# whigg/surikatoko

Hardware: AMD Instinct MI355X
Metric: BA iterations/sec (higher is better)
Workload: dtype f64

## Files before the change

### include/srk_ba.h

```cpp
#ifndef SRK_BA_H
#define SRK_BA_H
#include <stdint.h>
#ifdef __cplusplus
extern "C" {
#endif

typedef struct srk_ba srk_ba;

enum srk_status {
    SRK_STATUS_NONE = 0,
    SRK_STATUS_ABS_ERR_THRESHOLD = 1,
    SRK_STATUS_SMALL_ERR_CHANGE = 2,
    SRK_STATUS_HESSIAN_OVERFLOW = 3,
    SRK_STATUS_ERR_CONVERGED = 4,
    SRK_STATUS_MAX_ITERATIONS = 5,
    SRK_STATUS_DEVICE_ERROR = 6
};

enum srk_error {
    SRK_OK = 0,
    SRK_E_ARGS = -1,
    SRK_E_DEVICE = -2,
    SRK_E_STATE = -3,
    SRK_E_NOMEM = -4
// ... 56 lines not shown
                               int32_t n_frames, float* cam_R, float* cam_T,
                               const float* K, int shared_k,
                               const int64_t* obs_row_ptr, const int32_t* obs_frame, const float* obs_uv,
                               const float* allowed_err_change, const float* max_hessian_factor,
                               int64_t max_iterations, srk_ba_report* out);

double srk_ba_reproj_error(srk_ba*, double f0,
                           int64_t n_points, const double* points_xyz,
                           int32_t n_frames, const double* cam_R, const double* cam_T,
                           const double* K, int shared_k,
                           const int64_t* obs_row_ptr, const int32_t* obs_frame, const double* obs_uv,
                           int64_t* seen );

int srk_ba_reproj_error_mvf(srk_ba*, double f0,
                            int64_t n_points, const double* points_xyz,
                            int32_t n_frames, const double* cam_R, const double* cam_T,
                            const double* K, int shared_k,
                            const int64_t* obs_row_ptr, const int32_t* obs_frame, const double* obs_uv,
                            double z_tol, double* reproj_err, int64_t* summands );

int srk_mvf_estimate_depths(srk_ba*, int64_t n_tracks, const int64_t* row_ptr, const int32_t* frame,
                            const double* x_meter , int32_t n_frames, const double* cam_R, const double* cam_T,
                            double* depth_out );
int srk_mvf_relative_motion(srk_ba*, int64_t n_points, const double* x_anchor , const double* x_target ,
                            const double* depth_anchor , double* R_out , double* T_out );
int srk_mvf_project_onto_so3(const double* R_noisy, const double* T_noisy, double* R_out, double* T_out);

int srk_ba_normalize_scene(int64_t n_points, double* points_xyz, int32_t n_frames, double* cam_R, double* cam_T,
                           double t1y, int32_t unity_comp_ind, srk_ba_normalizer* out);
void srk_ba_revert_normalization(int64_t n_points, double* points_xyz, int32_t n_frames, double* cam_R,
                                 double* cam_T, const srk_ba_normalizer* nrm);
int srk_ba_check_world_is_normalized(int32_t n_frames, const double* cam_R, const double* cam_T, double t1y,
                                     int32_t unity_comp_ind);

int srk_ba_upload_scene(srk_ba*, double f0,
                        int64_t n_points, const double* points_xyz,
                        int32_t n_frames, const double* cam_R, const double* cam_T,
                        const double* K, int shared_k,
                        const int64_t* obs_row_ptr, const int32_t* obs_frame, const double* obs_uv,
                        int already_normalized);
int srk_ba_optimize(srk_ba*, const double* allowed_err_change, const double* max_hessian_factor,
                    int64_t max_iterations, srk_ba_report* out);
int srk_ba_download_scene(srk_ba*, double* points_xyz, double* cam_R, double* cam_T, int revert_normalization);
int srk_ba_reset_scene(srk_ba*);

int srk_ba_phase_error(srk_ba*, double* err, int64_t* seen);
int srk_ba_phase_derivatives(srk_ba*);
int srk_ba_phase_schur(srk_ba*, double hessian_factor);
int srk_ba_phase_solve(srk_ba*);
int srk_ba_phase_backsub(srk_ba*, double hessian_factor);
int srk_ba_phase_accept(srk_ba*);

enum srk_buffer {
    SRK_BUF_GRAD = 0,
    SRK_BUF_POINT_BLOCKS,
    SRK_BUF_FRAME_BLOCKS,
    SRK_BUF_POINT_FRAME,
    SRK_BUF_RCS,
    SRK_BUF_RCS_RHS,
    SRK_BUF_CORRECTIONS,
    SRK_BUF_POINTS,
    SRK_BUF_CAM_R,
    SRK_BUF_CAM_T
};
int64_t srk_ba_buffer_size(srk_ba*, int which);
int srk_ba_download(srk_ba*, int which, double* dst, int64_t count);
int srk_ba_download_rcs_rows(srk_ba*, const int64_t* rows, int64_t n_rows, double* dst);

int srk_ba_set_covisibility(srk_ba*, const int32_t* min_cv );
int srk_ba_set_rcs_mode(srk_ba*, int mode );
int srk_ba_rcs_chunks(srk_ba*);
double srk_ba_rcs_fill(srk_ba*);
double srk_ba_solve_mfma_flops(srk_ba*);

int srk_ba_set_solver_fusion(srk_ba*, int on);
int64_t srk_ba_solver_sync_timeouts(srk_ba*);
int srk_ba_solver_fusion(srk_ba*);

int64_t srk_ba_iteration_log(srk_ba*, int64_t cap, int32_t* attempts, double* ms_since_start, double* err,
                             double* hessian_factor);

int srk_ba_set_speculation(srk_ba*, int on);

int srk_ba_set_deterministic(srk_ba*, int on);
int srk_ba_deterministic(srk_ba*);

int srk_ba_set_multi_schedule(srk_ba*, int mode);
int srk_ba_multi_schedule(srk_ba*);

int srk_ba_set_frame_reordering(srk_ba*, int mode);
int srk_ba_set_frame_order(srk_ba*, const int32_t* to_internal , int32_t n_frames);
int srk_ba_frame_order(srk_ba*, int32_t* to_internal );
int srk_frame_order(int mode, int64_t n_points, int32_t n_frames, const int64_t* obs_row_ptr, const int32_t* obs_frame,
                    int32_t* to_internal );

int srk_ba_set_jacobian_mode(srk_ba*, int mode);
int srk_ba_jacobian_kernel(srk_ba*);

int srk_ba_set_storage_precision(srk_ba*, int f32);

int srk_ba_set_schur_precision(srk_ba*, int fp32);

int srk_ba_set_fixed_intrinsics(srk_ba*, int on);
int srk_ba_frame_vars(srk_ba*);
int64_t srk_ba_schur_fallback_landmarks(srk_ba*);

int srk_ba_set_intrinsic_groups(srk_ba*, const int32_t* group , int32_t n_frames, int32_t n_groups);
int srk_ba_intrinsic_groups(srk_ba*);
int srk_ba_download_intrinsics(srk_ba*, double* K, int32_t n_groups);

int srk_ba_set_robust_loss(srk_ba*, int kind , double delta_pixels);
int srk_ba_robust_loss(srk_ba*, int* kind, double* delta_pixels);
int srk_ba_observation_weights(srk_ba*, double* w, int64_t count);

int srk_ba_set_observation_information(srk_ba*, const double* q , int64_t count);
int srk_ba_observation_information(srk_ba*, double* q, int64_t count);
int srk_ba_observation_residuals(srk_ba*, double* exy_pixels , int64_t count);

int srk_ba_set_constant_blocks(srk_ba*, const uint8_t* frame_const , int32_t n_frames,
                               const uint8_t* point_const , int64_t n_points, int keep_gauge);
int srk_ba_constant_blocks(srk_ba*, uint8_t* frame_const, uint8_t* point_const, int* keep_gauge);
int srk_ba_constant_counts(srk_ba*, int32_t* n_frames, int64_t* n_points);
int srk_ba_constant_pass_ms(srk_ba*, double* points_ms, double* frames_ms);

int srk_ba_set_position_priors(srk_ba*, int64_t n_point_priors, const int64_t* point_index ,
                               const double* point_pos , const double* point_info ,
                               int32_t n_frame_priors, const int32_t* frame_index ,
                               const double* frame_centre , const double* frame_info , int keep_gauge);
int srk_ba_position_prior_counts(srk_ba*, int64_t* n_point_priors, int32_t* n_frame_priors);
int srk_ba_position_priors(srk_ba*, int64_t* point_index, double* point_pos, double* point_info, int32_t* frame_index,
                           double* frame_centre, double* frame_info, int* keep_gauge);
int srk_ba_prior_error(srk_ba*, double* e_points, double* e_frames);
int srk_ba_prior_residuals(srk_ba*, double* d_points, double* d_frames);
int srk_ba_normalize_position_priors(const srk_ba_normalizer* nrm, int64_t n, const double* pos, const double* info,
                                     double* pos_out, double* info_out);
int srk_ba_prior_pass_ms(srk_ba*, double* derivative_ms, double* error_ms);

int srk_ba_set_relative_pose_factors(srk_ba*, int32_t n, const int32_t* frame_a, const int32_t* frame_b ,
                                     const double* rel_R , const double* rel_t ,
                                     const double* info );
int srk_ba_check_relative_pose_factors(int32_t n, const int32_t* frame_a, const int32_t* frame_b, const double* rel_R,
                                       const double* rel_t, const double* info, const char** why);
int srk_ba_relative_pose_factor_count(srk_ba*, int32_t* n);
int srk_ba_relative_pose_factors(srk_ba*, int32_t* frame_a, int32_t* frame_b, double* rel_R, double* rel_t, double* info);
int srk_ba_relative_pose_error(srk_ba*, double* e);
int srk_ba_relative_pose_residuals(srk_ba*, double* r);
int srk_ba_normalize_relative_pose_factors(const srk_ba_normalizer* nrm, int32_t n, const double* rel_t, const double* info,
                                           double* rel_t_out, double* info_out);
int srk_ba_relative_pose_pass_ms(srk_ba*, double* derivative_ms, double* couple_ms, double* error_ms);

int srk_ba_phase_covariance(srk_ba*, int32_t n_frames_sel, const int32_t* frames ,
                            double* frame_blocks , int64_t n_points_sel, const int64_t* points,
                            double* point_blocks );
int srk_ba_covariances(srk_ba*, double sigma_pixels, int32_t n_frames_sel, const int32_t* frames, double* frame_cov ,
                       int64_t n_points_sel, const int64_t* points, double* point_cov , int caller_coordinates);
int srk_ba_revert_covariances(const srk_ba_normalizer* nrm, int frame_vars, int32_t n_frames, double* frame_cov ,
                              int64_t n_points, double* point_cov );
int srk_ba_set_covariance_batch(srk_ba*, int64_t max_columns);

int srk_ba_phase_cross_covariance(srk_ba*, int64_t n_ff, const int32_t* ff_a, const int32_t* ff_b,
                                  double* ff_blocks , int64_t n_pf, const int64_t* pf_point,
                                  const int32_t* pf_frame, double* pf_blocks , int64_t n_pp, const int64_t* pp_a,
                                  const int64_t* pp_b, double* pp_blocks );
int srk_ba_cross_covariances(srk_ba*, double sigma_pixels, int64_t n_ff, const int32_t* ff_a, const int32_t* ff_b, double* ff_cov,
                             int64_t n_pf, const int64_t* pf_point, const int32_t* pf_frame, double* pf_cov, int64_t n_pp,
                             const int64_t* pp_a, const int64_t* pp_b, double* pp_cov, int caller_coordinates);
// ... 42 lines not shown
```

### surikatoko_amd/_lib.py

```python
import ctypes as C
import os
import subprocess

_HERE = os.path.dirname(os.path.abspath(__file__))
_PATH = os.environ.get("SRK_BA_LIBRARY") or os.path.join(_HERE, "libsrk_ba.so")
_lib = None


class LibraryNotBuilt(RuntimeError):
    pass


def library_path():
    return _PATH


def build_library(jobs=4):
    subprocess.check_call(["make", "-s", "-j", str(jobs), "-C", os.path.join(_HERE, "csrc")])
    return _PATH


class Report(C.Structure):
    _fields_ = [("status", C.c_int32), ("optimized", C.c_int32), ("iterations", C.c_int64),
                ("attempts", C.c_int64), ("seen", C.c_int64), ("err_initial", C.c_double),
                ("err_final", C.c_double), ("hessian_factor", C.c_double), ("world_scale", C.c_double),
                ("ms_jacobian", C.c_double), ("ms_schur", C.c_double), ("ms_solve", C.c_double),
                ("ms_backsub", C.c_double), ("ms_apply", C.c_double), ("ms_error", C.c_double),
                ("ms_total", C.c_double), ("schur_launches", C.c_int64), ("jacobian_launches", C.c_int64),
                ("ms_jacobian_kernel", C.c_double), ("ms_solve_syrk", C.c_double),
                ("solve_mfma_flops", C.c_double)]

    def as_dict(self):
        return {k: getattr(self, k) for k, _ in self._fields_}


class Normalizer(C.Structure):
    _fields_ = [("R0", C.c_double * 9), ("T0", C.c_double * 3), ("world_scale", C.c_double)]


class SceneSpecC(C.Structure):
    _fields_ = [("n_frames", C.c_int32), ("grid_nx", C.c_int32), ("grid_ny", C.c_int32), ("vis_window", C.c_int32),
                ("half_extent_x", C.c_double), ("half_extent_y", C.c_double), ("f0", C.c_double),
                ("noise_x3d_hi", C.c_double), ("noise_r_hi", C.c_double), ("noise_uv_pix", C.c_double),
                ("seed", C.c_uint32)]


ALLREDUCE_FN = C.CFUNCTYPE(C.c_int, C.c_void_p, C.c_void_p, C.c_int64)

EXPORTS = [
    "srk_ba_create", "srk_ba_destroy", "srk_ba_last_error", "srk_ba_status_string", "srk_ba_device_count",
    "srk_ba_set_stream", "srk_ba_set_allreduce", "srk_ba_rccl_get_unique_id", "srk_ba_rccl_init", "srk_ba_rccl_init_second", "srk_ba_rccl_set_comm", "srk_ba_compute_inplace", "srk_ba_compute_inplace_f32", "srk_ba_reproj_error", "srk_ba_reproj_error_mvf", "srk_mvf_estimate_depths", "srk_mvf_relative_motion",
    "srk_mvf_project_onto_so3", "srk_ba_set_schur_precision", "srk_ba_set_storage_precision", "srk_ba_set_speculation", "srk_ba_set_deterministic", "srk_ba_deterministic", "srk_ba_set_multi_schedule", "srk_ba_multi_schedule", "srk_ba_set_frame_reordering", "srk_ba_set_frame_order", "srk_ba_frame_order", "srk_frame_order", "srk_ba_set_solver_fusion", "srk_ba_solver_sync_timeouts", "srk_ba_iteration_log", "srk_ba_solver_fusion", "srk_ba_set_jacobian_mode", "srk_ba_jacobian_kernel", "srk_ba_set_fixed_intrinsics", "srk_ba_frame_vars", "srk_ba_schur_fallback_landmarks",
    "srk_ba_set_robust_loss", "srk_ba_robust_loss", "srk_ba_observation_weights",
    "srk_ba_set_observation_information", "srk_ba_observation_information", "srk_ba_observation_residuals",
    "srk_ba_set_intrinsic_groups", "srk_ba_intrinsic_groups", "srk_ba_download_intrinsics",
    "srk_ba_set_constant_blocks", "srk_ba_constant_blocks", "srk_ba_constant_counts", "srk_ba_constant_pass_ms",
    "srk_ba_set_position_priors", "srk_ba_position_prior_counts", "srk_ba_position_priors", "srk_ba_prior_error",
    "srk_ba_prior_residuals", "srk_ba_normalize_position_priors", "srk_ba_prior_pass_ms",
    "srk_ba_set_relative_pose_factors", "srk_ba_check_relative_pose_factors", "srk_ba_relative_pose_factor_count", "srk_ba_relative_pose_factors",
    "srk_ba_relative_pose_error", "srk_ba_relative_pose_residuals", "srk_ba_normalize_relative_pose_factors",
    "srk_ba_relative_pose_pass_ms",
    "srk_ba_phase_covariance", "srk_ba_covariances", "srk_ba_revert_covariances", "srk_ba_set_covariance_batch",
    "srk_ba_phase_cross_covariance", "srk_ba_cross_covariances", "srk_ba_revert_cross_covariances", "srk_ba_relative_pose_covariances",
    "srk_ba_normalize_scene", "srk_ba_revert_normalization", "srk_ba_check_world_is_normalized",
    "srk_ba_upload_scene", "srk_ba_optimize", "srk_ba_download_scene", "srk_ba_reset_scene", "srk_ba_phase_error",
    "srk_ba_phase_derivatives", "srk_ba_phase_schur", "srk_ba_phase_solve", "srk_ba_phase_backsub",
    "srk_ba_phase_accept", "srk_ba_buffer_size", "srk_ba_download", "srk_ba_download_rcs_rows", "srk_ba_set_profile", "srk_ba_dense_spd_solve",
    "srk_ba_set_covisibility", "srk_ba_set_rcs_mode", "srk_ba_rcs_fill", "srk_ba_solve_mfma_flops", "srk_ba_rcs_chunks",
    "srk_scene_num_observations", "srk_scene_generate", "srk_circle_camera_shots",
    "srk_read_matrix_file", "srk_decompose_proj_mat", "srk_triangulate_least_squares", "srk_dino_load",
]


def lib():
    global _lib
    if _lib is not None:
        return _lib
    try:
        import torch
    except ImportError:
        pass
    if not os.path.exists(_PATH):
        raise LibraryNotBuilt(
            f"{_PATH} is missing: run `python -c 'import __graft_entry__ as g; g.build()'` "
            "(or make -C surikatoko_amd/csrc).  There is no CPU fallback.")
    L = C.CDLL(_PATH)
    L.srk_ba_create.restype = C.c_void_p
    L.srk_ba_create.argtypes = [C.c_int]
    L.srk_ba_destroy.argtypes = [C.c_void_p]
    L.srk_ba_destroy.restype = None
    L.srk_ba_last_error.restype = C.c_char_p
    L.srk_ba_last_error.argtypes = [C.c_void_p]
    L.srk_ba_status_string.restype = C.c_char_p
    L.srk_ba_status_string.argtypes = [C.c_int]
    L.srk_ba_reproj_error.restype = C.c_double
    L.srk_ba_reproj_error_mvf.restype = C.c_int
    L.srk_ba_buffer_size.restype = C.c_int64
    L.srk_ba_buffer_size.argtypes = [C.c_void_p, C.c_int]
    L.srk_scene_num_observations.restype = C.c_int64
    L.srk_ba_rcs_fill.restype = C.c_double
    L.srk_ba_rcs_fill.argtypes = [C.c_void_p]
    L.srk_ba_solve_mfma_flops.restype = C.c_double
    L.srk_ba_solve_mfma_flops.argtypes = [C.c_void_p]
    L.srk_ba_set_stream.argtypes = [C.c_void_p, C.c_void_p]
    L.srk_ba_set_allreduce.argtypes = [C.c_void_p, ALLREDUCE_FN, C.c_void_p, C.c_int, C.c_int]
    L.srk_ba_set_robust_loss.argtypes = [C.c_void_p, C.c_int, C.c_double]
    L.srk_ba_robust_loss.argtypes = [C.c_void_p, C.POINTER(C.c_int), C.POINTER(C.c_double)]
    L.srk_ba_observation_weights.argtypes = [C.c_void_p, C.POINTER(C.c_double), C.c_int64]
    L.srk_ba_set_observation_information.argtypes = [C.c_void_p, C.POINTER(C.c_double), C.c_int64]
    L.srk_ba_observation_information.argtypes = [C.c_void_p, C.POINTER(C.c_double), C.c_int64]
    L.srk_ba_observation_residuals.argtypes = [C.c_void_p, C.POINTER(C.c_double), C.c_int64]
    L.srk_ba_set_intrinsic_groups.argtypes = [C.c_void_p, C.c_void_p, C.c_int32, C.c_int32]
    L.srk_ba_intrinsic_groups.argtypes = [C.c_void_p]
    L.srk_ba_download_intrinsics.argtypes = [C.c_void_p, C.POINTER(C.c_double), C.c_int32]
    L.srk_ba_set_constant_blocks.argtypes = [C.c_void_p, C.c_void_p, C.c_int32, C.c_void_p, C.c_int64, C.c_int]
    L.srk_ba_constant_blocks.argtypes = [C.c_void_p, C.c_void_p, C.c_void_p, C.POINTER(C.c_int)]
    L.srk_ba_constant_counts.argtypes = [C.c_void_p, C.POINTER(C.c_int32), C.POINTER(C.c_int64)]
    L.srk_ba_constant_pass_ms.argtypes = [C.c_void_p, C.POINTER(C.c_double), C.POINTER(C.c_double)]
    L.srk_ba_set_position_priors.argtypes = [C.c_void_p, C.c_int64, C.c_void_p, C.c_void_p, C.c_void_p, C.c_int32, C.c_void_p,
                                             C.c_void_p, C.c_void_p, C.c_int]
    L.srk_ba_position_prior_counts.argtypes = [C.c_void_p, C.POINTER(C.c_int64), C.POINTER(C.c_int32)]
    L.srk_ba_position_priors.argtypes = [C.c_void_p, C.c_void_p, C.c_void_p, C.c_void_p, C.c_void_p, C.c_void_p, C.c_void_p,
                                         C.POINTER(C.c_int)]
    L.srk_ba_prior_error.argtypes = [C.c_void_p, C.POINTER(C.c_double), C.POINTER(C.c_double)]
    L.srk_ba_prior_residuals.argtypes = [C.c_void_p, C.c_void_p, C.c_void_p]
    L.srk_ba_normalize_position_priors.argtypes = [C.c_void_p, C.c_int64, C.c_void_p, C.c_void_p, C.c_void_p, C.c_void_p]
    L.srk_ba_prior_pass_ms.argtypes = [C.c_void_p, C.POINTER(C.c_double), C.POINTER(C.c_double)]
    L.srk_ba_set_relative_pose_factors.argtypes = [C.c_void_p, C.c_int32, C.c_void_p, C.c_void_p, C.c_void_p, C.c_void_p, C.c_void_p]
    L.srk_ba_check_relative_pose_factors.argtypes = [C.c_int32, C.c_void_p, C.c_void_p, C.c_void_p, C.c_void_p, C.c_void_p, C.POINTER(C.c_char_p)]
    L.srk_ba_relative_pose_factor_count.argtypes = [C.c_void_p, C.POINTER(C.c_int32)]
    L.srk_ba_relative_pose_factors.argtypes = [C.c_void_p, C.c_void_p, C.c_void_p, C.c_void_p, C.c_void_p, C.c_void_p]
    L.srk_ba_relative_pose_error.argtypes = [C.c_void_p, C.POINTER(C.c_double)]
    L.srk_ba_relative_pose_residuals.argtypes = [C.c_void_p, C.c_void_p]
    L.srk_ba_normalize_relative_pose_factors.argtypes = [C.c_void_p, C.c_int32, C.c_void_p, C.c_void_p, C.c_void_p, C.c_void_p]
    L.srk_ba_relative_pose_pass_ms.argtypes = [C.c_void_p, C.POINTER(C.c_double), C.POINTER(C.c_double), C.POINTER(C.c_double)]
# ... 14 lines not shown
```

### surikatoko_amd/ba.py

```python
import ctypes as C
import math

import numpy as np

from ._lib import Normalizer, Report, lib

BUF_GRAD, BUF_POINT_BLOCKS, BUF_FRAME_BLOCKS, BUF_POINT_FRAME, BUF_RCS, BUF_RCS_RHS, BUF_CORRECTIONS, BUF_POINTS, \
    BUF_CAM_R, BUF_CAM_T = range(10)


def _p(a):
    return a.ctypes.data_as(C.c_void_p)


def status_string(status):
    return lib().srk_ba_status_string(int(status)).decode()


def device_count():
    return int(lib().srk_ba_device_count())


class Scene:

# ... 296 lines not shown
        a32 = C.c_float(term_crit.AllowedReprojErrRelativeChange()) if a64 is not None else None
        m32 = C.c_float(term_crit.MaxHessianFactor()) if m64 is not None else None
        self._f0 = float(f0)
        self.report = Report()
        rc = self._lib.srk_ba_compute_inplace_f32(
            C.c_void_p(self._h), C.c_float(f0), C.c_int64(points.shape[0]), _p(points), C.c_int32(cam_R.shape[0]), _p(cam_R),
            _p(cam_T), _p(K), C.c_int(int(bool(shared_k))), _p(rp), _p(fr), _p(obs_uv),
            C.byref(a32) if a32 is not None else None, C.byref(m32) if m32 is not None else None,
            C.c_int64(max_iterations), C.byref(self.report))
        self._raise(rc)
        self._status = status_string(self.report.status)
        return rc == 0

    def ReprojError(self, f0, scene):
        seen = C.c_int64(0)
        e = self._lib.srk_ba_reproj_error(C.c_void_p(self._h), C.c_double(f0), *scene.scene_args(), C.byref(seen))
        if math.isnan(e):
            msg = self.last_error()
            if "hip" in msg.lower():
                raise RuntimeError("srk_ba_reproj_error: " + msg)
            raise ValueError("srk_ba_reproj_error: " + msg)
        self._f0 = float(f0)
        return float(e), int(seen.value)

    def ReprojErrorMvf(self, f0, scene, z_tol=1e-5):
        e, n = C.c_double(0), C.c_int64(0)
        rc = self._lib.srk_ba_reproj_error_mvf(C.c_void_p(self._h), C.c_double(f0), *scene.scene_args(), C.c_double(z_tol),
                                               C.byref(e), C.byref(n))
        if rc < 0:
            msg = self.last_error()
            if "hip" in msg.lower():
                raise RuntimeError("srk_ba_reproj_error_mvf: " + msg)
            raise ValueError("srk_ba_reproj_error_mvf: " + msg)
        return rc == 1, float(e.value), int(n.value)

    def ReprojErrorPixPerPoint(self, reproj_err, seen_points_count):
        return self._f0 * math.sqrt(reproj_err / float(seen_points_count))

    def OptimizationStatusString(self):
        return self._status

    def PointsCount(self):
        return self._scene.N

    def FramesCount(self):
        return self._scene.M

    def VarsCount(self):
        return 3 * self._scene.N + self.frame_vars() * self._scene.M + 4 * self.intrinsic_groups()

    def NormalizedVarsCount(self):
        return self.VarsCount() - 7

    def upload(self, f0, scene, already_normalized=False):
        self._f0 = float(f0)
        self._scene = scene
        rc = self._lib.srk_ba_upload_scene(C.c_void_p(self._h), C.c_double(f0), *scene.scene_args(),
                                           C.c_int(int(already_normalized)))
        if rc == 1:
            return False
        self._raise(rc)
        return True

    def optimize(self, term_crit=None, max_iterations=0):
        a, m = self._criteria(term_crit)
        self.report = Report()
        rc = self._lib.srk_ba_optimize(C.c_void_p(self._h), a, m, C.c_int64(max_iterations), C.byref(self.report))
        self._raise(rc)
        self._status = status_string(self.report.status)
        return rc == 0

    def download(self, scene=None, revert_normalization=True):
        scene = scene or self._scene
        self._raise(self._lib.srk_ba_download_scene(C.c_void_p(self._h), _p(scene.points), _p(scene.cam_R),
                                                    _p(scene.cam_T), C.c_int(int(revert_normalization))))
        return scene

    def reset(self):
        self._raise(self._lib.srk_ba_reset_scene(C.c_void_p(self._h)))

    def set_speculation(self, on=True):
        self._raise(self._lib.srk_ba_set_speculation(C.c_void_p(self._h), C.c_int(int(bool(on)))))

    def set_deterministic(self, on=True):
        self._raise(self._lib.srk_ba_set_deterministic(C.c_void_p(self._h), C.c_int(int(bool(on)))))

    def deterministic(self):
        return int(self._lib.srk_ba_deterministic(C.c_void_p(self._h))) == 1

    MULTI_SCHEDULES = {"allreduce": 0, "dp": 1, "dp_force": 2}

    def set_multi_schedule(self, schedule="dp"):
        self._raise(self._lib.srk_ba_set_multi_schedule(C.c_void_p(self._h), C.c_int(self.MULTI_SCHEDULES[schedule])))

    def multi_schedule(self):
        return {0: "allreduce", 1: "dp", 2: "dp (self-check passed)", 3: "allreduce (dp self-check failed)"}[
            int(self._lib.srk_ba_multi_schedule(C.c_void_p(self._h)))]

    def set_frame_reordering(self, mode=-1):
        self._raise(self._lib.srk_ba_set_frame_reordering(C.c_void_p(self._h), C.c_int(mode)))

    def set_frame_order(self, to_internal=None):
        if to_internal is None:
            self._raise(self._lib.srk_ba_set_frame_order(C.c_void_p(self._h), None, C.c_int32(0)))
        else:
            a = np.ascontiguousarray(to_internal, dtype=np.int32)
            self._raise(self._lib.srk_ba_set_frame_order(C.c_void_p(self._h), _p(a), C.c_int32(a.size)))

    def frame_order(self):
        to_int = np.zeros(self._scene.M if self._scene is not None else 0, np.int32)
        rc = self._lib.srk_ba_frame_order(C.c_void_p(self._h), _p(to_int))
        if rc < 0:
            self._raise(rc)
        return to_int if rc == 1 else None

    def set_solver_fusion(self, on=True):
        self._raise(self._lib.srk_ba_set_solver_fusion(C.c_void_p(self._h), C.c_int(int(bool(on)))))

    def solver_fusion(self):
        return bool(self._lib.srk_ba_solver_fusion(C.c_void_p(self._h)))

    def solver_sync_timeouts(self):
        self._lib.srk_ba_solver_sync_timeouts.restype = C.c_int64
        return int(self._lib.srk_ba_solver_sync_timeouts(C.c_void_p(self._h)))

    def iteration_log(self):
        fn = self._lib.srk_ba_iteration_log
        fn.restype = C.c_int64
        n = int(fn(C.c_void_p(self._h), C.c_int64(0), None, None, None, None))
        att = np.zeros(max(n, 1), dtype=np.int32)
        ms = np.zeros(max(n, 1))
        err = np.zeros(max(n, 1))
        fac = np.zeros(max(n, 1))
        fn(C.c_void_p(self._h), C.c_int64(n), att.ctypes.data_as(C.c_void_p), ms.ctypes.data_as(C.c_void_p),
           err.ctypes.data_as(C.c_void_p), fac.ctypes.data_as(C.c_void_p))
        return {"attempts": att[:n], "ms": ms[:n], "err": err[:n], "hessian_factor": fac[:n]}

    def set_jacobian_mode(self, mode=-1):
        self._raise(self._lib.srk_ba_set_jacobian_mode(C.c_void_p(self._h), C.c_int(mode)))

    def jacobian_kernel(self):
        return int(self._lib.srk_ba_jacobian_kernel(C.c_void_p(self._h)))

    def set_storage_precision(self, f32=False):
        self._raise(self._lib.srk_ba_set_storage_precision(C.c_void_p(self._h), C.c_int(int(bool(f32)))))

    def set_fixed_intrinsics(self, on=True):
        self._raise(self._lib.srk_ba_set_fixed_intrinsics(C.c_void_p(self._h), C.c_int(int(bool(on)))))

    def frame_vars(self):
        n = int(self._lib.srk_ba_frame_vars(C.c_void_p(self._h)))
        self._raise(n)
        return n

    def set_intrinsic_groups(self, groups):
        if groups is None:
            self._raise(self._lib.srk_ba_set_intrinsic_groups(C.c_void_p(self._h), None, C.c_int32(0), C.c_int32(0)))
            return
        g = np.ascontiguousarray(groups, dtype=np.int32)
        n_groups = int(g.max()) + 1 if g.size else 0
        self._raise(self._lib.srk_ba_set_intrinsic_groups(C.c_void_p(self._h), g.ctypes.data_as(C.c_void_p),
                                                          C.c_int32(g.size), C.c_int32(n_groups)))

    def intrinsic_groups(self):
        n = int(self._lib.srk_ba_intrinsic_groups(C.c_void_p(self._h)))
        self._raise(n)
# ... 446 lines not shown
```

### surikatoko_amd/csrc/srk_ba_host.hip

```cpp
#include "../../include/srk_ba.h"
#include "srk_dev.hpp"
#include "srk_cov.hpp"
#include "srk_geom.hpp"
#include "srk_plan.hpp"

#include <dlfcn.h>
#include <rccl/rccl.h>

#include <algorithm>
#include <chrono>
#include <numeric>
#include <cmath>
#include <cstdio>
#include <cstdlib>
#include <cstring>
#include <string>
#include <iterator>
#include <map>
#include <memory>
#include <vector>
#include <unordered_set>
#include <thread>

namespace {

struct DevBuf {
    void* p = nullptr;
    size_t bytes = 0;
};

}

#define SRK_FUSION_RETRIES 3
#define SRK_SLOTS 3
struct srk_ba : SrkPlanKept {
    int device = 0;
    int cus = 256;
    bool own_stream = true;
    std::string last_error;

    bool have_scene = false;
    SrkDims d{};
    double f0 = 0;
    srk_ba_normalizer nrm{};
    bool normalized_on_upload = false;

    DevBuf pts[SRK_SLOTS + 1], camR[SRK_SLOTS + 1], camT[SRK_SLOTS + 1], K, cam[SRK_SLOTS + 1];
    DevBuf pts0, camR0, camT0;
    DevBuf row_ptr, obs_frame, obs_pt, obs_uv, col_ptr, fobs_pt, fobs_uv;
    DevBuf W, Vg, Ug, scratch;
    int frame_order_mode = -1;
    std::vector<int32_t> frame_order_given;
    DevBuf grp_first, grp_count, grp_nf, grp_frames, obs_slot, pt_mask, gen_list, wg_jmin;
    DevBuf cal_list;
    DevBuf lg_item, lg_np, lg_nf, lg_pts, lg_frames, lg_obs_off, lg_obs;
    DevBuf sc_pts, sc_R, sc_T, sc_K, sc_cam, sc_frame, sc_pt, sc_uv, sc_partial, sc_out;
    DevBuf jr_first, jr_count, jr_jmin, jr_group;
    DevBuf jd_nf, jd_frames, jd_mask;
    bool deterministic = false;
    DevBuf dj_ptr, dj_ent, dj_stage, ds_pair_ptr, ds_pair_fa, ds_pair_fb, ds_pair_ent, ds_f_ptr, ds_f_ent;
    int jac_mode = -1;
    std::vector<int64_t> env_col_h, env_off_h, row_end_h, col_begin_h;
    DevBuf env_col, env_off, band_col, band_off;
    int64_t env_packed = 0, band_packed = 0;
    bool use_envelope = true;
    bool use_chunks = true;
    struct Attempt {
        DevBuf S, rhs, wy, dc, acc, dx, err_partial, info, dinv, packed, sync_flags;
        DevBuf irr;
        DevBuf det_stage, det_rhs;
        DevBuf Ssh, rsh, ysh, dcsh, dinvsh, Tsh;
        SrkChunkPlan plan;
        SrkCholSync sync;
        std::vector<DevBuf> plan_bufs;
        std::vector<char> plan_zeroed;
        std::vector<std::unique_ptr<SrkChunkPlan>> plan_children;
        std::vector<int64_t> plan_sig;
        SrkSolveProf solve_prof;
        double* host_back = nullptr;
        hipStream_t stream = nullptr;
        hipEvent_t done = nullptr;
        hipEvent_t ev_a = nullptr, ev_b = nullptr;
        double* err_dst = nullptr;
        int trial = 1;
        int slot = 0;
        bool allocated = false;
    };
    Attempt att[SRK_SLOTS];
    hipStream_t main_stream = nullptr;
    hipEvent_t ev_jac = nullptr;
    bool speculate = true;
    int cur = 0;

    srk_allreduce_fn allreduce = nullptr;
    void* allreduce_ctx = nullptr;
    int rank = 0, world = 1;
    ncclComm_t comm = nullptr;
    bool comm_owned = false;
    ncclComm_t comm2 = nullptr;
    bool spec_multi = true;
    bool dp_schedule = true;
    bool dp_force = false;
    bool dp_verified = false;
    bool dp_selfcheck_failed = false;
    DevBuf dp_chk;
    hipStream_t comm_stream = nullptr;
    hipEvent_t ev_comm = nullptr;
    DevBuf status_all;
    double* dp_back = nullptr;
    int64_t seen_global = -1;

    hipEvent_t ev[16]{};
    std::vector<hipEvent_t> chol_ev;
    bool schur_fp32 = false;
    bool store_f32 = false;
    bool fixed_k = false;
    std::vector<int32_t> igroup_user;
    int32_t igroup_n = 0;
    int32_t shk_G = 0;
    int64_t shk_ncols = 0, shk_ldb = 0;
    DevBuf Ks[SRK_SLOTS + 1], shk_grp, shk_lo, shk_hi, shk_mptr, shk_mem, shk_env;
    std::vector<int32_t> shk_grp_h, shk_first;
    std::vector<double> shk_k22_user;
    std::vector<int64_t> shk_row_end, shk_col_begin;
    int loss_kind = SRK_LOSS_NONE;
    double loss_delta_pix = 0;
    std::vector<double> info_user;
    bool info_on = false;
    DevBuf info_q, info_qf;
    bool cst_set = false;
    int cst_keep_gauge = 1;
    std::vector<uint8_t> cst_frame_user, cst_point_user;
    DevBuf cst_pts, cst_frames;
// ... 74 lines not shown
        a.Reduce = reinterpret_cast<decltype(a.Reduce)>(dlsym(a.lib, "ncclReduce"));
        a.Broadcast = reinterpret_cast<decltype(a.Broadcast)>(dlsym(a.lib, "ncclBroadcast"));
        a.GroupStart = reinterpret_cast<decltype(a.GroupStart)>(dlsym(a.lib, "ncclGroupStart"));
        a.GroupEnd = reinterpret_cast<decltype(a.GroupEnd)>(dlsym(a.lib, "ncclGroupEnd"));
        a.rooted = a.Reduce && a.Broadcast && a.GroupStart && a.GroupEnd;
        a.ok = a.GetUniqueId && a.CommInitRank && a.CommDestroy && a.AllReduce && a.GetErrorString;
        return a;
    }();
    return api;
}
}

#define HIPCHK(h, expr)                                                                              \
    do {                                                                                             \
        hipError_t _e = (expr);                                                                      \
        if (_e != hipSuccess) {                                                                      \
            (h)->last_error = std::string(#expr) + ": " + hipGetErrorString(_e);                     \
            return SRK_E_DEVICE;                                                                     \
        }                                                                                            \
    } while (0)

static int dev_alloc(srk_ba* h, DevBuf& b, size_t bytes)
{
    if (bytes == 0) bytes = 8;
    if (b.p && b.bytes >= bytes) return SRK_OK;
    if (b.p) {
        hipFree(b.p);
        b.p = nullptr;
        b.bytes = 0;
    }
    hipError_t e = hipMalloc(&b.p, bytes);
    if (e != hipSuccess) {
        h->last_error = std::string("hipMalloc: ") + hipGetErrorString(e);
        b.p = nullptr;
        return e == hipErrorOutOfMemory ? SRK_E_NOMEM : SRK_E_DEVICE;
    }
    b.bytes = bytes;
    return SRK_OK;
}
static void dev_free(DevBuf& b)
{
    if (b.p) hipFree(b.p);
    b.p = nullptr;
    b.bytes = 0;
}
template <typename T> static T* P(const DevBuf& b) { return reinterpret_cast<T*>(b.p); }

extern "C" {

int srk_ba_device_count(void)
{
    int n = 0;
    if (hipGetDeviceCount(&n) != hipSuccess) return 0;
    return n;
}

srk_ba* srk_ba_create(int device_id)
{
    int n = srk_ba_device_count();
    if (n <= 0 || device_id < 0 || device_id >= n) {
        fprintf(stderr, "srk_ba_create: no usable HIP device (count=%d, requested=%d); there is no CPU fallback\n", n,
                device_id);
        return nullptr;
    }
    if (hipSetDevice(device_id) != hipSuccess) return nullptr;
    srk_ba* h = new srk_ba();
    h->device = device_id;
    hipDeviceProp_t prop;
    if (hipGetDeviceProperties(&prop, device_id) == hipSuccess && prop.multiProcessorCount > 0) h->cus = prop.multiProcessorCount;
    if (hipStreamCreate(&h->main_stream) != hipSuccess) {
        delete h;
        return nullptr;
    }
#ifdef SRK_DEV
    if (const char* e = getenv("SRK_CHOL_FUSED")) h->chol_fused = h->chol_fused_wanted = e[0] != '0';
    if (const char* e = getenv("SRK_MULTI_SPECULATION")) h->spec_multi = e[0] != '0';
    if (const char* e = getenv("SRK_MULTI_SCHEDULE")) {
        h->dp_schedule = std::strcmp(e, "allreduce") != 0;
        h->dp_force = std::strcmp(e, "dp_force") == 0;
    }
#endif
    h->att[0].stream = h->main_stream;
    bool ok = hipEventCreateWithFlags(&h->ev_jac, hipEventDisableTiming) == hipSuccess &&
              hipEventCreateWithFlags(&h->ev_comm, hipEventDisableTiming) == hipSuccess &&
              hipStreamCreateWithFlags(&h->comm_stream, hipStreamNonBlocking) == hipSuccess &&
              hipHostMalloc(reinterpret_cast<void**>(&h->dp_back), 64 * SRK_SLOTS, hipHostMallocDefault) == hipSuccess &&
              hipMalloc(&h->status_all.p, 64 * SRK_SLOTS) == hipSuccess;
    if (ok) h->status_all.bytes = 64 * SRK_SLOTS, ok = hipMemset(h->status_all.p, 0, 64 * SRK_SLOTS) == hipSuccess;
    for (int sl = 0; sl < SRK_SLOTS; ++sl) {
        auto& a = h->att[sl];
        a.slot = sl;
        a.trial = sl + 1;
        a.err_dst = ok ? P<double>(h->status_all) + 8 * sl : nullptr;
        if (sl > 0) ok = ok && hipStreamCreateWithFlags(&a.stream, hipStreamNonBlocking) == hipSuccess;
        ok = ok && hipEventCreateWithFlags(&a.done, hipEventDisableTiming) == hipSuccess &&
             hipEventCreateWithFlags(&a.ev_a, hipEventDisableTiming) == hipSuccess &&
             hipEventCreateWithFlags(&a.ev_b, hipEventDisableTiming) == hipSuccess &&
             hipHostMalloc(reinterpret_cast<void**>(&a.host_back), 64, hipHostMallocDefault) == hipSuccess;
    }
    for (auto& e : h->ev) ok = ok && hipEventCreate(&e) == hipSuccess;
    if (!ok) {
        delete h;
        return nullptr;
    }
    return h;
}

void srk_ba_destroy(srk_ba* h)
{
    if (!h) return;
    hipSetDevice(h->device);
    if (h->main_stream) hipStreamSynchronize(h->main_stream);
    for (int sl = 1; sl < SRK_SLOTS; ++sl)
        if (h->att[sl].stream) hipStreamSynchronize(h->att[sl].stream);
    if (h->comm_stream) hipStreamSynchronize(h->comm_stream);
    if (h->comm2) rccl().CommDestroy(h->comm2);
    if (h->comm && h->comm_owned) rccl().CommDestroy(h->comm);
    h->comm = h->comm2 = nullptr;
    for (int w = 0; w < SRK_SLOTS + 1; ++w)
        for (DevBuf* b : { &h->pts[w], &h->camR[w], &h->camT[w], &h->cam[w], &h->Ks[w] }) dev_free(*b);
    dev_free(h->status_all);
    if (h->dp_back) hipHostFree(h->dp_back);
    DevBuf* all[] = { &h->K, &h->pts0, &h->camR0, &h->camT0, &h->row_ptr,
                      &h->obs_frame, &h->obs_pt, &h->obs_uv, &h->col_ptr, &h->fobs_pt, &h->fobs_uv, &h->W, &h->Vg, &h->Ug,
                      &h->scratch, &h->grp_first, &h->grp_count, &h->grp_nf, &h->grp_frames, &h->obs_slot, &h->pt_mask,
                      &h->gen_list, &h->cal_list, &h->env_col, &h->env_off, &h->wg_jmin, &h->band_col, &h->band_off,
                      &h->dj_ptr, &h->dj_ent, &h->dj_stage, &h->ds_pair_ptr, &h->ds_pair_fa, &h->ds_pair_fb, &h->ds_pair_ent, &h->ds_f_ptr, &h->ds_f_ent,
                      &h->jd_nf, &h->jd_frames, &h->jd_mask,
                      &h->jr_first, &h->jr_count, &h->jr_jmin, &h->jr_group, &h->lg_item, &h->lg_np, &h->lg_nf, &h->lg_pts, &h->lg_frames,
                      &h->lg_obs_off, &h->lg_obs, &h->shk_grp, &h->shk_lo, &h->shk_hi, &h->shk_mptr, &h->shk_mem, &h->shk_env, &h->dp_chk,
                      &h->info_q, &h->info_qf, &h->cst_pts, &h->cst_frames, &h->pri_pt_list, &h->pri_pt_val, &h->pri_fr_list, &h->pri_fr_val,
                      &h->rp_fa, &h->rp_fb, &h->rp_val, &h->rp_fr_list, &h->rp_fr_ptr, &h->rp_fr_ent, &h->rp_tgt, &h->rp_cpl,
                      &h->cov_Y, &h->cov_grp, &h->cov_blk, &h->cov_out, &h->cov_free, &h->cov_colb, &h->cov_pairs };
    for (DevBuf* b : all) dev_free(*b);
    for (auto& a : h->att) {
        for (DevBuf* b : { &a.S, &a.rhs, &a.wy, &a.dc, &a.acc, &a.dx, &a.err_partial, &a.info, &a.dinv, &a.packed, &a.sync_flags, &a.irr, &a.det_stage, &a.det_rhs,
                          &a.Ssh, &a.rsh, &a.ysh, &a.dcsh, &a.dinvsh, &a.Tsh }) dev_free(*b);
        for (DevBuf& b : a.plan_bufs) dev_free(b);
        if (a.host_back) hipHostFree(a.host_back);
        if (a.done) hipEventDestroy(a.done);
        if (a.ev_a) hipEventDestroy(a.ev_a);
        if (a.ev_b) hipEventDestroy(a.ev_b);
    }
    for (DevBuf* b : { &h->sc_pts, &h->sc_R, &h->sc_T, &h->sc_K, &h->sc_cam, &h->sc_frame, &h->sc_pt, &h->sc_uv, &h->sc_partial, &h->sc_out })
        dev_free(*b);
    for (auto& e : h->ev)
        if (e) hipEventDestroy(e);
    for (auto& e : h->chol_ev) hipEventDestroy(e);
    if (h->ev_jac) hipEventDestroy(h->ev_jac);
    for (auto& e : h->ev_cst)
        if (e) hipEventDestroy(e);
    for (auto& e : h->ev_pri)
        if (e) hipEventDestroy(e);
    for (auto& e : h->ev_rp)
        if (e) hipEventDestroy(e);
    if (h->ev_comm) hipEventDestroy(h->ev_comm);
    if (h->comm_stream) hipStreamDestroy(h->comm_stream);
    for (int sl = 1; sl < SRK_SLOTS; ++sl)
        if (h->att[sl].stream) hipStreamDestroy(h->att[sl].stream);
    if (h->own_stream && h->main_stream) hipStreamDestroy(h->main_stream);
    delete h;
}

const char* srk_ba_last_error(const srk_ba* h) { return h ? h->last_error.c_str() : "null handle"; }

const char* srk_ba_status_string(int status)
{
    switch (status) {
    case SRK_STATUS_ABS_ERR_THRESHOLD: return "abs err threshold";
    case SRK_STATUS_SMALL_ERR_CHANGE: return "small relative err change";
    case SRK_STATUS_HESSIAN_OVERFLOW: return "hessian overflow";
    case SRK_STATUS_ERR_CONVERGED: return "err converged to limit value";
    case SRK_STATUS_MAX_ITERATIONS: return "max iterations";
    case SRK_STATUS_DEVICE_ERROR: return "device error";
    default: return "";
    }
}

int srk_ba_set_stream(srk_ba* h, void* hip_stream)
{
    if (!h) return SRK_E_ARGS;
    hipSetDevice(h->device);
    if (h->main_stream) hipStreamSynchronize(h->main_stream);
    if (h->own_stream && h->main_stream) hipStreamDestroy(h->main_stream);
    h->main_stream = h->att[0].stream = reinterpret_cast<hipStream_t>(hip_stream);
    h->own_stream = false;
    return SRK_OK;
}

static bool exchange_after_reordered_upload(srk_ba* h, int world_size)
{
    if (world_size < 2 || !h->have_scene || h->frame_int.empty() || h->frame_order_supplied) return false;
    h->last_error = "the uploaded scene's frames were renumbered for one rank; configure the exchange before the upload";
    return true;
}

static const char* fixed_k_conflict(bool fixed_k, bool deterministic, bool store_f32, bool schur_fp32, int world)
{
    if (!fixed_k) return nullptr;
    if (deterministic) return "fixed intrinsics: not available in deterministic mode";
    if (store_f32) return "fixed intrinsics: not available with f32 storage of the point-frame blocks";
    if (schur_fp32) return "fixed intrinsics: not available with fp32 Schur accumulation";
    if (world > 1) return "fixed intrinsics: not available with more than one rank";
    return nullptr;
}
static const char* groups_conflict(bool groups, bool fixed_k, bool store_f32, bool schur_fp32, int world)
{
    if (!groups) return nullptr;
    if (fixed_k) return "intrinsic groups: not available with fixed intrinsics";
    if (store_f32) return "intrinsic groups: not available with f32 storage of the point-frame blocks";
    if (schur_fp32) return "intrinsic groups: not available with fp32 Schur accumulation";
    if (world > 1) return "intrinsic groups: not available with more than one rank";
    return nullptr;
}
static const char* constant_conflict(bool constant, bool groups, int world)
{
    if (!constant) return nullptr;
    if (groups) return "constant blocks: not available with intrinsic groups";
    if (world > 1) return "constant blocks: not available with more than one rank";
    return nullptr;
}
static const char* prior_conflict(bool priors, bool groups, int world)
{
    if (!priors) return nullptr;
    if (groups) return "position priors: not available with intrinsic groups";
    if (world > 1) return "position priors: not available with more than one rank";
    return nullptr;
}
static const char* relpose_conflict(bool factors, bool groups, int world)
{
    if (!factors) return nullptr;
    if (groups) return "relative-pose factors: not available with intrinsic groups";
    if (world > 1) return "relative-pose factors: not available with more than one rank";
    return nullptr;
}
static bool refuse_modes(srk_ba* h, bool fixed_k, bool deterministic, bool store_f32, bool schur_fp32, int world, bool groups)
{
    const char* e = fixed_k_conflict(fixed_k, deterministic, store_f32, schur_fp32, world);
    if (!e) e = groups_conflict(groups, fixed_k, store_f32, schur_fp32, world);
    if (!e) e = constant_conflict(h->cst_set, groups, world);
    if (!e) e = prior_conflict(h->pri_set, groups, world);
    if (!e) e = relpose_conflict(h->rp_set, groups, world);
    if (e) h->last_error = e;
    return e != nullptr;
}

int srk_ba_set_allreduce(srk_ba* h, srk_allreduce_fn fn, void* ctx, int rank, int world_size)
{
    if (!h || world_size < 1 || rank < 0 || rank >= world_size) return SRK_E_ARGS;
    if (refuse_modes(h, h->fixed_k, h->deterministic, h->store_f32, h->schur_fp32, world_size, !h->igroup_user.empty())) return SRK_E_ARGS;
    if (exchange_after_reordered_upload(h, world_size)) return SRK_E_STATE;
    if (h->comm || h->comm2) {
        hipSetDevice(h->device);
        if (h->main_stream) hipStreamSynchronize(h->main_stream);
        for (int sl = 1; sl < SRK_SLOTS; ++sl)
            if (h->att[sl].stream) hipStreamSynchronize(h->att[sl].stream);
        if (h->comm_stream) hipStreamSynchronize(h->comm_stream);
        if (h->comm2) rccl().CommDestroy(h->comm2);
        if (h->comm && h->comm_owned) rccl().CommDestroy(h->comm);
        h->comm = h->comm2 = nullptr;
        h->comm_owned = false;
    }
    h->allreduce = fn;
    h->allreduce_ctx = ctx;
    h->rank = rank;
    h->world = world_size;
    h->seen_global = -1;
    return SRK_OK;
}

int srk_ba_rccl_get_unique_id(void* id128)
{
    if (!id128 || !rccl().ok) return SRK_E_DEVICE;
    static_assert(sizeof(ncclUniqueId) == 128, "ncclUniqueId");
    return rccl().GetUniqueId(reinterpret_cast<ncclUniqueId*>(id128)) == ncclSuccess ? SRK_OK : SRK_E_DEVICE;
}
static int rccl_attach(srk_ba* h, ncclComm_t comm, bool owned, int rank, int world_size)
{
    if (refuse_modes(h, h->fixed_k, h->deterministic, h->store_f32, h->schur_fp32, world_size, !h->igroup_user.empty())) {
        if (owned) rccl().CommDestroy(comm);
        return SRK_E_ARGS;
    }
    if (exchange_after_reordered_upload(h, world_size)) {
        if (owned) rccl().CommDestroy(comm);
        return SRK_E_STATE;
    }
    if (h->comm && h->comm_owned) rccl().CommDestroy(h->comm);
    if (h->comm2) rccl().CommDestroy(h->comm2);
    h->comm2 = nullptr;
    h->comm = comm;
    h->comm_owned = owned;
    h->allreduce = nullptr;
    h->allreduce_ctx = nullptr;
    h->rank = rank;
    h->world = world_size;
    h->seen_global = -1;
    return SRK_OK;
}
int srk_ba_rccl_init(srk_ba* h, const void* id128, int rank, int world_size)
{
    if (!h || !id128 || world_size < 1 || rank < 0 || rank >= world_size) return SRK_E_ARGS;
    if (!rccl().ok) { h->last_error = "librccl.so could not be loaded"; return SRK_E_DEVICE; }
    HIPCHK(h, hipSetDevice(h->device));
    ncclUniqueId id;
    std::memcpy(&id, id128, sizeof id);
    ncclComm_t comm = nullptr;
    ncclResult_t r = rccl().CommInitRank(&comm, world_size, id, rank);
    if (r != ncclSuccess) { h->last_error = std::string("ncclCommInitRank: ") + rccl().GetErrorString(r); return SRK_E_DEVICE; }
    return rccl_attach(h, comm, true, rank, world_size);
}
int srk_ba_rccl_init_second(srk_ba* h, const void* id128)
{
    if (!h || !id128) return SRK_E_ARGS;
    if (!h->comm || !rccl().ok) { h->last_error = "srk_ba_rccl_init_second: srk_ba_rccl_init comes first"; return SRK_E_STATE; }
    HIPCHK(h, hipSetDevice(h->device));
    ncclUniqueId id;
// ... 609 lines not shown
    h->cov_pt_frame0.clear();

    struct Up { DevBuf& buf; const void* src; size_t bytes; };
    std::vector<Up> up;
    auto add = [&](DevBuf& b, const void* src, int64_t bytes) { up.push_back({ b, src, (size_t)bytes }); };
    auto tab = [&](DevBuf& b, const auto& v, size_t at_least = 0) { add(b, v.empty() ? nullptr : v.data(), (int64_t)(sizeof(v[0]) * std::max(v.size(), at_least))); };
    const int n_slots = (opt.multi_rank && h->dp_schedule && h->speculate && (h->world >= 2 || h->dp_force))
                            ? (h->dp_force ? SRK_SLOTS : std::min(SRK_SLOTS, h->world))
                            : (h->speculate ? 2 : 1);
    for (int w = 0; w <= n_slots; ++w) {
        add(h->pts[w], w ? nullptr : plan.pts.data(), 24 * N);
        add(h->camR[w], w ? nullptr : plan.camR.data(), 72 * (int64_t)M);
        add(h->camT[w], w ? nullptr : plan.camT.data(), 24 * (int64_t)M);
        add(h->cam[w], nullptr, 8 * SRK_CAM_PACK * (int64_t)M);
        if (h->shk_G > 0) add(h->Ks[w], w ? nullptr : plan.K.data(), 72 * (int64_t)M);
    }
    tab(h->pts0, plan.pts); tab(h->camR0, plan.camR); tab(h->camT0, plan.camT); tab(h->K, plan.K);
    tab(h->row_ptr, plan.row_ptr_int); tab(h->obs_frame, plan.obs_frame); tab(h->obs_pt, plan.obs_pt); tab(h->obs_uv, plan.obs_uv);
    tab(h->col_ptr, plan.col_ptr); tab(h->fobs_pt, plan.fobs_pt); tab(h->fobs_uv, plan.fobs_uv);
    add(h->W, nullptr, (d.w_f32 ? 4 : 8) * SRK_WF_PLANES * d.Os);
    add(h->Vg, nullptr, 8 * 9 * d.Ns);
    add(h->Ug, nullptr, 8 * SRK_UGS(d.fv) * (int64_t)M);
    bool new_flags[SRK_SLOTS] = {};
    for (int sl = 0; sl < SRK_SLOTS; ++sl) {
        srk_ba::Attempt& a = h->att[sl];
        a.allocated = sl < n_slots;
        if (!a.allocated) continue;
        if (plan.det_active) {
            add(a.det_stage, nullptr, 8 * (int64_t)SRK_DET_STRIDE * plan.n_groups);
            add(a.det_rhs, nullptr, 8 * (int64_t)SRK_DET_LD * plan.n_groups);
        }
        add(a.S, nullptr, 8 * d.ld * d.ld);
        add(a.rhs, nullptr, 8 * d.ld);
        add(a.wy, nullptr, 8 * 2 * d.ld);
        add(a.dc, nullptr, 8 * d.ld);
        add(a.acc, nullptr, 8 * 3 * d.Ns + 64);
        add(a.dx, nullptr, 24 * N);
        add(a.err_partial, nullptr, 8 * (std::max<int64_t>(1024, srk_error_partials_staged(d)) +
                                         (h->pri_set ? srk_prior_partials((int64_t)h->pri_pt_idx.size(), (int64_t)h->pri_fr_idx.size()) : 0) +
                                         srk_relpose_partials((int64_t)h->rp_act.size())));
        add(a.info, nullptr, 64);
        add(a.dinv, nullptr, 8 * 64 * d.ld);
        add(a.irr, nullptr, 4 * (N + 2));
        new_flags[sl] = !a.sync_flags.p;
        if (new_flags[sl]) add(a.sync_flags, nullptr, 4 * SRK_SYNC_WORDS);
    }
    tab(h->cal_list, plan.cal_list);
    tab(h->grp_first, plan.grp_first); tab(h->grp_count, plan.grp_count); tab(h->grp_nf, plan.grp_nf); tab(h->grp_frames, plan.grp_frames);
    tab(h->obs_slot, plan.obs_slot); tab(h->pt_mask, plan.pt_mask); tab(h->gen_list, plan.gen_list);
    tab(h->lg_item, plan.lg_item); tab(h->lg_np, plan.lg_np); tab(h->lg_nf, plan.lg_nf); tab(h->lg_pts, plan.lg_pts);
    tab(h->lg_frames, plan.lg_frames); tab(h->lg_obs_off, plan.lg_obs_off); tab(h->lg_obs, plan.lg_obs);
    tab(h->wg_jmin, plan.wg_jmin);
    if (plan.jac_runs) {
        tab(h->jr_first, plan.jr_first); tab(h->jr_count, plan.jr_count); tab(h->jr_jmin, plan.jr_jmin);
        if (plan.jac_runs_masked) tab(h->jr_group, plan.jr_group);
    }
    if (plan.det_active) {
        tab(h->dj_ptr, plan.dj_ptr); tab(h->dj_ent, plan.dj_ent, 1);
        add(h->dj_stage, nullptr, 8 * (int64_t)SRK_UG * 64 * (int64_t)plan.jr_first.size());
        tab(h->ds_pair_ptr, plan.ds_pair_ptr); tab(h->ds_pair_fa, plan.ds_pair_fa, 1); tab(h->ds_pair_fb, plan.ds_pair_fb, 1); tab(h->ds_pair_ent, plan.ds_pair_ent, 1);
        tab(h->ds_f_ptr, plan.ds_f_ptr); tab(h->ds_f_ent, plan.ds_f_ent, 1);
    }
    if (plan.jr_own_runs) {
        tab(h->jd_nf, plan.jd_nf); tab(h->jd_frames, plan.jd_frames); tab(h->jd_mask, plan.jd_mask);
    }
    for (const Up& u : up)
        if ((rc = dev_alloc(h, u.buf, u.bytes)) != SRK_OK) return rc;
    hipStream_t s = h->main_stream;
    stage("device allocations");
    for (const Up& u : up)
        if (u.src && u.bytes > 0) HIPCHK(h, hipMemcpyAsync(u.buf.p, u.src, u.bytes, hipMemcpyHostToDevice, s));
    for (int sl = 0; sl < SRK_SLOTS; ++sl) {
        srk_ba::Attempt& a = h->att[sl];
        if (!a.allocated) continue;
        HIPCHK(h, hipMemsetAsync(a.irr.p, 0, 4, s));
        if (new_flags[sl]) HIPCHK(h, hipMemset(a.sync_flags.p, 0, 4 * SRK_SYNC_WORDS));
        a.sync.flags = P<unsigned>(a.sync_flags);
        a.sync.fused = h->chol_fused;
        HIPCHK(h, hipMemsetAsync(a.dc.p, 0, 8 * d.ld, s));
        HIPCHK(h, hipMemsetAsync(a.dx.p, 0, 24 * N > 0 ? 24 * N : 8, s));
    }
    h->cur = 0;
    for (int sl = 0; sl < SRK_SLOTS; ++sl) h->att[sl].trial = sl + 1;
    rc = compute_cam_packs(h, 0);
    if (rc != SRK_OK) return rc;
    HIPCHK(h, hipStreamSynchronize(s));
    static_cast<SrkPlanKept&>(*h) = plan;
    stage("host-to-device copies");
    rc = build_envelope(h);
    if (rc != SRK_OK) return rc;
    if (h->shk_G > 0) {
        if ((rc = build_shared_k(h)) != SRK_OK) return rc;
    } else {
        for (auto& a : h->att)
            for (DevBuf* b : { &a.Ssh, &a.rsh, &a.ysh, &a.dcsh, &a.dinvsh, &a.Tsh }) dev_free(*b);
    }
    stage("skyline, solver plans");
    if ((rc = apply_information(h)) != SRK_OK) return rc;
    if ((rc = apply_constant_blocks(h)) != SRK_OK) return rc;
    if ((rc = apply_position_priors(h)) != SRK_OK) return rc;
    if ((rc = apply_relative_pose_factors(h)) != SRK_OK) return rc;
    h->have_scene = true;
    return SRK_OK;
}

static int apply_relative_pose_factors(srk_ba* h)
{
    const SrkDims& d = h->d;
    h->n_rp = 0;
    h->n_rp_frames = 0;
    h->rp_int_a.clear(); h->rp_int_b.clear();
    h->app_rp = h->rp_set;
    h->app_rp_a = h->rp_a; h->app_rp_b = h->rp_b; h->app_rp_R = h->rp_R; h->app_rp_t = h->rp_t;
    const size_t n = h->rp_act.size();
    if (n == 0) return SRK_OK;
    std::vector<double> tn(h->rp_t.size()), ln(h->rp_info.size());
    srk_ba_normalize_relative_pose_factors(&h->nrm, (int32_t)h->rp_a.size(), h->rp_t.data(), h->rp_info.data(), tn.data(), ln.data());
    std::vector<int32_t> fa(n), fb(n);
    std::vector<double> val((size_t)SRK_RP_PLANES * n);
    std::vector<int64_t> tgt(n);
    const int64_t t0 = 4 - (10 - d.fv);
    for (size_t i = 0; i < n; ++i) {
        const size_t k = (size_t)h->rp_act[i];
        fa[i] = h->frame_int.empty() ? h->rp_a[k] : h->frame_int[(size_t)h->rp_a[k]];
        fb[i] = h->frame_int.empty() ? h->rp_b[k] : h->frame_int[(size_t)h->rp_b[k]];
        for (int e = 0; e < 9; ++e) val[(size_t)e * n + i] = h->rp_R[9 * k + (size_t)e];
        for (int e = 0; e < 3; ++e) val[(size_t)(9 + e) * n + i] = tn[3 * k + (size_t)e];
        for (int e = 0; e < 21; ++e) val[(size_t)(12 + e) * n + i] = ln[21 * k + (size_t)e];
        const int64_t hi = std::max(fa[i], fb[i]), lo = std::min(fa[i], fb[i]);
        tgt[i] = (d.fv * hi + t0) * d.ld + d.fv * lo + t0;
    }
    std::vector<int32_t> cnt((size_t)d.M, 0), list, ptr(1, 0), ent;
    for (size_t i = 0; i < n; ++i) { ++cnt[(size_t)fa[i]]; ++cnt[(size_t)fb[i]]; }
    std::vector<int32_t> at((size_t)d.M, -1);
    for (int32_t j = 0; j < d.M; ++j)
        if (cnt[(size_t)j]) {
            at[(size_t)j] = (int32_t)list.size();
            list.push_back(j);
            ptr.push_back(ptr.back() + cnt[(size_t)j]);
        }
    ent.resize((size_t)ptr.back());
    std::vector<int32_t> fill(ptr.begin(), ptr.end() - 1);
    for (size_t i = 0; i < n; ++i) {
        ent[(size_t)fill[(size_t)at[(size_t)fa[i]]]++] = (int32_t)(2 * i);
        ent[(size_t)fill[(size_t)at[(size_t)fb[i]]]++] = (int32_t)(2 * i + 1);
    }
    HIPCHK(h, hipSetDevice(h->device));
    hipStream_t s = h->main_stream;
    int rc;
    struct { DevBuf* b; const void* src; size_t bytes; } up[] = {
        { &h->rp_fa, fa.data(), 4 * n }, { &h->rp_fb, fb.data(), 4 * n }, { &h->rp_val, val.data(), 8 * val.size() },
        { &h->rp_fr_list, list.data(), 4 * list.size() }, { &h->rp_fr_ptr, ptr.data(), 4 * ptr.size() },
        { &h->rp_fr_ent, ent.data(), 4 * ent.size() }, { &h->rp_tgt, tgt.data(), 8 * n },
    };
    for (auto& u : up) {
        if ((rc = dev_alloc(h, *u.b, u.bytes)) != SRK_OK) return rc;
        HIPCHK(h, hipMemcpyAsync(u.b->p, u.src, u.bytes, hipMemcpyHostToDevice, s));
    }
    if ((rc = dev_alloc(h, h->rp_cpl, 8 * 36 * n)) != SRK_OK) return rc;
    HIPCHK(h, hipMemsetAsync(h->rp_cpl.p, 0, 8 * 36 * n, s));
    HIPCHK(h, hipStreamSynchronize(s));
    h->rp_int_a = fa;
    h->rp_int_b = fb;
    h->n_rp = (int32_t)n;
    h->n_rp_frames = (int32_t)list.size();
    return SRK_OK;
// ... 197 lines not shown
            HIPCHK(h, hipMemsetAsync(a.ysh.p, 0, 16 * ldb, h->main_stream));
            HIPCHK(h, hipMemsetAsync(a.dcsh.p, 0, 8 * ldb, h->main_stream));
        }
        for (size_t i = 0; i < a.plan_bufs.size(); ++i)
            if (a.plan_zeroed[i]) HIPCHK(h, hipMemsetAsync(a.plan_bufs[i].p, 0, a.plan_bufs[i].bytes, h->main_stream));
    }
    HIPCHK(h, hipStreamSynchronize(h->main_stream));
    h->poisoned = false;
    return SRK_OK;
}

static void frames_to_user(const srk_ba* h, double* a, int w)
{
    if (h->frame_int.empty()) return;
    const int32_t M = h->d.M;
    std::vector<double> tmp(a, a + (size_t)w * (size_t)M);
    for (int32_t j = 0; j < M; ++j) std::memcpy(a + (size_t)w * (size_t)j, &tmp[(size_t)w * (size_t)h->frame_int[(size_t)j]], (size_t)(8 * w));
}

extern "C" int srk_ba_reset_scene(srk_ba* h)
{
    if (!h || !h->have_scene) return SRK_E_STATE;
    HIPCHK(h, hipSetDevice(h->device));
    hipStream_t s = h->main_stream;
    for (int sl = 1; sl < SRK_SLOTS; ++sl) HIPCHK(h, hipStreamSynchronize(h->att[sl].stream));
    {
        int rcp = clear_poison(h);
        if (rcp != SRK_OK) return rcp;
    }
    h->cur = 0;
    for (int sl = 0; sl < SRK_SLOTS; ++sl) h->att[sl].trial = sl + 1;
    if (h->d.N > 0) HIPCHK(h, hipMemcpyAsync(h->pts[0].p, h->pts0.p, 24 * h->d.N, hipMemcpyDeviceToDevice, s));
    HIPCHK(h, hipMemcpyAsync(h->camR[0].p, h->camR0.p, 72 * (int64_t)h->d.M, hipMemcpyDeviceToDevice, s));
    HIPCHK(h, hipMemcpyAsync(h->camT[0].p, h->camT0.p, 24 * (int64_t)h->d.M, hipMemcpyDeviceToDevice, s));
    if (h->shk_G > 0) HIPCHK(h, hipMemcpyAsync(h->Ks[0].p, h->K.p, 72 * (int64_t)h->d.M, hipMemcpyDeviceToDevice, s));
    return compute_cam_packs(h, 0);
}

extern "C" int srk_ba_download_scene(srk_ba* h, double* pts, double* cam_R, double* cam_T, int revert)
{
    if (!h || !h->have_scene) return SRK_E_STATE;
    HIPCHK(h, hipSetDevice(h->device));
    hipStream_t s = h->main_stream;
    int c = h->cur;
    std::vector<double> tmp((size_t)(3 * h->d.N));
    if (h->d.N > 0) HIPCHK(h, hipMemcpyAsync(tmp.data(), h->pts[c].p, 24 * h->d.N, hipMemcpyDeviceToHost, s));
    HIPCHK(h, hipMemcpyAsync(cam_R, h->camR[c].p, 72 * (int64_t)h->d.M, hipMemcpyDeviceToHost, s));
    HIPCHK(h, hipMemcpyAsync(cam_T, h->camT[c].p, 24 * (int64_t)h->d.M, hipMemcpyDeviceToHost, s));
    HIPCHK(h, hipStreamSynchronize(s));
    frames_to_user(h, cam_R, 9);
    frames_to_user(h, cam_T, 3);
    for (int64_t i = 0; i < h->d.N; ++i) std::memcpy(pts + 3 * h->perm[(size_t)i], &tmp[(size_t)(3 * i)], 24);
    if (revert && h->normalized_on_upload) srk_ba_revert_normalization(h->d.N, pts, h->d.M, cam_R, cam_T, &h->nrm);
    return SRK_OK;
}


static int exchange(srk_ba* h, srk_ba::Attempt& a, double* dev_ptr, int64_t count)
{
    if (h->comm) {
        ncclComm_t comm = (a.slot == 1 && h->comm2) ? h->comm2 : h->comm;
        ncclResult_t r = rccl().AllReduce(dev_ptr, dev_ptr, (size_t)count, ncclDouble, ncclSum, comm, a.stream);
        if (r != ncclSuccess) {
            h->last_error = std::string("ncclAllReduce: ") + rccl().GetErrorString(r);
            return SRK_E_DEVICE;
        }
        return SRK_OK;
    }
    if (!h->allreduce) return SRK_OK;
    HIPCHK(h, hipStreamSynchronize(a.stream));
    int rc = h->allreduce(h->allreduce_ctx, dev_ptr, count);
    if (rc != 0) {
        h->last_error = "allreduce hook failed";
        return SRK_E_DEVICE;
    }
    return SRK_OK;
}

enum { SRK_COLL_ALLREDUCE = 0, SRK_COLL_REDUCE = 1, SRK_COLL_BCAST = 2 };
#define SRK_RETRY_ALLREDUCE 1000
#ifdef SRK_DEV
static int g_dp_corrupt = 0;
extern "C" void srk_dbg_dp_corrupt(int stage) { g_dp_corrupt = stage; }
#endif
static int dp_checksum(srk_ba* h, hipStream_t st, const double* p, int64_t n, double out[2])
{
    int rc = dev_alloc(h, h->dp_chk, 8 * (512 + 2 + 16));
    if (rc != SRK_OK) return rc;
    srk_launch_checksum(st, p, n, P<double>(h->dp_chk), P<double>(h->dp_chk) + 512);
    HIPCHK(h, hipGetLastError());
    HIPCHK(h, hipMemcpyAsync(out, P<double>(h->dp_chk) + 512, 16, hipMemcpyDeviceToHost, st));
    HIPCHK(h, hipStreamSynchronize(st));
    return SRK_OK;
}
static int dp_allreduce_host(srk_ba* h, double* v, int n)
{
    int rc = dev_alloc(h, h->dp_chk, 8 * (512 + 2 + 16));
    if (rc != SRK_OK) return rc;
    double* stage = P<double>(h->dp_chk) + 514;
    HIPCHK(h, hipMemcpyAsync(stage, v, (size_t)(8 * n), hipMemcpyHostToDevice, h->comm_stream));
    ncclResult_t r = rccl().AllReduce(stage, stage, (size_t)n, ncclDouble, ncclSum, h->comm, h->comm_stream);
    if (r != ncclSuccess) { h->last_error = std::string("ncclAllReduce (self-check): ") + rccl().GetErrorString(r); return SRK_E_DEVICE; }
    HIPCHK(h, hipMemcpyAsync(v, stage, (size_t)(8 * n), hipMemcpyDeviceToHost, h->comm_stream));
    HIPCHK(h, hipStreamSynchronize(h->comm_stream));
    return SRK_OK;
}
static int coll_group(srk_ba* h, int op, int G, double* const* ptrs, const int64_t* counts)
{
    if (h->comm) {
        for (int k = 0; k < G; ++k) {
            HIPCHK(h, hipEventRecord(h->att[k].ev_a, h->att[k].stream));
            HIPCHK(h, hipStreamWaitEvent(h->comm_stream, h->att[k].ev_a, 0));
        }
        const bool rooted = rccl().rooted && op != SRK_COLL_ALLREDUCE;
        if (!rooted && op == SRK_COLL_BCAST)
            for (int k = 0; k < G; ++k)
                if (h->rank != k % h->world) HIPCHK(h, hipMemsetAsync(ptrs[k], 0, (size_t)(8 * counts[k]), h->comm_stream));
        ncclResult_t r = ncclSuccess;
        if (rooted) r = rccl().GroupStart();
        for (int k = 0; k < G && r == ncclSuccess; ++k) {
            const int root = k % h->world;
            if (rooted && op == SRK_COLL_REDUCE)
                r = rccl().Reduce(ptrs[k], ptrs[k], (size_t)counts[k], ncclDouble, ncclSum, root, h->comm, h->comm_stream);
            else if (rooted && op == SRK_COLL_BCAST)
                r = rccl().Broadcast(ptrs[k], ptrs[k], (size_t)counts[k], ncclDouble, root, h->comm, h->comm_stream);
            else
                r = rccl().AllReduce(ptrs[k], ptrs[k], (size_t)counts[k], ncclDouble, ncclSum, h->comm, h->comm_stream);
        }
        if (rooted) {
            ncclResult_t r2 = rccl().GroupEnd();
            if (r == ncclSuccess) r = r2;
        }
        if (r != ncclSuccess) {
            h->last_error = std::string("RCCL collective: ") + rccl().GetErrorString(r);
            return SRK_E_DEVICE;
        }
        HIPCHK(h, hipEventRecord(h->ev_comm, h->comm_stream));
        for (int k = 0; k < G; ++k) HIPCHK(h, hipStreamWaitEvent(h->att[k].stream, h->ev_comm, 0));
        return SRK_OK;
    }
    if (!h->allreduce) return SRK_OK;
    for (int k = 0; k < G; ++k) {
        hipStream_t st = h->att[k].stream;
        if (op == SRK_COLL_BCAST && h->rank != k % h->world) HIPCHK(h, hipMemsetAsync(ptrs[k], 0, (size_t)(8 * counts[k]), st));
        HIPCHK(h, hipStreamSynchronize(st));
        if (h->allreduce(h->allreduce_ctx, ptrs[k], counts[k]) != 0) {
            h->last_error = "allreduce hook failed";
            return SRK_E_DEVICE;
        }
    }
    return SRK_OK;
}

static const SrkLoss* robust_loss(const srk_ba* h, SrkLoss& L)
{
    if (h->loss_kind == SRK_LOSS_NONE && !h->info_on) return nullptr;
    L.kind = h->loss_kind;
    L.d = h->loss_delta_pix / h->f0;
    L.d2 = L.d * L.d;
    L.q = h->info_on ? P<double>(h->info_q) : nullptr;
    L.qf = h->info_on && !h->fobs_of.empty() ? P<double>(h->info_qf) : nullptr;
    return &L;
}

static int phase_error(srk_ba* h, srk_ba::Attempt& a, int which, double* err_host, bool with_status = false, bool no_exchange = false)
{
    const SrkDims& d = h->d;
    hipStream_t s = a.stream;
    int32_t np = srk_error_partials(d);
    SrkLoss L;
    SrkPrior pr;
    const SrkPrior* prior = position_priors(h, pr);
    const bool timed = prior && h->profile_level >= 1 && pri_events(h);
    if (prior) h->pri_timed[1] = timed;
    SrkRelPose rpl;
    const SrkRelPose* relpose = relpose_factors(h, rpl);
    const bool rp_timed = relpose && h->profile_level >= 1 && rp_events(h);
    if (relpose) h->rp_timed[2] = rp_timed;
    srk_launch_error(s, d, P<double>(h->pts[which]), P<double>(h->cam[which]), P<int32_t>(h->obs_frame),
                     P<int32_t>(h->obs_pt), P<double>(h->obs_uv), P<double>(a.err_partial), np, a.err_dst,
                     h->jac_fused ? P<int32_t>(h->wg_jmin) : nullptr, with_status ? P<int>(a.info) : nullptr,
                     with_status ? reinterpret_cast<int*>(reinterpret_cast<char*>(a.acc.p) + 8 * 3 * d.Ns) : nullptr,
                     robust_loss(h, L), prior, timed ? &h->ev_pri[2] : nullptr, relpose, rp_timed ? &h->ev_rp[4] : nullptr);
    HIPCHK(h, hipGetLastError());
    int rc = no_exchange ? SRK_OK : exchange(h, a, a.err_dst, with_status ? 3 : 1);
    if (rc != SRK_OK) return rc;
    if (err_host) {
        HIPCHK(h, hipMemcpyAsync(err_host, a.err_dst, 8, hipMemcpyDeviceToHost, s));
        HIPCHK(h, hipStreamSynchronize(s));
    }
    return SRK_OK;
}

static bool cst_events(srk_ba* h)
{
    for (auto& e : h->ev_cst)
        if (!e && hipEventCreate(&e) != hipSuccess) return false;
    return true;
}

static int phase_derivatives(srk_ba* h)
{
    const SrkDims& d = h->d;
    hipStream_t s = h->main_stream;
    int c = h->cur;
    HIPCHK(h, hipMemsetAsync(h->Vg.p, 0, 8 * 9 * d.Ns, s));
    HIPCHK(h, hipMemsetAsync(h->Ug.p, 0, 8 * SRK_UGS(d.fv) * (int64_t)d.M, s));
    if (h->profile_level >= 1) HIPCHK(h, hipEventRecord(h->ev[12], s));
    const SrkDetJac detj{ P<double>(h->dj_stage), P<int32_t>(h->dj_ptr), P<int32_t>(h->dj_ent) };
    SrkLoss Ls;
    const SrkLoss* L = robust_loss(h, Ls);
    if (h->jac_runs) {
        srk_launch_jac_runs(s, d, P<double>(h->pts[c]), P<double>(h->cam[c]), P<int64_t>(h->row_ptr), P<int32_t>(h->obs_frame),
                            P<double>(h->obs_uv), P<double>(h->W), P<double>(h->Vg), P<double>(h->Ug), P<int32_t>(h->jr_first),
                            P<int32_t>(h->jr_count), h->jr_tasks, P<int32_t>(h->jr_jmin),
                            h->jac_runs_masked ? P<int32_t>(h->jr_group) : nullptr,
                            h->jr_own_runs ? P<int32_t>(h->jd_nf) : P<int32_t>(h->grp_nf),
                            h->jr_own_runs ? P<int32_t>(h->jd_frames) : P<int32_t>(h->grp_frames),
                            h->jr_own_runs ? P<uint32_t>(h->jd_mask) : P<uint32_t>(h->pt_mask), h->det_active ? &detj : nullptr,
                            h->jr_own_runs ? SRK_JD_MAXNF_HOST : SRK_GRP_MAXNF_HOST, L);
        if (h->profile_level >= 1) HIPCHK(h, hipEventRecord(h->ev[13], s));
    } else if (h->jac_fused) {
        srk_launch_jac_fused(s, d, P<double>(h->pts[c]), P<double>(h->cam[c]), P<int32_t>(h->obs_frame),
                             P<int32_t>(h->obs_pt), P<double>(h->obs_uv), P<double>(h->W), P<double>(h->Vg),
                             P<double>(h->Ug), P<int32_t>(h->wg_jmin), L);
        if (h->profile_level >= 1) HIPCHK(h, hipEventRecord(h->ev[13], s));
    } else {
        srk_launch_jac_points(s, d, P<double>(h->pts[c]), P<double>(h->cam[c]), P<int32_t>(h->obs_frame),
                              P<int32_t>(h->obs_pt), P<double>(h->obs_uv), P<double>(h->W), P<double>(h->Vg), L);
        if (h->profile_level >= 1) HIPCHK(h, hipEventRecord(h->ev[13], s));
        srk_launch_jac_frames(s, d, h->max_frame_obs, P<double>(h->pts[c]), P<double>(h->cam[c]),
                              P<int64_t>(h->col_ptr), P<int32_t>(h->fobs_pt), P<double>(h->fobs_uv), P<double>(h->Ug), L);
    }
    HIPCHK(h, hipGetLastError());
    SrkPrior pr;
    if (const SrkPrior* prior = position_priors(h, pr)) {
        const bool timed = h->profile_level >= 1 && pri_events(h);
        if (timed) HIPCHK(h, hipEventRecord(h->ev_pri[0], s));
        srk_launch_prior_add(s, d, P<double>(h->pts[c]), P<double>(h->cam[c]), *prior, P<double>(h->Vg), P<double>(h->Ug));
        if (timed) HIPCHK(h, hipEventRecord(h->ev_pri[1], s));
        h->pri_timed[0] = timed;
        HIPCHK(h, hipGetLastError());
    }
    SrkRelPose rpl;
    if (const SrkRelPose* relpose = relpose_factors(h, rpl)) {
        const bool timed = h->profile_level >= 1 && rp_events(h);
        if (timed) HIPCHK(h, hipEventRecord(h->ev_rp[0], s));
        srk_launch_relpose_add(s, d, P<double>(h->cam[c]), *relpose, P<double>(h->Ug));
        if (timed) HIPCHK(h, hipEventRecord(h->ev_rp[1], s));
        h->rp_timed[0] = timed;
        HIPCHK(h, hipGetLastError());
    }
    if (h->n_cst_pts > 0) {
        const bool timed = h->profile_level >= 1 && cst_events(h);
        if (timed) HIPCHK(h, hipEventRecord(h->ev_cst[0], s));
        srk_launch_const_points(s, d, P<int32_t>(h->cst_pts), h->n_cst_pts, P<int64_t>(h->row_ptr), P<double>(h->W), P<double>(h->Vg));
        if (timed) HIPCHK(h, hipEventRecord(h->ev_cst[1], s));
        h->cst_timed[0] = timed;
        HIPCHK(h, hipGetLastError());
    }
    return SRK_OK;
}

static int phase_schur(srk_ba* h, srk_ba::Attempt& a, double c, bool local_only = false);
static int schur_pack(srk_ba* h, srk_ba::Attempt& a)
{
    const SrkDims& d = h->d;
    hipStream_t s = a.stream;
    int rc;
    if ((rc = dev_alloc(h, a.packed, (size_t)(8 * (h->band_packed + d.ld)))) != SRK_OK) return rc;
    double* tail = P<double>(a.packed) + h->band_packed;
    srk_launch_band_pack(s, d.ld, P<int64_t>(h->band_col), P<int64_t>(h->band_off), P<double>(a.S), P<double>(a.packed), 0);
    HIPCHK(h, hipMemcpyAsync(tail, a.rhs.p, (size_t)(8 * d.ld), hipMemcpyDeviceToDevice, s));
    HIPCHK(h, hipGetLastError());
    return SRK_OK;
}
static int schur_unpack(srk_ba* h, srk_ba::Attempt& a)
{
    const SrkDims& d = h->d;
    hipStream_t s = a.stream;
    double* tail = P<double>(a.packed) + h->band_packed;
    srk_launch_band_pack(s, d.ld, P<int64_t>(h->band_col), P<int64_t>(h->band_off), P<double>(a.S), P<double>(a.packed), 1);
    HIPCHK(h, hipMemcpyAsync(a.rhs.p, tail, (size_t)(8 * d.ld), hipMemcpyDeviceToDevice, s));
    HIPCHK(h, hipGetLastError());
    return SRK_OK;
}
static int phase_schur(srk_ba* h, srk_ba::Attempt& a, double c, bool local_only)
{
    const SrkDims& d = h->d;
    hipStream_t s = a.stream;
    srk_launch_env_zero(s, d.ld, P<int64_t>(h->env_col), P<double>(a.S), P<double>(a.rhs), P<int32_t>(a.irr));
    const SrkDetSchur dets{ P<double>(a.det_stage), P<double>(a.det_rhs), P<int32_t>(h->ds_pair_ptr), P<int32_t>(h->ds_pair_fa),
                            P<int32_t>(h->ds_pair_fb), P<int32_t>(h->ds_pair_ent), h->ds_n_pairs, P<int32_t>(h->ds_f_ptr), P<int32_t>(h->ds_f_ent) };
    const bool cal = d.fv == 6;
    srk_launch_schur_grouped(s, d, c, P<int64_t>(h->row_ptr), P<int32_t>(h->obs_pt), P<uint8_t>(h->obs_slot),
                             P<uint32_t>(h->pt_mask), P<double>(h->W), P<double>(h->Vg), P<double>(a.S),
                             P<double>(a.rhs), P<int32_t>(h->grp_first), P<int32_t>(h->grp_count), P<int32_t>(h->grp_nf),
                             P<int32_t>(h->grp_frames), h->n_groups, h->n_groups_wide, h->n_groups_mid,
                             !cal && h->schur_fp32 ? 1 : 0, P<int32_t>(a.irr), h->n_mm_uniform, h->n_mm_ragged,
                             !cal && h->det_active ? &dets : nullptr);
    if (cal) {
        srk_launch_schur(s, d, c, P<int64_t>(h->row_ptr), P<int32_t>(h->obs_frame), P<double>(h->W), P<double>(h->Vg),
                         P<double>(a.S), P<double>(a.rhs), P<int32_t>(h->cal_list), h->n_cal_list);
    } else {
        srk_launch_schur_long(s, d, c, P<double>(h->W), P<double>(h->Vg), P<double>(a.S), P<double>(a.rhs),
                              P<int32_t>(h->lg_item), h->n_long_items, P<int32_t>(h->lg_np), P<int32_t>(h->lg_nf), P<int32_t>(h->lg_pts),
                              P<int32_t>(h->lg_frames), P<int64_t>(h->lg_obs_off), P<int32_t>(h->lg_obs), h->long_fb);
        srk_launch_schur(s, d, c, P<int64_t>(h->row_ptr), P<int32_t>(h->obs_frame), P<double>(h->W), P<double>(h->Vg),
                         P<double>(a.S), P<double>(a.rhs), P<int32_t>(h->gen_list), h->n_generic);
    }
    HIPCHK(h, hipGetLastError());
    srk_launch_assemble(s, d, c, P<double>(h->Ug), P<double>(a.S), P<double>(a.rhs), h->rank == 0 ? 1.0 : 0.0,
                        P<int64_t>(h->row_ptr), P<int32_t>(h->obs_frame), P<double>(h->W), P<double>(h->Vg), P<int32_t>(a.irr));
    HIPCHK(h, hipGetLastError());
    SrkRelPose rpl;
    if (const SrkRelPose* relpose = relpose_factors(h, rpl)) {
        const bool timed = h->profile_level >= 1 && rp_events(h);
        if (timed) HIPCHK(h, hipEventRecord(h->ev_rp[2], s));
        srk_launch_relpose_couple(s, d, *relpose, P<double>(a.S));
        if (timed) HIPCHK(h, hipEventRecord(h->ev_rp[3], s));
        h->rp_timed[1] = timed;
        HIPCHK(h, hipGetLastError());
    }
    if (h->n_cst_frames > 0) {
        const bool timed = h->profile_level >= 1 && cst_events(h);
        if (timed) HIPCHK(h, hipEventRecord(h->ev_cst[2], s));
        srk_launch_const_frames(s, d, P<int32_t>(h->cst_frames), h->n_cst_frames, P<int64_t>(h->env_col), P<double>(a.S), P<double>(a.rhs));
        if (timed) HIPCHK(h, hipEventRecord(h->ev_cst[3], s));
        h->cst_timed[1] = timed;
        HIPCHK(h, hipGetLastError());
    }
    if (h->shk_G > 0) {
        srk_launch_rcs_fold(s, shk_args(h, a), P<double>(a.S), P<double>(a.rhs), P<double>(a.Ssh), P<double>(a.rsh));
        HIPCHK(h, hipGetLastError());
    }
    h->last_hessian_factor = c;
    if ((h->allreduce || h->comm) && !local_only) {
        int rc = schur_pack(h, a);
        if (rc == SRK_OK) rc = exchange(h, a, P<double>(a.packed), h->band_packed + d.ld);
        if (rc == SRK_OK) rc = schur_unpack(h, a);
        if (rc != SRK_OK) return rc;
    }
    return SRK_OK;
}

static int launch_solve(srk_ba* h, srk_ba::Attempt& a, SrkSolveProf* prof)
{
    const SrkDims& d = h->d;
    if (h->shk_G > 0) {
        const bool sky = h->use_envelope;
        double* w = P<double>(a.ysh);
        if (!(prof && prof->dry)) HIPCHK(h, hipMemcpyAsync(w, a.rsh.p, (size_t)(8 * h->shk_ldb), hipMemcpyDeviceToDevice, a.stream));
        srk_chol_solve_bordered(a.stream, h->shk_ncols, h->shk_ldb, P<double>(a.Ssh), w, w + h->shk_ldb,
                                P<double>(a.dcsh), P<double>(a.dinvsh), P<int>(a.info), sky ? h->shk_row_end.data() : nullptr,
                                sky ? h->shk_col_begin.data() : nullptr, 6 * (int64_t)d.M, 4 * (int64_t)h->shk_G, prof, &a.sync);
    } else if (a.plan.P >= 2)
        srk_chol_solve_chunked(a.stream, a.plan, d.ld, P<double>(a.S), P<double>(a.rhs), P<double>(a.dc),
                               P<int64_t>(h->env_col), P<int>(a.info), prof, &a.sync);
    else
        srk_chol_solve(a.stream, d.ld, P<double>(a.S), P<double>(a.rhs), P<double>(a.wy), P<double>(a.dc),
                       P<int>(a.info), h->row_end_h.data(), h->col_begin_h.data(), P<double>(a.dinv), prof, &a.sync, d.fv * (int64_t)d.M);
    return SRK_OK;
}

static int phase_solve(srk_ba* h, srk_ba::Attempt& a, bool profile)
{
    const SrkDims& d = h->d;
    if (!h->lean_resets) HIPCHK(h, hipMemsetAsync(a.info.p, 0, 4, a.stream));
    a.solve_prof = SrkSolveProf{};
    if (profile) {
        size_t need = (size_t)(2 * (2 * (d.ld / SRK_CHOL_NB) + 64));
        while (h->chol_ev.size() < need) {
            hipEvent_t e;
            HIPCHK(h, hipEventCreate(&e));
            h->chol_ev.push_back(e);
        }
        a.solve_prof.ev = h->chol_ev.data();
        a.solve_prof.cap = h->chol_ev.size();
    }
    const int rc = launch_solve(h, a, profile ? &a.solve_prof : nullptr);
    if (rc != SRK_OK) return rc;
    HIPCHK(h, hipGetLastError());
    return SRK_OK;
}

static int read_info(srk_ba* h, srk_ba::Attempt& a, int* info_host)
{
    HIPCHK(h, hipMemcpyAsync(info_host, a.info.p, 4, hipMemcpyDeviceToHost, a.stream));
    HIPCHK(h, hipStreamSynchronize(a.stream));
    return SRK_OK;
}

static int phase_backsub_apply(srk_ba* h, srk_ba::Attempt& a, double c)
{
    const SrkDims& d = h->d;
    hipStream_t s = a.stream;
    int cur = h->cur, tr = a.trial;
    if (!h->lean_resets) HIPCHK(h, hipMemsetAsync(a.acc.p, 0, 8 * 3 * d.Ns + 64, s));
    if (h->shk_G > 0)
        srk_launch_rcs_expand(s, shk_args(h, a), P<double>(a.dcsh), P<double>(a.dc), kbuf(h, cur), kbuf(h, tr));
    srk_launch_backsub(s, d, c, P<int32_t>(h->obs_frame), P<int32_t>(h->obs_pt), P<double>(h->W), P<double>(h->Vg),
                       P<double>(a.dc), P<double>(a.acc), P<double>(h->pts[cur]), P<double>(h->pts[tr]),
                       P<double>(a.dx));
    HIPCHK(h, hipGetLastError());
    return SRK_OK;
}

static int phase_cam_apply(srk_ba* h, srk_ba::Attempt& a)
{
    int cur = h->cur, tr = a.trial;
    srk_launch_cam_apply(a.stream, h->d.M, P<double>(h->camR[cur]), P<double>(h->camT[cur]), P<double>(a.dc),
                         P<double>(h->camR[tr]), P<double>(h->camT[tr]), kbuf(h, tr), h->f0, P<double>(h->cam[tr]), h->d.fv);
    srk_launch_const_cam_keep(a.stream, P<int32_t>(h->cst_frames), h->n_cst_frames, P<double>(h->camR[cur]), P<double>(h->camT[cur]),
                              P<double>(h->cam[cur]), P<double>(h->camR[tr]), P<double>(h->camT[tr]), P<double>(h->cam[tr]));
    HIPCHK(h, hipGetLastError());
    return SRK_OK;
}

extern "C" {

int srk_ba_phase_error(srk_ba* h, double* err, int64_t* seen)
{
    if (!h || !h->have_scene) return SRK_E_STATE;
    HIPCHK(h, hipSetDevice(h->device));
    if (seen) *seen = h->d.O;
    return phase_error(h, h->att[0], h->cur, err);
}
int srk_ba_phase_derivatives(srk_ba* h)
{
    if (!h || !h->have_scene) return SRK_E_STATE;
    HIPCHK(h, hipSetDevice(h->device));
    int rc = phase_derivatives(h);
    if (rc != SRK_OK) return rc;
    HIPCHK(h, hipStreamSynchronize(h->main_stream));
    return SRK_OK;
}
int srk_ba_phase_schur(srk_ba* h, double c)
{
    if (!h || !h->have_scene) return SRK_E_STATE;
    HIPCHK(h, hipSetDevice(h->device));
    srk_ba::Attempt& a = h->att[0];
    h->last_slot = 0;
    int rc = clear_poison(h);
    if (rc != SRK_OK) return rc;
    rc = phase_schur(h, a, c);
    if (rc != SRK_OK) return rc;
    HIPCHK(h, hipStreamSynchronize(a.stream));
    return SRK_OK;
}
int srk_ba_phase_solve(srk_ba* h)
{
    if (!h || !h->have_scene) return SRK_E_STATE;
    HIPCHK(h, hipSetDevice(h->device));
    srk_ba::Attempt& a = h->att[0];
    int rc = phase_solve(h, a, false);
    if (rc != SRK_OK) return rc;
    int info = 0;
    rc = read_info(h, a, &info);
    if (rc != SRK_OK) return rc;
    if (info && srk_debug()) fprintf(stderr, "srk_ba_phase_solve: info=%d (1 = pivot, 4 = non-finite solution, 8 = hand-off timeout of the fused solve)\n", info);
    if ((info & 8) && a.plan.P >= 2) {
        fusion_off(h);
        HIPCHK(h, hipStreamSynchronize(a.stream));
        for (size_t i = 0; i < a.plan_bufs.size(); ++i)
            if (a.plan_zeroed[i]) HIPCHK(h, hipMemsetAsync(a.plan_bufs[i].p, 0, a.plan_bufs[i].bytes, a.stream));
        HIPCHK(h, hipMemsetAsync(a.info.p, 0, 4, a.stream));
        rc = phase_solve(h, a, false);
        if (rc != SRK_OK) return rc;
        rc = read_info(h, a, &info);
        if (rc != SRK_OK) return rc;
    } else if (info & 8) {
        fusion_off(h);
        h->last_error = "a hand-off of the fused solve timed out; the system was factorised in place: call srk_ba_phase_schur again "
                        "(the unfused launch sequence is selected from now on)";
    }
    if (info) h->poisoned = true;
    return info ? 1 : 0;
}
int srk_ba_phase_backsub(srk_ba* h, double c)
{
    if (!h || !h->have_scene) return SRK_E_STATE;
    HIPCHK(h, hipSetDevice(h->device));
    srk_ba::Attempt& a = h->att[0];
    int rc = phase_backsub_apply(h, a, c);
    if (rc != SRK_OK) return rc;
    rc = phase_cam_apply(h, a);
    if (rc != SRK_OK) return rc;
    HIPCHK(h, hipStreamSynchronize(a.stream));
    return SRK_OK;
}
int srk_ba_phase_accept(srk_ba* h)
{
    if (!h || !h->have_scene) return SRK_E_STATE;
    std::swap(h->cur, h->att[0].trial);
    return SRK_OK;
}

}


static void cov_revert_frame(const srk_ba_normalizer& nrm, int fv, double* B)
{
    const int off = fv - 6;
    const double is = 1.0 / nrm.world_scale;
    double D[100] = {};
    for (int i = 0; i < off; ++i) D[i * fv + i] = 1.0;
    for (int a = 0; a < 3; ++a)
        for (int b = 0; b < 3; ++b) {
            D[(off + a) * fv + off + b] = nrm.R0[3 * b + a] * is;
            D[(off + 3 + a) * fv + off + 3 + b] = nrm.R0[3 * b + a];
        }
    double T[100];
    for (int i = 0; i < fv; ++i)
        for (int j = 0; j < fv; ++j) {
            double v = 0;
            for (int k = 0; k < fv; ++k) v += D[i * fv + k] * B[k * fv + j];
            T[i * fv + j] = v;
        }
    for (int i = 0; i < fv; ++i)
        for (int j = i; j < fv; ++j) {
            double v = 0;
            for (int k = 0; k < fv; ++k) v += T[i * fv + k] * D[j * fv + k];
            B[i * fv + j] = B[j * fv + i] = v;
        }
}
static void cov_revert_point(const srk_ba_normalizer& nrm, double* B)
{
    const double is2 = 1.0 / (nrm.world_scale * nrm.world_scale);
    const double* R = nrm.R0;
    double T[9];
    for (int i = 0; i < 3; ++i)
        for (int j = 0; j < 3; ++j) T[3 * i + j] = R[i] * B[j] + R[3 + i] * B[3 + j] + R[6 + i] * B[6 + j];
    for (int i = 0; i < 3; ++i)
        for (int j = i; j < 3; ++j) B[3 * i + j] = B[3 * j + i] = (T[3 * i] * R[j] + T[3 * i + 1] * R[3 + j] + T[3 * i + 2] * R[6 + j]) * is2;
}

static int cov_check_args(srk_ba* h, int32_t nf, const int32_t* frames, const double* fb, int64_t np, const int64_t* points, const double* pb)
{
    if (nf < 0 || np < 0 || (nf > 0 && (!frames || !fb)) || (np > 0 && (!points || !pb))) {
        h->last_error = "covariance: a negative count, or a NULL array with a positive count";
        return SRK_E_ARGS;
    }
    if (h->world > 1 || h->allreduce || h->comm) { h->last_error = "covariance: more than one rank is not supported"; return SRK_E_ARGS; }
    if (h->shk_G > 0) { h->last_error = "covariance: intrinsic groups are not supported"; return SRK_E_ARGS; }
    for (int32_t k = 0; k < nf; ++k)
        if (frames[k] < 0 || frames[k] >= h->d.M) { h->last_error = "covariance: a frame index is out of range"; return SRK_E_ARGS; }
    for (int64_t k = 0; k < np; ++k)
        if (points[k] < 0 || points[k] >= h->d.N) { h->last_error = "covariance: a landmark index is out of range"; return SRK_E_ARGS; }
    return SRK_OK;
}

static int cov_prepare(srk_ba* h, bool want_selection, bool want_points, std::vector<int64_t>& pt_int)
{
    const SrkDims& d = h->d;
    srk_ba::Attempt& a = h->att[0];
    hipStream_t s = a.stream;
    const int fv = d.fv;
    const int64_t n_rows = fv * (int64_t)d.M;
    int rc;
    HIPCHK(h, hipMemsetAsync(a.info.p, 0, 4, s));
    HIPCHK(h, hipMemsetAsync(a.rhs.p, 0, (size_t)(8 * d.ld), s));
    srk_chol_solve(s, d.ld, P<double>(a.S), P<double>(a.rhs), P<double>(a.wy), P<double>(a.dc), P<int>(a.info), h->row_end_h.data(),
                   h->col_begin_h.data(), P<double>(a.dinv), nullptr, nullptr, n_rows);
    HIPCHK(h, hipGetLastError());
    int info = 0;
    if ((rc = read_info(h, a, &info)) != SRK_OK) return rc;
    if (info) { h->poisoned = true; return 1; }
    if (!want_selection) return 0;

// ... 78 lines not shown
            grp.push_back(g);
            ++b1;
        }
        const int64_t ncp = (cols + SRK_COV_CB - 1) / SRK_COV_CB * SRK_COV_CB;
        blk.assign((size_t)(ncp / SRK_COV_CB), n_tiles);
        for (const SrkCovGroup& g : grp)
            for (int64_t q = g.col0 / SRK_COV_CB; q <= (g.col0 + g.ncols - 1) / SRK_COV_CB; ++q)
                blk[(size_t)q] = std::min<int32_t>(blk[(size_t)q], g.first_row / 64);
        const int32_t ng = (int32_t)grp.size();
        if ((rc = dev_alloc(h, h->cov_Y, (size_t)(8 * d.ld * ncp))) != SRK_OK) return rc;
        if ((rc = dev_alloc(h, h->cov_grp, sizeof(SrkCovGroup) * grp.size())) != SRK_OK) return rc;
        if ((rc = dev_alloc(h, h->cov_blk, 4 * blk.size())) != SRK_OK) return rc;
        if ((rc = dev_alloc(h, h->cov_out, (size_t)(800 * ng))) != SRK_OK) return rc;
        HIPCHK(h, hipMemcpyAsync(h->cov_grp.p, grp.data(), sizeof(SrkCovGroup) * grp.size(), hipMemcpyHostToDevice, s));
        HIPCHK(h, hipMemcpyAsync(h->cov_blk.p, blk.data(), 4 * blk.size(), hipMemcpyHostToDevice, s));
        HIPCHK(h, hipMemsetAsync(h->cov_Y.p, 0, (size_t)(8 * 64 * (int64_t)n_tiles * ncp), s));
        HIPCHK(h, hipMemsetAsync(h->cov_out.p, 0, (size_t)(800 * ng), s));
        srk_launch_cov_rhs(s, d, c, P<SrkCovGroup>(h->cov_grp), ng, P<int64_t>(h->row_ptr), P<int32_t>(h->obs_frame), P<double>(h->W),
                           P<double>(h->Vg), P<uint8_t>(h->cov_free), P<double>(h->cov_Y), ncp, P<int>(a.info));
        srk_launch_cov_fwd(s, d.ld, P<double>(a.S), P<double>(a.dinv), P<int64_t>(h->cov_colb), n_tiles, P<int32_t>(h->cov_blk),
                           P<double>(h->cov_Y), ncp);
        srk_launch_cov_gram(s, d, c, P<SrkCovGroup>(h->cov_grp), ng, P<double>(h->Vg), P<double>(h->cov_Y), ncp, n_rows, P<double>(h->cov_out));
        HIPCHK(h, hipGetLastError());
        HIPCHK(h, hipMemcpyAsync(res.data() + 100 * b0, h->cov_out.p, (size_t)(800 * ng), hipMemcpyDeviceToHost, s));
        HIPCHK(h, hipStreamSynchronize(s));
        b0 = b1;
    }
    if ((rc = read_info(h, a, &info)) != SRK_OK) return rc;
    if (info) return 1;
    for (size_t k = 0; k < sel.size(); ++k) {
        const int n = sel[k].g.ncols;
        for (int e = 0; e < n * n; ++e)
            if (!std::isfinite(res[100 * k + e])) return 1;
    }
    for (size_t k = 0; k < sel.size(); ++k) {
        const int n = sel[k].g.ncols;
        double* dst = sel[k].g.is_point ? point_blocks + 9 * (sel[k].dst - nf) : frame_blocks + (int64_t)fv * fv * sel[k].dst;
        std::memcpy(dst, res.data() + 100 * k, sizeof(double) * (size_t)(n * n));
    }
    for (int64_t k = 0; k < np; ++k)
        if (pt_zero[(size_t)k]) std::fill(point_blocks + 9 * k, point_blocks + 9 * k + 9, 0.0);
    return 0;
}

extern "C" {

int srk_ba_set_covariance_batch(srk_ba* h, int64_t max_columns)
{
    if (!h || max_columns < 0) return SRK_E_ARGS;
    h->cov_batch_cols = max_columns;
    return SRK_OK;
}

int srk_ba_phase_covariance(srk_ba* h, int32_t n_frames_sel, const int32_t* frames, double* frame_blocks, int64_t n_points_sel,
                            const int64_t* points, double* point_blocks)
{
    if (!h || !h->have_scene) return SRK_E_STATE;
    int rc = cov_check_args(h, n_frames_sel, frames, frame_blocks, n_points_sel, points, point_blocks);
    if (rc != SRK_OK) return rc;
    HIPCHK(h, hipSetDevice(h->device));
    return phase_covariance(h, n_frames_sel, frames, frame_blocks, n_points_sel, points, point_blocks);
}

int srk_ba_revert_covariances(const srk_ba_normalizer* nrm, int frame_vars, int32_t n_frames, double* frame_cov, int64_t n_points,
                              double* point_cov)
{
    if (!nrm || (frame_vars != 6 && frame_vars != 10) || n_frames < 0 || n_points < 0 || (n_frames > 0 && !frame_cov) ||
        (n_points > 0 && !point_cov) || !(nrm->world_scale > 0) || !std::isfinite(nrm->world_scale))
        return SRK_E_ARGS;
    for (int32_t k = 0; k < n_frames; ++k) cov_revert_frame(*nrm, frame_vars, frame_cov + (int64_t)frame_vars * frame_vars * k);
    for (int64_t k = 0; k < n_points; ++k) cov_revert_point(*nrm, point_cov + 9 * k);
    return SRK_OK;
}

int srk_ba_covariances(srk_ba* h, double sigma_pixels, int32_t n_frames_sel, const int32_t* frames, double* frame_cov,
                       int64_t n_points_sel, const int64_t* points, double* point_cov, int caller_coordinates)
{
    if (!h || !h->have_scene) return SRK_E_STATE;
    if (!(sigma_pixels > 0) || !std::isfinite(sigma_pixels)) { h->last_error = "covariances: sigma_pixels must be finite and positive"; return SRK_E_ARGS; }
    int rc = cov_check_args(h, n_frames_sel, frames, frame_cov, n_points_sel, points, point_cov);
    if (rc != SRK_OK) return rc;
    HIPCHK(h, hipSetDevice(h->device));
    if ((rc = clear_poison(h)) != SRK_OK) return rc;
    if ((rc = phase_derivatives(h)) != SRK_OK) return rc;
    h->last_slot = 0;
    if ((rc = phase_schur(h, h->att[0], 0.0)) != SRK_OK) return rc;
    rc = phase_covariance(h, n_frames_sel, frames, frame_cov, n_points_sel, points, point_cov);
    if (rc != 0) return rc;
    const int fv = h->d.fv;
    const double k = 2.0 * (sigma_pixels / h->f0) * (sigma_pixels / h->f0);
    for (int64_t e = 0; e < (int64_t)fv * fv * n_frames_sel; ++e) frame_cov[e] *= k;
    for (int64_t e = 0; e < 9 * n_points_sel; ++e) point_cov[e] *= k;
    if (caller_coordinates && h->normalized_on_upload) srk_ba_revert_covariances(&h->nrm, fv, n_frames_sel, frame_cov, n_points_sel, point_cov);
    return 0;
}

}


struct CovPairArgs {
    int64_t n_ff; const int32_t* ff_a; const int32_t* ff_b; double* ff_blocks;
    int64_t n_pf; const int64_t* pf_point; const int32_t* pf_frame; double* pf_blocks;
    int64_t n_pp; const int64_t* pp_a; const int64_t* pp_b; double* pp_blocks;
};

static void cov_cross_map(const srk_ba_normalizer& nrm, int fv, double* D)
{
    const double is = 1.0 / nrm.world_scale;
    const int n = fv ? fv : 3, off = fv ? fv - 6 : 0;
    std::fill(D, D + n * n, 0.0);
    for (int i = 0; i < off; ++i) D[i * n + i] = 1.0;
    for (int a = 0; a < 3; ++a)
        for (int b = 0; b < 3; ++b) {
            D[(off + a) * n + off + b] = nrm.R0[3 * b + a] * is;
            if (fv) D[(off + 3 + a) * n + off + 3 + b] = nrm.R0[3 * b + a];
        }
}
static void cov_revert_cross(const double* Dp, int np, const double* Dq, int nq, double* B)
{
    double T[100];
    for (int i = 0; i < np; ++i)
        for (int j = 0; j < nq; ++j) {
            double v = 0;
            for (int k = 0; k < np; ++k) v += Dp[i * np + k] * B[k * nq + j];
            T[i * nq + j] = v;
        }
    for (int i = 0; i < np; ++i)
        for (int j = 0; j < nq; ++j) {
            double v = 0;
            for (int k = 0; k < nq; ++k) v += T[i * nq + k] * Dq[j * nq + k];
            B[i * nq + j] = v;
        }
}

static int cov_cross_check_args(srk_ba* h, const CovPairArgs& q)
{
    if (q.n_ff < 0 || q.n_pf < 0 || q.n_pp < 0 || (q.n_ff > 0 && (!q.ff_a || !q.ff_b || !q.ff_blocks)) ||
        (q.n_pf > 0 && (!q.pf_point || !q.pf_frame || !q.pf_blocks)) || (q.n_pp > 0 && (!q.pp_a || !q.pp_b || !q.pp_blocks))) {
        h->last_error = "cross-covariance: a negative count, or a NULL array with a positive count";
        return SRK_E_ARGS;
    }
    if (q.n_ff + q.n_pf + q.n_pp > INT32_MAX / 2) { h->last_error = "cross-covariance: too many pairs in one call"; return SRK_E_ARGS; }
    if (h->world > 1 || h->allreduce || h->comm) { h->last_error = "cross-covariance: more than one rank is not supported"; return SRK_E_ARGS; }
    if (h->shk_G > 0) { h->last_error = "cross-covariance: intrinsic groups are not supported"; return SRK_E_ARGS; }
    const auto bad_f = [&](int32_t f) { return f < 0 || f >= h->d.M; };
    const auto bad_p = [&](int64_t i) { return i < 0 || i >= h->d.N; };
    for (int64_t k = 0; k < q.n_ff; ++k)
        if (bad_f(q.ff_a[k]) || bad_f(q.ff_b[k])) { h->last_error = "cross-covariance: a frame index is out of range"; return SRK_E_ARGS; }
    for (int64_t k = 0; k < q.n_pf; ++k) {
        if (bad_p(q.pf_point[k])) { h->last_error = "cross-covariance: a landmark index is out of range"; return SRK_E_ARGS; }
        if (bad_f(q.pf_frame[k])) { h->last_error = "cross-covariance: a frame index is out of range"; return SRK_E_ARGS; }
    }
    for (int64_t k = 0; k < q.n_pp; ++k)
        if (bad_p(q.pp_a[k]) || bad_p(q.pp_b[k])) { h->last_error = "cross-covariance: a landmark index is out of range"; return SRK_E_ARGS; }
    return SRK_OK;
}

static int phase_cross_covariance(srk_ba* h, const CovPairArgs& q)
{
    const SrkDims& d = h->d;
    srk_ba::Attempt& a = h->att[0];
    hipStream_t s = a.stream;
    const int fv = d.fv;
    const double c = h->last_hessian_factor;
    const int64_t n_rows = fv * (int64_t)d.M;
    const int32_t n_tiles = (int32_t)((n_rows + 63) / 64);
    const int64_t n_all = q.n_ff + q.n_pf + q.n_pp;
    std::vector<int64_t> pt_int;
    int rc = cov_prepare(h, n_all > 0, q.n_pf + q.n_pp > 0, pt_int);
// ... 42 lines not shown
    std::vector<int32_t> blk;
    for (size_t b0 = 0; b0 < pairs.size();) {
        size_t b1 = b0;
        int64_t cols = 0;
        members.clear();
        for (; b1 < pairs.size(); ++b1) {
            const Pair& x = pairs[b1];
            const int64_t need = (slot[(size_t)x.p] < 0 ? blocks[(size_t)x.p].ncols : 0) +
                                 (x.q != x.p && slot[(size_t)x.q] < 0 ? blocks[(size_t)x.q].ncols : 0);
            if (cols + need > max_cols) break;
            for (int32_t m : { x.p, x.q })
                if (slot[(size_t)m] < 0) { slot[(size_t)m] = 0; members.push_back(m); }
            cols += need;
        }
        std::stable_sort(members.begin(), members.end(), [&](int32_t x, int32_t y) { return blocks[(size_t)x].first_row < blocks[(size_t)y].first_row; });
        grp.clear();
        cols = 0;
        for (int32_t m : members) {
            SrkCovGroup g = blocks[(size_t)m];
            g.col0 = (int32_t)cols;
            cols += g.ncols;
            slot[(size_t)m] = (int32_t)grp.size();
            grp.push_back(g);
        }
        const int64_t ncp = (cols + SRK_COV_CB - 1) / SRK_COV_CB * SRK_COV_CB;
        blk.assign((size_t)(ncp / SRK_COV_CB), n_tiles);
        for (const SrkCovGroup& g : grp)
            for (int64_t cb = g.col0 / SRK_COV_CB; cb <= (g.col0 + g.ncols - 1) / SRK_COV_CB; ++cb)
                blk[(size_t)cb] = std::min<int32_t>(blk[(size_t)cb], g.first_row / 64);
        tab.clear();
        int32_t n_kind[3] = { 0, 0, 0 };
        for (int kind = 0; kind < 3; ++kind)
            for (size_t k = b0; k < b1; ++k)
                if (pairs[k].kind == kind) {
                    pairs[k].res = (int64_t)(b0 + tab.size());
                    tab.push_back(SrkCovPair{ slot[(size_t)pairs[k].p], slot[(size_t)pairs[k].q] });
                    ++n_kind[kind];
                }
        const int32_t ng = (int32_t)grp.size(), npr = (int32_t)tab.size();
        if ((rc = dev_alloc(h, h->cov_Y, (size_t)(8 * d.ld * ncp))) != SRK_OK) return rc;
        if ((rc = dev_alloc(h, h->cov_grp, sizeof(SrkCovGroup) * grp.size())) != SRK_OK) return rc;
        if ((rc = dev_alloc(h, h->cov_blk, 4 * blk.size())) != SRK_OK) return rc;
        if ((rc = dev_alloc(h, h->cov_pairs, sizeof(SrkCovPair) * tab.size())) != SRK_OK) return rc;
        if ((rc = dev_alloc(h, h->cov_out, (size_t)(800 * (int64_t)npr))) != SRK_OK) return rc;
        HIPCHK(h, hipMemcpyAsync(h->cov_grp.p, grp.data(), sizeof(SrkCovGroup) * grp.size(), hipMemcpyHostToDevice, s));
        HIPCHK(h, hipMemcpyAsync(h->cov_blk.p, blk.data(), 4 * blk.size(), hipMemcpyHostToDevice, s));
        HIPCHK(h, hipMemcpyAsync(h->cov_pairs.p, tab.data(), sizeof(SrkCovPair) * tab.size(), hipMemcpyHostToDevice, s));
        HIPCHK(h, hipMemsetAsync(h->cov_Y.p, 0, (size_t)(8 * 64 * (int64_t)n_tiles * ncp), s));
        HIPCHK(h, hipMemsetAsync(h->cov_out.p, 0, (size_t)(800 * (int64_t)npr), s));
        srk_launch_cov_rhs(s, d, c, P<SrkCovGroup>(h->cov_grp), ng, P<int64_t>(h->row_ptr), P<int32_t>(h->obs_frame), P<double>(h->W),
                           P<double>(h->Vg), P<uint8_t>(h->cov_free), P<double>(h->cov_Y), ncp, P<int>(a.info));
        srk_launch_cov_fwd(s, d.ld, P<double>(a.S), P<double>(a.dinv), P<int64_t>(h->cov_colb), n_tiles, P<int32_t>(h->cov_blk),
                           P<double>(h->cov_Y), ncp);
        srk_launch_cov_cross(s, d, c, P<SrkCovGroup>(h->cov_grp), P<SrkCovPair>(h->cov_pairs), n_kind[0], n_kind[1], n_kind[2], P<double>(h->Vg),
                             P<double>(h->cov_Y), ncp, n_rows, P<double>(h->cov_out));
        HIPCHK(h, hipGetLastError());
        HIPCHK(h, hipMemcpyAsync(res.data() + 100 * b0, h->cov_out.p, (size_t)(800 * (int64_t)npr), hipMemcpyDeviceToHost, s));
        HIPCHK(h, hipStreamSynchronize(s));
        for (int32_t m : members) slot[(size_t)m] = -1;
        b0 = b1;
    }
    int info = 0;
    if ((rc = read_info(h, a, &info)) != SRK_OK) return rc;
    if (info) return 1;
    const int shape[3][2] = { { fv, fv }, { 3, fv }, { 3, 3 } };
    for (const Pair& x : pairs)
        for (int e = 0; e < shape[x.kind][0] * shape[x.kind][1]; ++e)
            if (!std::isfinite(res[(size_t)(100 * x.res + e)])) return 1;
    double* const outs[3] = { q.ff_blocks, q.pf_blocks, q.pp_blocks };
    const int64_t counts[3] = { q.n_ff, q.n_pf, q.n_pp };
    for (int kind = 0; kind < 3; ++kind)
        if (counts[kind] > 0) std::fill(outs[kind], outs[kind] + counts[kind] * shape[kind][0] * shape[kind][1], 0.0);
    for (const Pair& x : pairs) {
        const int n = shape[x.kind][0] * shape[x.kind][1];
        std::memcpy(outs[x.kind] + x.dst * n, res.data() + 100 * x.res, sizeof(double) * (size_t)n);
    }
    return 0;
}

static int cov_build_undamped(srk_ba* h)
{
    int rc;
    if ((rc = clear_poison(h)) != SRK_OK) return rc;
    if ((rc = phase_derivatives(h)) != SRK_OK) return rc;
    h->last_slot = 0;
    return phase_schur(h, h->att[0], 0.0);
}

extern "C" {

int srk_ba_phase_cross_covariance(srk_ba* h, int64_t n_ff, const int32_t* ff_a, const int32_t* ff_b, double* ff_blocks, int64_t n_pf,
                                  const int64_t* pf_point, const int32_t* pf_frame, double* pf_blocks, int64_t n_pp, const int64_t* pp_a,
                                  const int64_t* pp_b, double* pp_blocks)
{
    if (!h || !h->have_scene) return SRK_E_STATE;
    const CovPairArgs q{ n_ff, ff_a, ff_b, ff_blocks, n_pf, pf_point, pf_frame, pf_blocks, n_pp, pp_a, pp_b, pp_blocks };
    int rc = cov_cross_check_args(h, q);
    if (rc != SRK_OK) return rc;
    HIPCHK(h, hipSetDevice(h->device));
    return phase_cross_covariance(h, q);
}

int srk_ba_revert_cross_covariances(const srk_ba_normalizer* nrm, int frame_vars, int64_t n_ff, double* ff_blocks, int64_t n_pf,
                                    double* pf_blocks, int64_t n_pp, double* pp_blocks)
{
    if (!nrm || (frame_vars != 6 && frame_vars != 10) || n_ff < 0 || n_pf < 0 || n_pp < 0 || (n_ff > 0 && !ff_blocks) ||
        (n_pf > 0 && !pf_blocks) || (n_pp > 0 && !pp_blocks) || !(nrm->world_scale > 0) || !std::isfinite(nrm->world_scale))
        return SRK_E_ARGS;
    const int fv = frame_vars;
    double Df[100], Dp[9];
    cov_cross_map(*nrm, fv, Df);
    cov_cross_map(*nrm, 0, Dp);
    for (int64_t k = 0; k < n_ff; ++k) cov_revert_cross(Df, fv, Df, fv, ff_blocks + (int64_t)fv * fv * k);
    for (int64_t k = 0; k < n_pf; ++k) cov_revert_cross(Dp, 3, Df, fv, pf_blocks + (int64_t)3 * fv * k);
    for (int64_t k = 0; k < n_pp; ++k) cov_revert_cross(Dp, 3, Dp, 3, pp_blocks + 9 * k);
    return SRK_OK;
}

int srk_ba_cross_covariances(srk_ba* h, double sigma_pixels, int64_t n_ff, const int32_t* ff_a, const int32_t* ff_b, double* ff_cov,
                             int64_t n_pf, const int64_t* pf_point, const int32_t* pf_frame, double* pf_cov, int64_t n_pp,
                             const int64_t* pp_a, const int64_t* pp_b, double* pp_cov, int caller_coordinates)
{
    if (!h || !h->have_scene) return SRK_E_STATE;
    if (!(sigma_pixels > 0) || !std::isfinite(sigma_pixels)) { h->last_error = "cross-covariances: sigma_pixels must be finite and positive"; return SRK_E_ARGS; }
    const CovPairArgs q{ n_ff, ff_a, ff_b, ff_cov, n_pf, pf_point, pf_frame, pf_cov, n_pp, pp_a, pp_b, pp_cov };
    int rc = cov_cross_check_args(h, q);
    if (rc != SRK_OK) return rc;
    HIPCHK(h, hipSetDevice(h->device));
    if ((rc = cov_build_undamped(h)) != SRK_OK) return rc;
    if ((rc = phase_cross_covariance(h, q)) != 0) return rc;
    const int fv = h->d.fv;
    const double k = 2.0 * (sigma_pixels / h->f0) * (sigma_pixels / h->f0);
    for (int64_t e = 0; e < (int64_t)fv * fv * n_ff; ++e) ff_cov[e] *= k;
    for (int64_t e = 0; e < (int64_t)3 * fv * n_pf; ++e) pf_cov[e] *= k;
    for (int64_t e = 0; e < 9 * n_pp; ++e) pp_cov[e] *= k;
    if (caller_coordinates && h->normalized_on_upload) {
        double Df[100], Dp[9];
        cov_cross_map(h->nrm, fv, Df);
        cov_cross_map(h->nrm, 0, Dp);
        const auto square = [](const double* D, int n, bool swapped, double* B) {
            const auto transpose = [&] {
                for (int i = 0; i < n; ++i)
                    for (int j = i + 1; j < n; ++j) std::swap(B[i * n + j], B[j * n + i]);
            };
            if (swapped) transpose();
            cov_revert_cross(D, n, D, n, B);
            if (swapped) transpose();
        };
        for (int64_t e = 0; e < n_ff; ++e) {
            double* B = ff_cov + (int64_t)fv * fv * e;
            if (ff_a[e] == ff_b[e]) cov_revert_frame(h->nrm, fv, B);
            else square(Df, fv, ff_a[e] > ff_b[e], B);
        }
        for (int64_t e = 0; e < n_pf; ++e) cov_revert_cross(Dp, 3, Df, fv, pf_cov + (int64_t)3 * fv * e);
        for (int64_t e = 0; e < n_pp; ++e) {
            if (pp_a[e] == pp_b[e]) cov_revert_point(h->nrm, pp_cov + 9 * e);
            else square(Dp, 3, pp_a[e] > pp_b[e], pp_cov + 9 * e);
        }
    }
    return 0;
}

int srk_ba_relative_pose_covariances(srk_ba* h, double sigma_pixels, int32_t n, const int32_t* frame_a, const int32_t* frame_b, double* cov)
{
    if (!h || !h->have_scene) return SRK_E_STATE;
    if (!(sigma_pixels > 0) || !std::isfinite(sigma_pixels)) { h->last_error = "relative-pose covariances: sigma_pixels must be finite and positive"; return SRK_E_ARGS; }
    if (n < 0 || (n > 0 && (!frame_a || !frame_b || !cov))) {
        h->last_error = "relative-pose covariances: a negative count, or a NULL array with a positive count";
        return SRK_E_ARGS;
// ... 67 lines not shown
            for (int cc = r; cc < 6; ++cc) {
                double v = 0;
                for (int e = 0; e < 12; ++e) v += JS[r][e] * J[cc][e];
                v *= kf * (r < 3 ? is : 1.0) * (cc < 3 ? is : 1.0);
                out[6 * r + cc] = out[6 * cc + r] = v;
            }
    }
    return 0;
}

}


namespace {

struct LmRun {
    enum { Done = 0, Again = 1 };
    enum class Decrease { Undecided, Accepted, Overflow, Converged };

    srk_ba* const h;
    srk_ba_report* const rep;
    const double* const allowed_err_change;
    const double* const max_hessian_factor;
    const int64_t max_iterations;
    const std::chrono::steady_clock::time_point t_begin = std::chrono::steady_clock::now();
    double hessian_factor = (double)0.0001f;
    double err_value = 0;
    bool result_true = false, spec_wanted = false, spec_drain = false;
    int64_t prev_attempts = 0;
    Decrease decrease = Decrease::Undecided;
    bool have_prev = false, jac_timed = false, dp_mode = false;
    double err_new_prev = 0, err_new = 0;
    int accepted_slot = 0, round = 0;
    unsigned spec_in_flight = 0;
    std::chrono::steady_clock::time_point t_iter;

    bool undecided() const { return decrease == Decrease::Undecided; }
    int fail_device(int rc)
    {
        rep->status = SRK_STATUS_DEVICE_ERROR;
        rep->optimized = 0;
        return rc;
    }
    double ev_ms(int a, int b) const
    {
        float ms = 0;
        if (h->profile_level < 1 || hipEventElapsedTime(&ms, h->ev[a], h->ev[b]) != hipSuccess) return 0.0;
        return (double)ms;
    }
    int mark(int i)
    {
        if (h->profile_level >= 1) HIPCHK(h, hipEventRecord(h->ev[i], h->main_stream));
        return SRK_OK;
    }

    int begin()
    {
        hipStream_t s = h->main_stream;
        const SrkDims& d = h->d;
        srk_ba::Attempt& a0 = h->att[0];
        h->iter_log.clear();
        rep->world_scale = h->nrm.world_scale;
        rearm_fusion(h);
        int rc = clear_poison(h);
        if (rc != SRK_OK) return rc;
        for (auto& a : h->att)
            if (a.allocated) {
                HIPCHK(h, hipMemsetAsync(a.info.p, 0, 4, s));
                HIPCHK(h, hipMemsetAsync(a.acc.p, 0, 8 * 3 * d.Ns + 64, s));
            }
        HIPCHK(h, hipStreamSynchronize(s));
        if (h->seen_global < 0) {
            double seen_d = (double)d.O;
            if (h->allreduce || h->comm) {
                HIPCHK(h, hipMemcpyAsync(a0.err_dst, &seen_d, 8, hipMemcpyHostToDevice, s));
                rc = exchange(h, a0, a0.err_dst, 1);
                if (rc != SRK_OK) return fail_device(rc);
                HIPCHK(h, hipMemcpyAsync(&seen_d, a0.err_dst, 8, hipMemcpyDeviceToHost, s));
                HIPCHK(h, hipStreamSynchronize(s));
            }
            h->seen_global = (int64_t)seen_d;
        }
        rep->seen = h->seen_global;

        double err_initial = 0;
        if ((rc = mark(0)) != SRK_OK) return rc;
        rc = phase_error(h, a0, h->cur, nullptr);
        if (rc != SRK_OK) return fail_device(rc);
        if ((rc = mark(1)) != SRK_OK) return rc;
        HIPCHK(h, hipMemcpyAsync(&err_initial, a0.err_dst, 8, hipMemcpyDeviceToHost, s));
        HIPCHK(h, hipStreamSynchronize(s));
        rep->ms_error += ev_ms(0, 1);
        rep->err_initial = rep->err_final = err_value = err_initial;
        if (allowed_err_change && err_initial < *allowed_err_change) {
            rep->status = SRK_STATUS_ABS_ERR_THRESHOLD;
            result_true = true;
            return Done;
        }
        return Again;
    }

    int enqueue_schur(int sl, double c)
    {
        srk_ba::Attempt& a = h->att[sl];
        int r2 = SRK_OK, e;
        if (sl >= 1 && hipStreamWaitEvent(a.stream, h->ev_jac, 0) != hipSuccess) r2 = SRK_E_DEVICE;
        if (sl == 0 && (e = mark(2)) != SRK_OK) return e;
        if (r2 == SRK_OK) r2 = phase_schur(h, a, c);
        if (sl == 0 && (e = mark(3)) != SRK_OK) return e;
        return r2;
    }
    int enqueue_rest(int sl, double c)
    {
        srk_ba::Attempt& a = h->att[sl];
        int e, r2 = phase_solve(h, a, h->profile_level >= 2);
        if (sl == 0 && (e = mark(4)) != SRK_OK) return e;
        if (r2 == SRK_OK) r2 = phase_backsub_apply(h, a, c);
        if (sl == 0 && (e = mark(5)) != SRK_OK) return e;
        if (r2 == SRK_OK) r2 = phase_cam_apply(h, a);
        if (sl == 0 && (e = mark(6)) != SRK_OK) return e;
        if (r2 == SRK_OK) r2 = phase_error(h, a, a.trial, nullptr, true);
        if (sl == 0 && (e = mark(7)) != SRK_OK) return e;
        if (r2 == SRK_OK && hipMemcpyAsync(a.host_back, a.err_dst, 24, hipMemcpyDeviceToHost, a.stream) != hipSuccess)
            r2 = SRK_E_DEVICE;
        if (r2 == SRK_OK && hipEventRecord(a.done, a.stream) != hipSuccess) r2 = SRK_E_DEVICE;
        return r2;
    }
    int redo_unfused(int sl, double c)
    {
        fusion_off(h);
        if (srk_debug()) fprintf(stderr, "srk_ba[rank %d]: hand-off timeout in the fused solve (slot %d); repeating unfused\n", h->rank, sl);
        h->poisoned = true;
        int r2 = clear_poison(h);
        if (r2 == SRK_OK) r2 = enqueue_schur(sl, c);
        if (r2 == SRK_OK) r2 = enqueue_rest(sl, c);
        return r2;
    }

    int judge(int sl)
    {
        if (hipStreamSynchronize(h->att[sl].stream) != hipSuccess) return SRK_E_DEVICE;
        const double* hb = h->att[sl].host_back;
        const bool multi_rank = (h->allreduce || h->comm) && !dp_mode;
        if (multi_rank ? ((int)hb[1] != 0 && h->att[sl].sync.fused) : (((int)hb[1] & 8) != 0 && !dp_mode)) {
            int r2 = redo_unfused(sl, hessian_factor);
            if (r2 != SRK_OK) return r2;
            if (hipStreamSynchronize(h->att[sl].stream) != hipSuccess) return SRK_E_DEVICE;
        }
        struct { double err; int info; } back{ hb[0], (int)hb[1] };
        const int info2 = (int)hb[2];
        rep->attempts += 1;
        rep->schur_launches += 2;
        h->last_slot = sl;
        if (srk_debug())
            fprintf(stderr, "srk_ba[rank %d] iteration %lld attempt %lld (slot %d, +%.3f ms): hessian_factor %.3g err %.17g -> "
                            "%.17g, solver info %d, point-update info %d\n", h->rank, (long long)rep->iterations + 1,
                    (long long)rep->attempts, sl,
                    std::chrono::duration<double, std::milli>(std::chrono::steady_clock::now() - t_iter).count(),
                    hessian_factor, err_value, back.err, back.info, info2);
        if (back.info != 0 || info2 != 0) { h->poisoned = true; decrease = Decrease::Overflow; return SRK_OK; }
        err_new = back.err;
        if (err_new - err_value < 0) { decrease = Decrease::Accepted; accepted_slot = sl; return SRK_OK; }
        if (have_prev && allowed_err_change) {
            double change = err_new - err_new_prev;
            if (std::fabs(change) < *allowed_err_change) { decrease = Decrease::Converged; return SRK_OK; }
        }
        hessian_factor *= 10;
        if (max_hessian_factor && hessian_factor > *max_hessian_factor) { decrease = Decrease::Overflow; return SRK_OK; }
        err_new_prev = err_new;
        have_prev = true;
        return SRK_OK;
    }

    int pair_round()
    {
        const bool multi = h->allreduce || h->comm;
        const bool can_speculate = h->speculate && h->att[1].allocated && h->profile_level == 0 &&
                                   (!multi || (h->spec_multi && (h->allreduce || h->comm2)));
        const bool pair_pays = round == 0 ? (spec_wanted || rep->iterations >= 1) : (round >= 2 || prev_attempts >= 4);
        const int want = (can_speculate && pair_pays) ? 2 : 1;
        int n_now = 1;
        for (double cc = hessian_factor * 10; n_now < want && !(max_hessian_factor && cc > *max_hessian_factor); cc *= 10) ++n_now;
        const bool speculate_now = n_now >= 2;
        ++round;
        double cfk[SRK_SLOTS];
        for (int k = 0; k < SRK_SLOTS; ++k) cfk[k] = k == 0 ? hessian_factor : cfk[k - 1] * 10;
        int rc = enqueue_schur(0, cfk[0]);
        if (multi) {
            if (rc == SRK_OK) rc = enqueue_rest(0, cfk[0]);
            if (rc == SRK_OK && speculate_now) rc = enqueue_schur(1, cfk[1]);
        } else {
            for (int k = 1; k < n_now && rc == SRK_OK; ++k) rc = enqueue_schur(k, cfk[k]);
            if (rc == SRK_OK) rc = enqueue_rest(0, cfk[0]);
        }
        for (int k = 1; k < n_now && rc == SRK_OK; ++k) rc = enqueue_rest(k, cfk[k]);
        if (rc != SRK_OK) return fail_device(rc);
        for (int k = 1; k < n_now; ++k) spec_in_flight |= 1u << k;
        rc = judge(0);
        if (rc != SRK_OK) return fail_device(rc);
        if (!jac_timed) {
            rep->ms_jacobian += ev_ms(0, 1);
            rep->ms_jacobian_kernel += ev_ms(12, 13);
            jac_timed = true;
        }
        rep->ms_schur += ev_ms(2, 3);
        rep->ms_solve += ev_ms(3, 4);
        rep->ms_backsub += ev_ms(4, 5);
        rep->ms_apply += ev_ms(5, 6);
        rep->ms_error += ev_ms(6, 7);
        if (h->profile_level >= 2) {
            for (size_t kb = 0; kb < h->att[0].solve_prof.n; ++kb) {
                float ms = 0;
                if (hipEventElapsedTime(&ms, h->chol_ev[2 * kb], h->chol_ev[2 * kb + 1]) == hipSuccess)
                    rep->ms_solve_syrk += ms;
            }
            rep->solve_mfma_flops += h->att[0].solve_prof.flops;
        }
        if (undecided()) spec_wanted = true;
        for (int k = 1; k < n_now && undecided(); ++k) {
            rc = judge(k);
            if (rc != SRK_OK) return fail_device(rc);
            spec_in_flight &= ~(1u << k);
        }
        return SRK_OK;
    }

    int dp_round(int G, const double* cf)
    {
        double* ptrs[SRK_SLOTS];
        int64_t counts[SRK_SLOTS];
        const bool verify = h->comm != nullptr && !h->dp_verified;
        double expect[2 * SRK_SLOTS] = {}, rootv[2 * SRK_SLOTS] = {};
        int r2 = dp_build_and_reduce(G, cf, ptrs, counts, verify ? expect : nullptr);
        if (verify && (r2 = dp_verify_reduce(G, r2, ptrs, counts, expect)) == SRK_RETRY_ALLREDUCE) return r2;
        if (r2 == SRK_OK) r2 = dp_solve_and_broadcast(G, ptrs, counts, verify ? rootv : nullptr);
        if (verify && (r2 = dp_verify_broadcast(G, r2, ptrs, counts, rootv)) == SRK_RETRY_ALLREDUCE) return r2;
        if (r2 == SRK_OK) r2 = dp_score(G, cf);
        if (r2 == SRK_OK) r2 = dp_collect_status(G);
        return r2;
    }
    int dp_build_and_reduce(int G, const double* cf, double** ptrs, int64_t* counts, double* expect)
    {
        int r2 = SRK_OK;
        for (int k = 0; k < G && r2 == SRK_OK; ++k) {
            srk_ba::Attempt& a = h->att[k];
            if (k > 0 && hipStreamWaitEvent(a.stream, h->ev_jac, 0) != hipSuccess) r2 = SRK_E_DEVICE;
            if (r2 == SRK_OK) r2 = phase_schur(h, a, cf[k], true);
            if (r2 == SRK_OK) r2 = schur_pack(h, a);
            ptrs[k] = P<double>(a.packed);
            counts[k] = h->band_packed + h->d.ld;
        }
        if (expect && r2 == SRK_OK) {
            for (int k = 0; k < G && r2 == SRK_OK; ++k) r2 = dp_checksum(h, h->att[k].stream, ptrs[k], counts[k], expect + 2 * k);
            if (r2 == SRK_OK) r2 = dp_allreduce_host(h, expect, 2 * G);
        }
        if (r2 == SRK_OK) r2 = coll_group(h, SRK_COLL_REDUCE, G, ptrs, counts);
        return r2;
    }
    int dp_solve_and_broadcast(int G, double** ptrs, int64_t* counts, double* rootv)
    {
        int r2 = SRK_OK;
        for (int k = 0; k < G && r2 == SRK_OK; ++k) {
            srk_ba::Attempt& a = h->att[k];
            if (h->rank == k % h->world) {
                r2 = schur_unpack(h, a);
                if (r2 == SRK_OK) r2 = phase_solve(h, a, false);
            }
            ptrs[k] = P<double>(a.dc);
            counts[k] = h->d.ld;
        }
        if (rootv && r2 == SRK_OK) {
            for (int k = 0; k < G && r2 == SRK_OK; ++k)
                if (h->rank == k % h->world) r2 = dp_checksum(h, h->att[k].stream, ptrs[k], counts[k], rootv + 2 * k);
            if (r2 == SRK_OK) r2 = dp_allreduce_host(h, rootv, 2 * G);
        }
        if (r2 == SRK_OK) r2 = coll_group(h, SRK_COLL_BCAST, G, ptrs, counts);
        return r2;
    }
    int dp_score(int G, const double* cf)
    {
        int r2 = SRK_OK;
        for (int k = 0; k < G && r2 == SRK_OK; ++k) {
            srk_ba::Attempt& a = h->att[k];
            r2 = phase_backsub_apply(h, a, cf[k]);
            if (r2 == SRK_OK) r2 = phase_cam_apply(h, a);
            if (r2 == SRK_OK) r2 = phase_error(h, a, a.trial, nullptr, true, true);
        }
        return r2;
    }
    int dp_collect_status(int G)
    {
        if (h->comm) {
            for (int k = 0; k < G; ++k) {
                if (hipEventRecord(h->att[k].ev_b, h->att[k].stream) != hipSuccess ||
                    hipStreamWaitEvent(h->comm_stream, h->att[k].ev_b, 0) != hipSuccess) return SRK_E_DEVICE;
            }
            ncclResult_t nr = rccl().AllReduce(h->status_all.p, h->status_all.p, (size_t)(8 * G), ncclDouble, ncclSum, h->comm, h->comm_stream);
            if (nr != ncclSuccess) { h->last_error = std::string("ncclAllReduce: ") + rccl().GetErrorString(nr); return SRK_E_DEVICE; }
            if (hipMemcpyAsync(h->dp_back, h->status_all.p, (size_t)(64 * G), hipMemcpyDeviceToHost, h->comm_stream) != hipSuccess ||
                hipStreamSynchronize(h->comm_stream) != hipSuccess) return SRK_E_DEVICE;
        } else {
            for (int k = 0; k < G; ++k)
                if (hipStreamSynchronize(h->att[k].stream) != hipSuccess) return SRK_E_DEVICE;
            if (h->allreduce(h->allreduce_ctx, P<double>(h->status_all), 8 * G) != 0) { h->last_error = "allreduce hook failed"; return SRK_E_DEVICE; }
            if (hipMemcpy(h->dp_back, h->status_all.p, (size_t)(64 * G), hipMemcpyDeviceToHost) != hipSuccess) return SRK_E_DEVICE;
        }
        for (int k = 0; k < G; ++k)
            for (int e = 0; e < 3; ++e) h->att[k].host_back[e] = h->dp_back[8 * k + e];
        return SRK_OK;
    }
    int dp_selfcheck_failed(const char* what)
    {
        h->dp_schedule = false;
        h->dp_selfcheck_failed = true;
        h->last_error = std::string("damping-parallel schedule: self-check of the first native round failed (") + what +
                        "); this handle runs the all-reduce schedule";
        if (srk_debug()) fprintf(stderr, "srk_ba[rank %d]: %s\n", h->rank, h->last_error.c_str());
        return SRK_RETRY_ALLREDUCE;
    }
    int dp_verify_reduce(int G, int r2, double* const* ptrs, const int64_t* counts, const double* expect)
    {
        if (r2 == SRK_E_DEVICE) return dp_selfcheck_failed("an RCCL call of the reduce group returned an error");
        double bad = 0;
        for (int k = 0; k < G && r2 == SRK_OK; ++k) {
            if (h->rank != k % h->world) continue;
            double got[2];
            r2 = dp_checksum(h, h->att[k].stream, ptrs[k], counts[k], got);
            if (!(std::fabs(got[0] - expect[2 * k]) <= 1e-9 * expect[2 * k + 1] + 1e-300)) bad += 1;
        }
#ifdef SRK_DEV
        if (g_dp_corrupt == 1) bad += 1, g_dp_corrupt = 0;
#endif
        if (r2 == SRK_OK) r2 = dp_allreduce_host(h, &bad, 1);
        if (r2 == SRK_OK && bad > 0) return dp_selfcheck_failed("a reduced band does not sum to the all-reduced checksum");
        return r2;
    }
    int dp_verify_broadcast(int G, int r2, double* const* ptrs, const int64_t* counts, const double* rootv)
    {
        if (r2 == SRK_E_DEVICE) return dp_selfcheck_failed("an RCCL call of the broadcast group returned an error");
        double bad = 0;
        for (int k = 0; k < G && r2 == SRK_OK; ++k) {
            double got[2];
            r2 = dp_checksum(h, h->att[k].stream, ptrs[k], counts[k], got);
            if (got[0] == got[0] && rootv[2 * k] == rootv[2 * k] && (got[0] != rootv[2 * k] || got[1] != rootv[2 * k + 1])) bad += 1;
        }
#ifdef SRK_DEV
        if (g_dp_corrupt == 2) bad += 1, g_dp_corrupt = 0;
#endif
        if (r2 == SRK_OK) r2 = dp_allreduce_host(h, &bad, 1);
        if (r2 == SRK_OK && bad > 0) return dp_selfcheck_failed("broadcast corrections differ from the solving rank's");
        if (r2 == SRK_OK) h->dp_verified = true;
        return r2;
    }
    int dp_rounds()
    {
        while (dp_mode && undecided()) {
            double cf[SRK_SLOTS];
            int G = 0;
            for (double cc = hessian_factor; G < SRK_SLOTS && h->att[G].allocated; cc *= 10) {
                if (G > 0 && max_hessian_factor && cc > *max_hessian_factor) break;
                cf[G++] = cc;
            }
            int rc = dp_round(G, cf);
            if (rc == SRK_RETRY_ALLREDUCE) {
                dp_mode = false;
                h->poisoned = true;
                rc = clear_poison(h);
                if (rc != SRK_OK) return fail_device(rc);
                break;
            }
            if (rc != SRK_OK) return fail_device(rc);
            bool timeout = false;
            for (int k = 0; k < G; ++k) timeout = timeout || (((int)h->att[k].host_back[1] & 8) != 0);
            if (timeout && h->chol_fused) {
                fusion_off(h);
                h->poisoned = true;
                rc = clear_poison(h);
                if (rc != SRK_OK) return fail_device(rc);
                continue;
            }
            for (int k = 0; k < G && undecided(); ++k) {
                rc = judge(k);
                if (rc != SRK_OK) return fail_device(rc);
            }
        }
        return SRK_OK;
    }

    int iterate()
    {
        hipStream_t s = h->main_stream;
        if (max_iterations > 0 && rep->iterations >= max_iterations) {
            rep->status = SRK_STATUS_MAX_ITERATIONS;
            result_true = false;
            return Done;
        }
        int rc;
        if ((rc = mark(0)) != SRK_OK) return rc;
        rc = phase_derivatives(h);
        if (rc != SRK_OK) return fail_device(rc);
        if ((rc = mark(1)) != SRK_OK) return rc;
        rep->jacobian_launches += 2;
        HIPCHK(h, hipEventRecord(h->ev_jac, s));
        t_iter = std::chrono::steady_clock::now();

        decrease = Decrease::Undecided;
        have_prev = jac_timed = false;
        err_new_prev = 0, err_new = std::nan("");
        accepted_slot = round = 0;
        spec_in_flight = 0;
        dp_mode = (h->allreduce || h->comm) && (h->world >= 2 || h->dp_force) && h->dp_schedule &&
                  h->profile_level == 0 && h->att[1].allocated;
        const int64_t attempts_before = rep->attempts;
        if ((rc = dp_rounds()) != SRK_OK) return rc;
        while (undecided())
            if ((rc = pair_round()) != SRK_OK) return rc;
        prev_attempts = rep->attempts - attempts_before;
        if (spec_in_flight) {
            for (int k = 1; k < SRK_SLOTS; ++k)
                if (spec_in_flight & (1u << k)) HIPCHK(h, hipStreamWaitEvent(s, h->att[k].done, 0));
            spec_in_flight = 0;
            spec_drain = true;
        }
        if (decrease != Decrease::Accepted) {
            rep->status = decrease == Decrease::Overflow ? SRK_STATUS_HESSIAN_OVERFLOW : SRK_STATUS_ERR_CONVERGED;
            result_true = false;
            return Done;
        }
        {
            const int newcur = h->att[accepted_slot].trial;
            h->att[accepted_slot].trial = h->cur;
            h->cur = newcur;
        }
        rep->iterations += 1;
        if (h->iter_log.size() < (size_t)1 << 20)
            h->iter_log.push_back({ (int32_t)prev_attempts, std::chrono::duration<double, std::milli>(std::chrono::steady_clock::now() - t_begin).count(),
                                    err_new, hessian_factor });
        double change = err_new - err_value;
        rep->err_final = err_new;
        if (allowed_err_change && std::fabs(change) < *allowed_err_change) {
            rep->status = SRK_STATUS_SMALL_ERR_CHANGE;
            result_true = true;
            return Done;
        }
        err_value = err_new;
        hessian_factor /= 10;
        return Again;
    }

    int finish()
    {
        if (spec_drain) {
            for (int k = 1; k < SRK_SLOTS; ++k) {
                if (!h->att[k].allocated) continue;
                HIPCHK(h, hipStreamSynchronize(h->att[k].stream));
                if (h->att[k].host_back[1] != 0.0 || h->att[k].host_back[2] != 0.0) h->poisoned = true;
            }
        }
        rep->hessian_factor = hessian_factor;
        rep->optimized = result_true ? 1 : 0;
        rep->ms_total = std::chrono::duration<double, std::milli>(std::chrono::steady_clock::now() - t_begin).count();
        return result_true ? 0 : 1;
    }
};

}

extern "C" {

int srk_ba_optimize(srk_ba* h, const double* allowed_err_change, const double* max_hessian_factor,
                    int64_t max_iterations, srk_ba_report* rep)
{
    srk_ba_report local;
    if (!rep) rep = &local;
    std::memset(rep, 0, sizeof *rep);
    if (!h || !h->have_scene) return SRK_E_STATE;
    HIPCHK(h, hipSetDevice(h->device));
    LmRun run{ h, rep, allowed_err_change, max_hessian_factor, max_iterations };
    struct LeanGuard {
        srk_ba* h;
        explicit LeanGuard(srk_ba* hh) : h(hh) { h->lean_resets = true; }
        ~LeanGuard() { h->lean_resets = false; }
    } lean_guard(h);
    int rc = run.begin();
    while (rc == LmRun::Again) rc = run.iterate();
    return rc < 0 ? rc : run.finish();
}

int srk_ba_compute_inplace(srk_ba* h, double f0, int64_t N, double* pts, int32_t M, double* cam_R, double* cam_T,
                           const double* K, int shared_k, const int64_t* row_ptr, const int32_t* obs_frame,
                           const double* obs_uv, const double* allowed_err_change, const double* max_hessian_factor,
                           int64_t max_iterations, srk_ba_report* rep)
{
    srk_ba_report local;
    if (!rep) rep = &local;
    std::memset(rep, 0, sizeof *rep);
    if (!h) return SRK_E_ARGS;
    int rc = srk_ba_upload_scene(h, f0, N, pts, M, cam_R, cam_T, K, shared_k, row_ptr, obs_frame, obs_uv, 0);
    if (rc == 1) {
        rep->status = SRK_STATUS_NONE;
        return 1;
    }
    if (rc != SRK_OK) return rc;
    int result = srk_ba_optimize(h, allowed_err_change, max_hessian_factor, max_iterations, rep);
    if (result < 0) return result;
    if (!h->cst_set) {
        rc = srk_ba_download_scene(h, pts, cam_R, cam_T, 1);
        if (rc != SRK_OK) return rc;
        return result;
    }
    std::vector<double> p2((size_t)(3 * N)), r2((size_t)(9 * (int64_t)M)), t2((size_t)(3 * (int64_t)M));
    rc = srk_ba_download_scene(h, p2.data(), r2.data(), t2.data(), 1);
    if (rc != SRK_OK) return rc;
    for (int64_t i = 0; i < N; ++i)
        if (h->cst_point_user.empty() || !h->cst_point_user[(size_t)i]) std::memcpy(pts + 3 * i, &p2[(size_t)(3 * i)], 24);
    for (int32_t j = 0; j < M; ++j)
        if (h->cst_frame_user.empty() || !h->cst_frame_user[(size_t)j]) {
            std::memcpy(cam_R + 9 * (int64_t)j, &r2[9 * (size_t)j], 72);
            std::memcpy(cam_T + 3 * (int64_t)j, &t2[3 * (size_t)j], 24);
        }
    return result;
}

static int score_scene(srk_ba* h, double f0, int64_t N, const double* pts, int32_t M, const double* cam_R,
                       const double* cam_T, const double* K, int shared_k, const int64_t* row_ptr,
                       const int32_t* obs_frame, const double* obs_uv, int32_t min_frames, double z_tol, double* err,
                       int64_t* count)
{
    int rc = validate_scene(h, f0, N, pts, M, cam_R, cam_T, K, row_ptr, obs_frame, obs_uv, min_frames);
    if (rc != SRK_OK) return rc;
    HIPCHK(h, hipSetDevice(h->device));
    hipStream_t s = h->main_stream;
    const int64_t O = row_ptr[N];
    std::vector<int32_t> obs_pt((size_t)O);
// ... 584 lines not shown
    }
    return build_envelope(h);
}

int srk_ba_set_rcs_mode(srk_ba* h, int use_envelope)
{
    if (!h) return SRK_E_ARGS;
    h->use_envelope = use_envelope != 0;
    h->use_chunks = use_envelope != 1;
    if (h->have_scene) return build_envelope(h);
    return SRK_OK;
}

int srk_ba_rcs_chunks(srk_ba* h) { return (h && h->have_scene) ? h->att[0].plan.P : 0; }

double srk_ba_rcs_fill(srk_ba* h)
{
    if (!h || !h->have_scene) return -1.0;
    double full = 0.5 * (double)h->d.ld * (double)h->d.ld;
    return (double)h->env_packed / full;
}

double srk_ba_solve_mfma_flops(srk_ba* h)
{
    if (!h || !h->have_scene) return -1.0;
    SrkSolveProf dry;
    dry.dry = true;
    return launch_solve(h, h->att[0], &dry) == SRK_OK ? dry.flops : -1.0;
}

int srk_ba_set_solver_fusion(srk_ba* h, int on)
{
    if (!h || (on != 0 && on != 1)) return SRK_E_ARGS;
    h->chol_fused = h->chol_fused_wanted = on != 0;
    h->fusion_rearms_left = SRK_FUSION_RETRIES;
    for (auto& a : h->att) a.sync.fused = h->chol_fused;
    return SRK_OK;
}
int64_t srk_ba_solver_sync_timeouts(srk_ba* h) { return h ? h->sync_timeouts : -1; }
int64_t srk_ba_iteration_log(srk_ba* h, int64_t cap, int32_t* attempts, double* ms_since_start, double* err, double* hessian_factor)
{
    if (!h) return -1;
    const int64_t n = (int64_t)h->iter_log.size();
    for (int64_t k = 0; k < n && k < cap; ++k) {
        if (attempts) attempts[k] = h->iter_log[k].attempts;
        if (ms_since_start) ms_since_start[k] = h->iter_log[k].ms;
        if (err) err[k] = h->iter_log[k].err;
        if (hessian_factor) hessian_factor[k] = h->iter_log[k].factor;
    }
    return n;
}
int srk_ba_solver_fusion(srk_ba* h) { return h ? (h->chol_fused ? 1 : 0) : -1; }

int srk_ba_set_deterministic(srk_ba* h, int on)
{
    if (!h) return SRK_E_ARGS;
    if (refuse_modes(h, h->fixed_k, on != 0, h->store_f32, h->schur_fp32, h->world, !h->igroup_user.empty())) return SRK_E_ARGS;
    h->deterministic = on != 0;
    return SRK_OK;
}
int srk_ba_deterministic(srk_ba* h) { return (h && h->have_scene && h->det_active) ? 1 : 0; }
int srk_ba_set_multi_schedule(srk_ba* h, int mode)
{
    if (!h || mode < 0 || mode > 2) return SRK_E_ARGS;
    h->dp_schedule = mode != 0;
    h->dp_force = mode == 2;
    h->dp_selfcheck_failed = false;
    return SRK_OK;
}
int srk_ba_multi_schedule(srk_ba* h)
{
    if (!h) return -1;
    if (h->dp_selfcheck_failed) return 3;
    if (!h->dp_schedule) return 0;
    return h->dp_verified ? 2 : 1;
}
int srk_ba_set_speculation(srk_ba* h, int on)
{
    if (!h || (on != 0 && on != 1)) return SRK_E_ARGS;
    h->speculate = on != 0;
    return SRK_OK;
}

int srk_ba_set_frame_reordering(srk_ba* h, int mode)
{
    if (!h || mode < -1 || mode > 1) return SRK_E_ARGS;
    h->frame_order_mode = mode;
    return SRK_OK;
}
int srk_ba_set_frame_order(srk_ba* h, const int32_t* to_internal, int32_t n_frames)
{
    if (!h || (to_internal && n_frames < 1)) return SRK_E_ARGS;
    if (!to_internal) { h->frame_order_given.clear(); return SRK_OK; }
    std::vector<char> hit((size_t)n_frames, 0);
    for (int32_t j = 0; j < n_frames; ++j) {
        if (to_internal[j] < 0 || to_internal[j] >= n_frames || hit[(size_t)to_internal[j]]) { h->last_error = "set_frame_order: not a permutation"; return SRK_E_ARGS; }
        hit[(size_t)to_internal[j]] = 1;
    }
    h->frame_order_given.assign(to_internal, to_internal + n_frames);
    return SRK_OK;
}
int srk_ba_frame_order(srk_ba* h, int32_t* to_internal)
{
    if (!h || !h->have_scene) return SRK_E_STATE;
    for (int32_t j = 0; to_internal && j < h->d.M; ++j) to_internal[j] = h->frame_int.empty() ? j : h->frame_int[(size_t)j];
    return h->frame_int.empty() ? 0 : 1;
}
int srk_frame_order(int mode, int64_t N, int32_t M, const int64_t* row_ptr, const int32_t* obs_frame, int32_t* to_internal)
{
    if (N < 0 || M < 1 || !row_ptr || (row_ptr[N] > 0 && !obs_frame) || !to_internal) return SRK_E_ARGS;
    std::vector<int32_t> to_int;
    const bool on = srk_frame_reorder(mode, N, M, row_ptr, obs_frame, to_int);
    for (int32_t j = 0; j < M; ++j) to_internal[j] = on ? to_int[(size_t)j] : j;
    return on ? 1 : 0;
}

int srk_ba_set_jacobian_mode(srk_ba* h, int mode)
{
    if (!h || mode < -1 || mode > 2) return SRK_E_ARGS;
    h->jac_mode = mode;
    return SRK_OK;
}
int srk_ba_jacobian_kernel(srk_ba* h) { return (h && h->have_scene) ? (h->jac_runs ? (h->jac_runs_masked ? 3 : 2) : (h->jac_fused ? 1 : 0)) : -1; }

int srk_ba_set_storage_precision(srk_ba* h, int f32)
{
    if (!h || (f32 != 0 && f32 != 1)) return SRK_E_ARGS;
    if (refuse_modes(h, h->fixed_k, h->deterministic, f32 != 0, h->schur_fp32, h->world, !h->igroup_user.empty())) return SRK_E_ARGS;
    h->store_f32 = f32 != 0;
    return SRK_OK;
}

int srk_ba_set_schur_precision(srk_ba* h, int fp32)
{
    if (!h || (fp32 != 0 && fp32 != 1)) return SRK_E_ARGS;
    if (refuse_modes(h, h->fixed_k, h->deterministic, h->store_f32, fp32 != 0, h->world, !h->igroup_user.empty())) return SRK_E_ARGS;
    h->schur_fp32 = fp32 != 0;
    return SRK_OK;
}

int srk_ba_set_fixed_intrinsics(srk_ba* h, int on)
{
    if (!h || (on != 0 && on != 1)) return SRK_E_ARGS;
    if (refuse_modes(h, on != 0, h->deterministic, h->store_f32, h->schur_fp32, h->world, !h->igroup_user.empty())) return SRK_E_ARGS;
    h->fixed_k = on != 0;
    return SRK_OK;
}
int srk_ba_frame_vars(srk_ba* h)
{
    if (!h) return SRK_E_ARGS;
    if (h->have_scene) return h->shk_G > 0 ? 6 : h->d.fv;
    return (h->fixed_k || !h->igroup_user.empty()) ? 6 : 10;
}

int srk_ba_set_intrinsic_groups(srk_ba* h, const int32_t* group, int32_t n_frames, int32_t n_groups)
{
    if (!h) return SRK_E_ARGS;
    if (!group) {
        h->igroup_user.clear();
        h->igroup_n = 0;
        return SRK_OK;
    }
    if (n_groups < 1 || n_groups > SRK_SHK_MAX_GROUPS) { h->last_error = "intrinsic groups: the number of groups must be 1..32"; return SRK_E_ARGS; }
    if (n_frames < 1) { h->last_error = "intrinsic groups: need at least one frame"; return SRK_E_ARGS; }
    std::vector<int32_t> used((size_t)n_groups, 0);
    for (int32_t j = 0; j < n_frames; ++j) {
// ... 567 lines not shown
```

Measured before the change: 371.3.

## Add look-ahead scheduling that starts next iteration's derivatives on speculative acceptance

Adds a look-ahead optimizer loop. While the current damping attempt is still being judged, a trial that lowers the error immediately starts computing the next iteration's Jacobian, Schur complement and solve into a second set of derivative buffers (la_W, la_Vg, la_Ug, la_dj_stage) on the attempt streams. If that trial is accepted, the buffers are swapped in and the next iteration resumes the pipelined work, hiding host round-trips and serial derivative latency. It is on by default for single-rank scenes without intrinsic groups below an observations-per-CU threshold. The cost is extra device memory, much more complex host bookkeeping, and wasted GPU work when the speculated trial is rejected.

```diff
diff --git a/include/srk_ba.h b/include/srk_ba.h
--- a/include/srk_ba.h
+++ b/include/srk_ba.h
@@ -162,6 +162,8 @@
 
 int srk_ba_set_speculation(srk_ba*, int on);
 
+int srk_ba_set_lookahead(srk_ba*, int on);
+
 int srk_ba_set_deterministic(srk_ba*, int on);
 int srk_ba_deterministic(srk_ba*);
 
diff --git a/surikatoko_amd/_lib.py b/surikatoko_amd/_lib.py
--- a/surikatoko_amd/_lib.py
+++ b/surikatoko_amd/_lib.py
@@ -50,7 +50,7 @@
 EXPORTS = [
     "srk_ba_create", "srk_ba_destroy", "srk_ba_last_error", "srk_ba_status_string", "srk_ba_device_count",
     "srk_ba_set_stream", "srk_ba_set_allreduce", "srk_ba_rccl_get_unique_id", "srk_ba_rccl_init", "srk_ba_rccl_init_second", "srk_ba_rccl_set_comm", "srk_ba_compute_inplace", "srk_ba_compute_inplace_f32", "srk_ba_reproj_error", "srk_ba_reproj_error_mvf", "srk_mvf_estimate_depths", "srk_mvf_relative_motion",
-    "srk_mvf_project_onto_so3", "srk_ba_set_schur_precision", "srk_ba_set_storage_precision", "srk_ba_set_speculation", "srk_ba_set_deterministic", "srk_ba_deterministic", "srk_ba_set_multi_schedule", "srk_ba_multi_schedule", "srk_ba_set_frame_reordering", "srk_ba_set_frame_order", "srk_ba_frame_order", "srk_frame_order", "srk_ba_set_solver_fusion", "srk_ba_solver_sync_timeouts", "srk_ba_iteration_log", "srk_ba_solver_fusion", "srk_ba_set_jacobian_mode", "srk_ba_jacobian_kernel", "srk_ba_set_fixed_intrinsics", "srk_ba_frame_vars", "srk_ba_schur_fallback_landmarks",
+    "srk_mvf_project_onto_so3", "srk_ba_set_schur_precision", "srk_ba_set_storage_precision", "srk_ba_set_speculation", "srk_ba_set_lookahead", "srk_ba_set_deterministic", "srk_ba_deterministic", "srk_ba_set_multi_schedule", "srk_ba_multi_schedule", "srk_ba_set_frame_reordering", "srk_ba_set_frame_order", "srk_ba_frame_order", "srk_frame_order", "srk_ba_set_solver_fusion", "srk_ba_solver_sync_timeouts", "srk_ba_iteration_log", "srk_ba_solver_fusion", "srk_ba_set_jacobian_mode", "srk_ba_jacobian_kernel", "srk_ba_set_fixed_intrinsics", "srk_ba_frame_vars", "srk_ba_schur_fallback_landmarks",
     "srk_ba_set_robust_loss", "srk_ba_robust_loss", "srk_ba_observation_weights",
     "srk_ba_set_observation_information", "srk_ba_observation_information", "srk_ba_observation_residuals",
     "srk_ba_set_intrinsic_groups", "srk_ba_intrinsic_groups", "srk_ba_download_intrinsics",
diff --git a/surikatoko_amd/ba.py b/surikatoko_amd/ba.py
--- a/surikatoko_amd/ba.py
+++ b/surikatoko_amd/ba.py
@@ -402,6 +402,9 @@
     def set_speculation(self, on=True):
         self._raise(self._lib.srk_ba_set_speculation(C.c_void_p(self._h), C.c_int(int(bool(on)))))
 
+    def set_lookahead(self, on=True):
+        self._raise(self._lib.srk_ba_set_lookahead(C.c_void_p(self._h), C.c_int(int(bool(on)))))
+
     def set_deterministic(self, on=True):
         self._raise(self._lib.srk_ba_set_deterministic(C.c_void_p(self._h), C.c_int(int(bool(on)))))
 
diff --git a/surikatoko_amd/csrc/srk_ba_host.hip b/surikatoko_amd/csrc/srk_ba_host.hip
--- a/surikatoko_amd/csrc/srk_ba_host.hip
+++ b/surikatoko_amd/csrc/srk_ba_host.hip
@@ -32,6 +32,7 @@
 }
 
 #define SRK_FUSION_RETRIES 3
+#define SRK_LA_RING 16
 #define SRK_SLOTS 3
 struct srk_ba : SrkPlanKept {
     int device = 0;
@@ -49,6 +50,11 @@
     DevBuf pts0, camR0, camT0;
     DevBuf row_ptr, obs_frame, obs_pt, obs_uv, col_ptr, fobs_pt, fobs_uv;
     DevBuf W, Vg, Ug, scratch;
+    DevBuf la_W, la_Vg, la_Ug, la_dj_stage;
+    bool lookahead = true;
+    bool la_no_memory = false;
+    hipEvent_t la_ev_jac = nullptr;
+    double* la_back = nullptr;
     int frame_order_mode = -1;
     std::vector<int32_t> frame_order_given;
     DevBuf grp_first, grp_count, grp_nf, grp_frames, obs_slot, pt_mask, gen_list, wg_jmin;
@@ -289,6 +295,8 @@
 #endif
     h->att[0].stream = h->main_stream;
     bool ok = hipEventCreateWithFlags(&h->ev_jac, hipEventDisableTiming) == hipSuccess &&
+              hipEventCreateWithFlags(&h->la_ev_jac, hipEventDisableTiming) == hipSuccess &&
+              hipHostMalloc(reinterpret_cast<void**>(&h->la_back), 8 * 3 * 2 * SRK_LA_RING, hipHostMallocDefault) == hipSuccess &&
               hipEventCreateWithFlags(&h->ev_comm, hipEventDisableTiming) == hipSuccess &&
               hipStreamCreateWithFlags(&h->comm_stream, hipStreamNonBlocking) == hipSuccess &&
               hipHostMalloc(reinterpret_cast<void**>(&h->dp_back), 64 * SRK_SLOTS, hipHostMallocDefault) == hipSuccess &&
@@ -329,7 +337,7 @@
     dev_free(h->status_all);
     if (h->dp_back) hipHostFree(h->dp_back);
     DevBuf* all[] = { &h->K, &h->pts0, &h->camR0, &h->camT0, &h->row_ptr,
-                      &h->obs_frame, &h->obs_pt, &h->obs_uv, &h->col_ptr, &h->fobs_pt, &h->fobs_uv, &h->W, &h->Vg, &h->Ug,
+                      &h->obs_frame, &h->obs_pt, &h->obs_uv, &h->col_ptr, &h->fobs_pt, &h->fobs_uv, &h->W, &h->Vg, &h->Ug, &h->la_W, &h->la_Vg, &h->la_Ug, &h->la_dj_stage,
                       &h->scratch, &h->grp_first, &h->grp_count, &h->grp_nf, &h->grp_frames, &h->obs_slot, &h->pt_mask,
                       &h->gen_list, &h->cal_list, &h->env_col, &h->env_off, &h->wg_jmin, &h->band_col, &h->band_off,
                       &h->dj_ptr, &h->dj_ent, &h->dj_stage, &h->ds_pair_ptr, &h->ds_pair_fa, &h->ds_pair_fb, &h->ds_pair_ent, &h->ds_f_ptr, &h->ds_f_ent,
@@ -355,6 +363,8 @@
         if (e) hipEventDestroy(e);
     for (auto& e : h->chol_ev) hipEventDestroy(e);
     if (h->ev_jac) hipEventDestroy(h->ev_jac);
+    if (h->la_ev_jac) hipEventDestroy(h->la_ev_jac);
+    if (h->la_back) hipHostFree(h->la_back);
     for (auto& e : h->ev_cst)
         if (e) hipEventDestroy(e);
     for (auto& e : h->ev_pri)
@@ -439,6 +449,14 @@
     if (!factors) return nullptr;
     if (groups) return "relative-pose factors: not available with intrinsic groups";
     if (world > 1) return "relative-pose factors: not available with more than one rank";
+    return nullptr;
+}
+#define SRK_LA_MAX_OBS_PER_CU 3500
+static bool lookahead_pays(int64_t observations, int cus) { return observations <= (int64_t)SRK_LA_MAX_OBS_PER_CU * std::max(cus, 1); }
+static const char* lookahead_conflict(bool groups, int world)
+{
+    if (groups) return "look-ahead: the intrinsics of a scene buffer set (intrinsic groups) are not in its pool";
+    if (world > 1) return "look-ahead: one rank only";
     return nullptr;
 }
 static bool refuse_modes(srk_ba* h, bool fixed_k, bool deterministic, bool store_f32, bool schur_fp32, int world, bool groups)
@@ -1214,6 +1232,7 @@
     }
     h->cur = 0;
     for (int sl = 0; sl < SRK_SLOTS; ++sl) h->att[sl].trial = sl + 1;
+    h->la_no_memory = false;
     rc = compute_cam_packs(h, 0);
     if (rc != SRK_OK) return rc;
     HIPCHK(h, hipStreamSynchronize(s));
@@ -1577,6 +1596,10 @@
 #ifdef SRK_DEV
 static int g_dp_corrupt = 0;
 extern "C" void srk_dbg_dp_corrupt(int stage) { g_dp_corrupt = stage; }
+static int g_la_favourite = 0;
+static int64_t g_la_ahead_drops = 0;
+extern "C" void srk_dbg_lookahead_favourite(int ordinal) { g_la_favourite = ordinal; }
+extern "C" int64_t srk_dbg_lookahead_drops(void) { return g_la_ahead_drops; }
 #endif
 static int dp_checksum(srk_ba* h, hipStream_t st, const double* p, int64_t n, double out[2])
 {
@@ -1694,20 +1717,27 @@
     return true;
 }
 
-static int phase_derivatives(srk_ba* h)
+struct SrkDerivSet {
+    void *W, *Vg, *Ug, *dj_stage;
+};
+static SrkDerivSet deriv_set(const srk_ba* h, bool lookahead = false)
+{
+    if (lookahead) return { h->la_W.p, h->la_Vg.p, h->la_Ug.p, h->la_dj_stage.p };
+    return { h->W.p, h->Vg.p, h->Ug.p, h->dj_stage.p };
+}
+
+static int phase_derivatives(srk_ba* h, int c, const SrkDerivSet& ds, hipStream_t s)
 {
     const SrkDims& d = h->d;
-    hipStream_t s = h->main_stream;
-    int c = h->cur;
-    HIPCHK(h, hipMemsetAsync(h->Vg.p, 0, 8 * 9 * d.Ns, s));
-    HIPCHK(h, hipMemsetAsync(h->Ug.p, 0, 8 * SRK_UGS(d.fv) * (int64_t)d.M, s));
+    HIPCHK(h, hipMemsetAsync(ds.Vg, 0, 8 * 9 * d.Ns, s));
+    HIPCHK(h, hipMemsetAsync(ds.Ug, 0, 8 * SRK_UGS(d.fv) * (int64_t)d.M, s));
     if (h->profile_level >= 1) HIPCHK(h, hipEventRecord(h->ev[12], s));
-    const SrkDetJac detj{ P<double>(h->dj_stage), P<int32_t>(h->dj_ptr), P<int32_t>(h->dj_ent) };
+    const SrkDetJac detj{ static_cast<double*>(ds.dj_stage), P<int32_t>(h->dj_ptr), P<int32_t>(h->dj_ent) };
     SrkLoss Ls;
     const SrkLoss* L = robust_loss(h, Ls);
     if (h->jac_runs) {
         srk_launch_jac_runs(s, d, P<double>(h->pts[c]), P<double>(h->cam[c]), P<int64_t>(h->row_ptr), P<int32_t>(h->obs_frame),
-                            P<double>(h->obs_uv), P<double>(h->W), P<double>(h->Vg), P<double>(h->Ug), P<int32_t>(h->jr_first),
+                            P<double>(h->obs_uv), static_cast<double*>(ds.W), static_cast<double*>(ds.Vg), static_cast<double*>(ds.Ug), P<int32_t>(h->jr_first),
                             P<int32_t>(h->jr_count), h->jr_tasks, P<int32_t>(h->jr_jmin),
                             h->jac_runs_masked ? P<int32_t>(h->jr_group) : nullptr,
                             h->jr_own_runs ? P<int32_t>(h->jd_nf) : P<int32_t>(h->grp_nf),
@@ -1717,22 +1747,22 @@
         if (h->profile_level >= 1) HIPCHK(h, hipEventRecord(h->ev[13], s));
     } else if (h->jac_fused) {
         srk_launch_jac_fused(s, d, P<double>(h->pts[c]), P<double>(h->cam[c]), P<int32_t>(h->obs_frame),
-                             P<int32_t>(h->obs_pt), P<double>(h->obs_uv), P<double>(h->W), P<double>(h->Vg),
-                             P<double>(h->Ug), P<int32_t>(h->wg_jmin), L);
+                             P<int32_t>(h->obs_pt), P<double>(h->obs_uv), static_cast<double*>(ds.W), static_cast<double*>(ds.Vg),
+                             static_cast<double*>(ds.Ug), P<int32_t>(h->wg_jmin), L);
         if (h->profile_level >= 1) HIPCHK(h, hipEventRecord(h->ev[13], s));
     } else {
         srk_launch_jac_points(s, d, P<double>(h->pts[c]), P<double>(h->cam[c]), P<int32_t>(h->obs_frame),
-                              P<int32_t>(h->obs_pt), P<double>(h->obs_uv), P<double>(h->W), P<double>(h->Vg), L);
+                              P<int32_t>(h->obs_pt), P<double>(h->obs_uv), static_cast<double*>(ds.W), static_cast<double*>(ds.Vg), L);
         if (h->profile_level >= 1) HIPCHK(h, hipEventRecord(h->ev[13], s));
         srk_launch_jac_frames(s, d, h->max_frame_obs, P<double>(h->pts[c]), P<double>(h->cam[c]),
-                              P<int64_t>(h->col_ptr), P<int32_t>(h->fobs_pt), P<double>(h->fobs_uv), P<double>(h->Ug), L);
+                              P<int64_t>(h->col_ptr), P<int32_t>(h->fobs_pt), P<double>(h->fobs_uv), static_cast<double*>(ds.Ug), L);
     }
     HIPCHK(h, hipGetLastError());
     SrkPrior pr;
     if (const SrkPrior* prior = position_priors(h, pr)) {
         const bool timed = h->profile_level >= 1 && pri_events(h);
         if (timed) HIPCHK(h, hipEventRecord(h->ev_pri[0], s));
-        srk_launch_prior_add(s, d, P<double>(h->pts[c]), P<double>(h->cam[c]), *prior, P<double>(h->Vg), P<double>(h->Ug));
+        srk_launch_prior_add(s, d, P<double>(h->pts[c]), P<double>(h->cam[c]), *prior, static_cast<double*>(ds.Vg), static_cast<double*>(ds.Ug));
         if (timed) HIPCHK(h, hipEventRecord(h->ev_pri[1], s));
         h->pri_timed[0] = timed;
         HIPCHK(h, hipGetLastError());
@@ -1741,7 +1771,7 @@
     if (const SrkRelPose* relpose = relpose_factors(h, rpl)) {
         const bool timed = h->profile_level >= 1 && rp_events(h);
         if (timed) HIPCHK(h, hipEventRecord(h->ev_rp[0], s));
-        srk_launch_relpose_add(s, d, P<double>(h->cam[c]), *relpose, P<double>(h->Ug));
+        srk_launch_relpose_add(s, d, P<double>(h->cam[c]), *relpose, static_cast<double*>(ds.Ug));
         if (timed) HIPCHK(h, hipEventRecord(h->ev_rp[1], s));
         h->rp_timed[0] = timed;
         HIPCHK(h, hipGetLastError());
@@ -1749,7 +1779,7 @@
     if (h->n_cst_pts > 0) {
         const bool timed = h->profile_level >= 1 && cst_events(h);
         if (timed) HIPCHK(h, hipEventRecord(h->ev_cst[0], s));
-        srk_launch_const_points(s, d, P<int32_t>(h->cst_pts), h->n_cst_pts, P<int64_t>(h->row_ptr), P<double>(h->W), P<double>(h->Vg));
+        srk_launch_const_points(s, d, P<int32_t>(h->cst_pts), h->n_cst_pts, P<int64_t>(h->row_ptr), static_cast<double*>(ds.W), static_cast<double*>(ds.Vg));
         if (timed) HIPCHK(h, hipEventRecord(h->ev_cst[1], s));
         h->cst_timed[0] = timed;
         HIPCHK(h, hipGetLastError());
@@ -1757,7 +1787,7 @@
     return SRK_OK;
 }
 
-static int phase_schur(srk_ba* h, srk_ba::Attempt& a, double c, bool local_only = false);
+static int phase_schur(srk_ba* h, srk_ba::Attempt& a, double c, const SrkDerivSet& ds, bool local_only = false);
 static int schur_pack(srk_ba* h, srk_ba::Attempt& a)
 {
     const SrkDims& d = h->d;
@@ -1780,7 +1810,7 @@
     HIPCHK(h, hipGetLastError());
     return SRK_OK;
 }
-static int phase_schur(srk_ba* h, srk_ba::Attempt& a, double c, bool local_only)
+static int phase_schur(srk_ba* h, srk_ba::Attempt& a, double c, const SrkDerivSet& ds, bool local_only)
 {
     const SrkDims& d = h->d;
     hipStream_t s = a.stream;
@@ -1789,24 +1819,24 @@
                             P<int32_t>(h->ds_pair_fb), P<int32_t>(h->ds_pair_ent), h->ds_n_pairs, P<int32_t>(h->ds_f_ptr), P<int32_t>(h->ds_f_ent) };
     const bool cal = d.fv == 6;
     srk_launch_schur_grouped(s, d, c, P<int64_t>(h->row_ptr), P<int32_t>(h->obs_pt), P<uint8_t>(h->obs_slot),
-                             P<uint32_t>(h->pt_mask), P<double>(h->W), P<double>(h->Vg), P<double>(a.S),
+                             P<uint32_t>(h->pt_mask), static_cast<double*>(ds.W), static_cast<double*>(ds.Vg), P<double>(a.S),
                              P<double>(a.rhs), P<int32_t>(h->grp_first), P<int32_t>(h->grp_count), P<int32_t>(h->grp_nf),
                              P<int32_t>(h->grp_frames), h->n_groups, h->n_groups_wide, h->n_groups_mid,
                              !cal && h->schur_fp32 ? 1 : 0, P<int32_t>(a.irr), h->n_mm_uniform, h->n_mm_ragged,
                              !cal && h->det_active ? &dets : nullptr);
     if (cal) {
-        srk_launch_schur(s, d, c, P<int64_t>(h->row_ptr), P<int32_t>(h->obs_frame), P<double>(h->W), P<double>(h->Vg),
+        srk_launch_schur(s, d, c, P<int64_t>(h->row_ptr), P<int32_t>(h->obs_frame), static_cast<double*>(ds.W), static_cast<double*>(ds.Vg),
                          P<double>(a.S), P<double>(a.rhs), P<int32_t>(h->cal_list), h->n_cal_list);
     } else {
-        srk_launch_schur_long(s, d, c, P<double>(h->W), P<double>(h->Vg), P<double>(a.S), P<double>(a.rhs),
+        srk_launch_schur_long(s, d, c, static_cast<double*>(ds.W), static_cast<double*>(ds.Vg), P<double>(a.S), P<double>(a.rhs),
                               P<int32_t>(h->lg_item), h->n_long_items, P<int32_t>(h->lg_np), P<int32_t>(h->lg_nf), P<int32_t>(h->lg_pts),
                               P<int32_t>(h->lg_frames), P<int64_t>(h->lg_obs_off), P<int32_t>(h->lg_obs), h->long_fb);
-        srk_launch_schur(s, d, c, P<int64_t>(h->row_ptr), P<int32_t>(h->obs_frame), P<double>(h->W), P<double>(h->Vg),
+        srk_launch_schur(s, d, c, P<int64_t>(h->row_ptr), P<int32_t>(h->obs_frame), static_cast<double*>(ds.W), static_cast<double*>(ds.Vg),
                          P<double>(a.S), P<double>(a.rhs), P<int32_t>(h->gen_list), h->n_generic);
     }
     HIPCHK(h, hipGetLastError());
-    srk_launch_assemble(s, d, c, P<double>(h->Ug), P<double>(a.S), P<double>(a.rhs), h->rank == 0 ? 1.0 : 0.0,
-                        P<int64_t>(h->row_ptr), P<int32_t>(h->obs_frame), P<double>(h->W), P<double>(h->Vg), P<int32_t>(a.irr));
+    srk_launch_assemble(s, d, c, static_cast<double*>(ds.Ug), P<double>(a.S), P<double>(a.rhs), h->rank == 0 ? 1.0 : 0.0,
+                        P<int64_t>(h->row_ptr), P<int32_t>(h->obs_frame), static_cast<double*>(ds.W), static_cast<double*>(ds.Vg), P<int32_t>(a.irr));
     HIPCHK(h, hipGetLastError());
     SrkRelPose rpl;
     if (const SrkRelPose* relpose = relpose_factors(h, rpl)) {
@@ -1886,24 +1916,22 @@
     return SRK_OK;
 }
 
-static int phase_backsub_apply(srk_ba* h, srk_ba::Attempt& a, double c)
+static int phase_backsub_apply(srk_ba* h, srk_ba::Attempt& a, double c, int cur, int tr, const SrkDerivSet& ds)
 {
     const SrkDims& d = h->d;
     hipStream_t s = a.stream;
-    int cur = h->cur, tr = a.trial;
     if (!h->lean_resets) HIPCHK(h, hipMemsetAsync(a.acc.p, 0, 8 * 3 * d.Ns + 64, s));
     if (h->shk_G > 0)
         srk_launch_rcs_expand(s, shk_args(h, a), P<double>(a.dcsh), P<double>(a.dc), kbuf(h, cur), kbuf(h, tr));
-    srk_launch_backsub(s, d, c, P<int32_t>(h->obs_frame), P<int32_t>(h->obs_pt), P<double>(h->W), P<double>(h->Vg),
+    srk_launch_backsub(s, d, c, P<int32_t>(h->obs_frame), P<int32_t>(h->obs_pt), static_cast<double*>(ds.W), static_cast<double*>(ds.Vg),
                        P<double>(a.dc), P<double>(a.acc), P<double>(h->pts[cur]), P<double>(h->pts[tr]),
                        P<double>(a.dx));
     HIPCHK(h, hipGetLastError());
     return SRK_OK;
 }
 
-static int phase_cam_apply(srk_ba* h, srk_ba::Attempt& a)
-{
-    int cur = h->cur, tr = a.trial;
+static int phase_cam_apply(srk_ba* h, srk_ba::Attempt& a, int cur, int tr)
+{
     srk_launch_cam_apply(a.stream, h->d.M, P<double>(h->camR[cur]), P<double>(h->camT[cur]), P<double>(a.dc),
                          P<double>(h->camR[tr]), P<double>(h->camT[tr]), kbuf(h, tr), h->f0, P<double>(h->cam[tr]), h->d.fv);
     srk_launch_const_cam_keep(a.stream, P<int32_t>(h->cst_frames), h->n_cst_frames, P<double>(h->camR[cur]), P<double>(h->camT[cur]),
@@ -1925,7 +1953,7 @@
 {
     if (!h || !h->have_scene) return SRK_E_STATE;
     HIPCHK(h, hipSetDevice(h->device));
-    int rc = phase_derivatives(h);
+    int rc = phase_derivatives(h, h->cur, deriv_set(h), h->main_stream);
     if (rc != SRK_OK) return rc;
     HIPCHK(h, hipStreamSynchronize(h->main_stream));
     return SRK_OK;
@@ -1938,7 +1966,7 @@
     h->last_slot = 0;
     int rc = clear_poison(h);
     if (rc != SRK_OK) return rc;
-    rc = phase_schur(h, a, c);
+    rc = phase_schur(h, a, c, deriv_set(h));
     if (rc != SRK_OK) return rc;
     HIPCHK(h, hipStreamSynchronize(a.stream));
     return SRK_OK;
@@ -1977,9 +2005,9 @@
     if (!h || !h->have_scene) return SRK_E_STATE;
     HIPCHK(h, hipSetDevice(h->device));
     srk_ba::Attempt& a = h->att[0];
-    int rc = phase_backsub_apply(h, a, c);
+    int rc = phase_backsub_apply(h, a, c, h->cur, a.trial, deriv_set(h));
     if (rc != SRK_OK) return rc;
-    rc = phase_cam_apply(h, a);
+    rc = phase_cam_apply(h, a, h->cur, a.trial);
     if (rc != SRK_OK) return rc;
     HIPCHK(h, hipStreamSynchronize(a.stream));
     return SRK_OK;
@@ -2224,9 +2252,9 @@
     if (rc != SRK_OK) return rc;
     HIPCHK(h, hipSetDevice(h->device));
     if ((rc = clear_poison(h)) != SRK_OK) return rc;
-    if ((rc = phase_derivatives(h)) != SRK_OK) return rc;
+    if ((rc = phase_derivatives(h, h->cur, deriv_set(h), h->main_stream)) != SRK_OK) return rc;
     h->last_slot = 0;
-    if ((rc = phase_schur(h, h->att[0], 0.0)) != SRK_OK) return rc;
+    if ((rc = phase_schur(h, h->att[0], 0.0, deriv_set(h))) != SRK_OK) return rc;
     rc = phase_covariance(h, n_frames_sel, frames, frame_cov, n_points_sel, points, point_cov);
     if (rc != 0) return rc;
     const int fv = h->d.fv;
@@ -2435,9 +2463,9 @@
 {
     int rc;
     if ((rc = clear_poison(h)) != SRK_OK) return rc;
-    if ((rc = phase_derivatives(h)) != SRK_OK) return rc;
+    if ((rc = phase_derivatives(h, h->cur, deriv_set(h), h->main_stream)) != SRK_OK) return rc;
     h->last_slot = 0;
-    return phase_schur(h, h->att[0], 0.0);
+    return phase_schur(h, h->att[0], 0.0, deriv_set(h));
 }
 
 extern "C" {
@@ -2671,6 +2699,8 @@
             h->seen_global = (int64_t)seen_d;
         }
         rep->seen = h->seen_global;
+        la_on = h->lookahead && h->speculate && h->att[1].allocated && h->profile_level == 0 && lookahead_pays(h->d.O, h->cus) &&
+                !lookahead_conflict(h->shk_G > 0, (h->allreduce || h->comm) ? std::max(h->world, 2) : 1);
 
         double err_initial = 0;
         if ((rc = mark(0)) != SRK_OK) return rc;
@@ -2695,7 +2725,7 @@
         int r2 = SRK_OK, e;
         if (sl >= 1 && hipStreamWaitEvent(a.stream, h->ev_jac, 0) != hipSuccess) r2 = SRK_E_DEVICE;
         if (sl == 0 && (e = mark(2)) != SRK_OK) return e;
-        if (r2 == SRK_OK) r2 = phase_schur(h, a, c);
+        if (r2 == SRK_OK) r2 = phase_schur(h, a, c, deriv_set(h));
         if (sl == 0 && (e = mark(3)) != SRK_OK) return e;
         return r2;
     }
@@ -2704,9 +2734,9 @@
         srk_ba::Attempt& a = h->att[sl];
         int e, r2 = phase_solve(h, a, h->profile_level >= 2);
         if (sl == 0 && (e = mark(4)) != SRK_OK) return e;
-        if (r2 == SRK_OK) r2 = phase_backsub_apply(h, a, c);
+        if (r2 == SRK_OK) r2 = phase_backsub_apply(h, a, c, h->cur, a.trial, deriv_set(h));
         if (sl == 0 && (e = mark(5)) != SRK_OK) return e;
-        if (r2 == SRK_OK) r2 = phase_cam_apply(h, a);
+        if (r2 == SRK_OK) r2 = phase_cam_apply(h, a, h->cur, a.trial);
         if (sl == 0 && (e = mark(6)) != SRK_OK) return e;
         if (r2 == SRK_OK) r2 = phase_error(h, a, a.trial, nullptr, true);
         if (sl == 0 && (e = mark(7)) != SRK_OK) return e;
@@ -2736,8 +2766,11 @@
             if (r2 != SRK_OK) return r2;
             if (hipStreamSynchronize(h->att[sl].stream) != hipSuccess) return SRK_E_DEVICE;
         }
-        struct { double err; int info; } back{ hb[0], (int)hb[1] };
-        const int info2 = (int)hb[2];
+        return judge_numbers(sl, hb[0], (int)hb[1], (int)hb[2]);
+    }
+    int judge_numbers(int sl, double err_back, int info_back, int info2)
+    {
+        struct { double err; int info; } back{ err_back, info_back };
         rep->attempts += 1;
         rep->schur_launches += 2;
         h->last_slot = sl;
@@ -2834,7 +2867,7 @@
         for (int k = 0; k < G && r2 == SRK_OK; ++k) {
             srk_ba::Attempt& a = h->att[k];
             if (k > 0 && hipStreamWaitEvent(a.stream, h->ev_jac, 0) != hipSuccess) r2 = SRK_E_DEVICE;
-            if (r2 == SRK_OK) r2 = phase_schur(h, a, cf[k], true);
+            if (r2 == SRK_OK) r2 = phase_schur(h, a, cf[k], deriv_set(h), true);
             if (r2 == SRK_OK) r2 = schur_pack(h, a);
             ptrs[k] = P<double>(a.packed);
             counts[k] = h->band_packed + h->d.ld;
@@ -2871,8 +2904,8 @@
         int r2 = SRK_OK;
         for (int k = 0; k < G && r2 == SRK_OK; ++k) {
             srk_ba::Attempt& a = h->att[k];
-            r2 = phase_backsub_apply(h, a, cf[k]);
-            if (r2 == SRK_OK) r2 = phase_cam_apply(h, a);
+            r2 = phase_backsub_apply(h, a, cf[k], h->cur, a.trial, deriv_set(h));
+            if (r2 == SRK_OK) r2 = phase_cam_apply(h, a, h->cur, a.trial);
             if (r2 == SRK_OK) r2 = phase_error(h, a, a.trial, nullptr, true, true);
         }
         return r2;
@@ -2976,8 +3009,407 @@
         return SRK_OK;
     }
 
+
+    struct Rec {
+        enum St { SchurEnqueued, RestEnqueued, Done, Judged, Dropped };
+        int64_t id = 0;
+        int gen = 0;
+        int ord = 0;
+        double factor = 0;
+        int base = 0, trial = 0;
+        SrkDerivSet ds{};
+        hipEvent_t ev_deriv = nullptr;
+        int deriv_slot = 0;
+        int slot = 0, ring = 0;
+        St st = SchurEnqueued;
+        bool complete = false;
+        bool own_reject = false;
+        double err = 0;
+        int info = 0, info2 = 0;
+        bool live() const { return st == SchurEnqueued || st == RestEnqueued || st == Done; }
+        bool in_flight() const { return st == SchurEnqueued || st == RestEnqueued; }
+    };
+    bool la_on = false;
+    std::vector<Rec> recs;
+    int64_t la_next_id = 1, la_slot_last[2] = { 0, 0 }, la_ahead_source = 0;
+    int la_ring_next[2] = { 0, 0 };
+    int la_next_judge = 1, la_fav = 1, la_home = 0, la_cur_dslot = 0;
+    bool la_ahead = false;
+    bool la_started = false;
+    bool la_poison = false;
+    Rec la_last_judged;
+
+    void la_trace(const char* what, const Rec& r) const
+    {
+        if (!srk_debug()) return;
+        fprintf(stderr, "srk_ba[rank %d] look-ahead +%.3f ms: %s (iteration %lld%s, ordinal %d, factor %.3g, slot %d, scene %d -> %d)\n", h->rank,
+                std::chrono::duration<double, std::milli>(std::chrono::steady_clock::now() - t_begin).count(), what,
+                (long long)rep->iterations + 1 + r.gen, r.gen ? " ahead" : "", r.ord, r.factor, r.slot, r.base, r.trial);
+    }
+    int la_rec(int gen, int ord) const
+    {
+        for (size_t i = 0; i < recs.size(); ++i)
+            if (recs[i].live() && recs[i].gen == gen && recs[i].ord == ord) return (int)i;
+        return -1;
+    }
+    bool la_slot_busy(int sl) const
+    {
+        for (const Rec& r : recs)
+            if (r.slot == sl && r.in_flight()) return true;
+        return false;
+    }
+    int la_free_set() const
+    {
+        for (int w = 0; w <= SRK_SLOTS; ++w) {
+            if (w == h->cur || !h->pts[w].p || !h->cam[w].p) continue;
+            bool used = false;
+            for (const Rec& r : recs)
+                if (r.live() && ((r.trial == w && !r.own_reject) || r.base == w)) used = true;
+            if (!used) return w;
+        }
+        return -1;
+    }
+    void la_retire()
+    {
+        size_t k = 0;
+        for (size_t i = 0; i < recs.size(); ++i) {
+            Rec& r = recs[i];
+            if (r.complete && !r.live()) {
+                const double* hb = h->la_back + 3 * (SRK_LA_RING * r.slot + r.ring);
+                if (r.st == Rec::Dropped && (hb[1] != 0.0 || hb[2] != 0.0)) la_poison = true;
+                continue;
+            }
+            if (k != i) recs[k] = recs[i];
+            ++k;
+        }
+        recs.resize(k);
+    }
+    void la_drop(Rec& r)
+    {
+        if (!r.live()) return;
+#ifdef SRK_DEV
+        if (r.gen == 1) ++g_la_ahead_drops;
+#endif
+        la_trace("dropped", r);
+        r.st = Rec::Dropped;
+    }
+    int la_order(int sl, int wr, const void* wds)
+    {
+        const int o = 1 - sl;
+        for (const Rec& r : recs)
+            if (r.slot == o && !r.complete && ((wr >= 0 && (r.trial == wr || r.base == wr)) || (wds && r.ds.W == wds))) {
+                if (hipStreamWaitEvent(h->att[sl].stream, h->att[o].done, 0) != hipSuccess) return SRK_E_DEVICE;
+                break;
+            }
+        return SRK_OK;
+    }
+    int la_schur(Rec& r, hipEvent_t behind)
+    {
+        srk_ba::Attempt& a = h->att[r.slot];
+        if (r.deriv_slot != r.slot && hipStreamWaitEvent(a.stream, r.ev_deriv, 0) != hipSuccess) return SRK_E_DEVICE;
+        if (behind && hipStreamWaitEvent(a.stream, behind, 0) != hipSuccess) return SRK_E_DEVICE;
+        int r2 = phase_schur(h, a, r.factor, r.ds);
+        if (r2 == SRK_OK && hipEventRecord(a.ev_a, a.stream) != hipSuccess) r2 = SRK_E_DEVICE;
+        r.st = Rec::SchurEnqueued;
+        return r2;
+    }
+    int la_rest(Rec& r)
+    {
+        srk_ba::Attempt& a = h->att[r.slot];
+        int r2 = la_order(r.slot, r.trial, nullptr);
+        if (r2 == SRK_OK) r2 = phase_solve(h, a, false);
+        if (r2 == SRK_OK) r2 = phase_backsub_apply(h, a, r.factor, r.base, r.trial, r.ds);
+        if (r2 == SRK_OK) r2 = phase_cam_apply(h, a, r.base, r.trial);
+        if (r2 == SRK_OK) r2 = phase_error(h, a, r.trial, nullptr, true);
+        r.ring = la_ring_next[r.slot];
+        la_ring_next[r.slot] = (r.ring + 1) % SRK_LA_RING;
+        double* hb = h->la_back + 3 * (SRK_LA_RING * r.slot + r.ring);
+        hb[0] = hb[1] = hb[2] = 0.0;
+        if (r2 == SRK_OK && hipMemcpyAsync(hb, a.err_dst, 24, hipMemcpyDeviceToHost, a.stream) != hipSuccess) r2 = SRK_E_DEVICE;
+        if (r2 == SRK_OK && hipEventRecord(a.done, a.stream) != hipSuccess) r2 = SRK_E_DEVICE;
+        r.st = Rec::RestEnqueued;
+        la_slot_last[r.slot] = r.id;
+        la_trace("enqueued", r);
+        return r2;
+    }
+    Rec la_new(int gen, int ord, double factor, int sl, int base, int trial, bool ahead_set)
+    {
+        Rec r;
+        r.id = la_next_id++;
+        r.gen = gen, r.ord = ord, r.factor = factor, r.slot = sl, r.base = base, r.trial = trial;
+        r.ds = deriv_set(h, ahead_set);
+        r.ev_deriv = ahead_set ? h->la_ev_jac : h->ev_jac;
+        r.deriv_slot = ahead_set ? la_ahead_dslot : la_cur_dslot;
+        return r;
+    }
+    int la_ahead_dslot = 0;
+    bool la_buffers()
+    {
+        if (h->la_no_memory) return false;
+        struct { DevBuf& b; size_t bytes; } need[] = {
+            { h->la_W, h->W.bytes }, { h->la_Vg, h->Vg.bytes }, { h->la_Ug, h->Ug.bytes },
+            { h->la_dj_stage, h->dj_stage.p ? h->dj_stage.bytes : 8 },
+            { h->pts[SRK_SLOTS], h->pts[0].bytes }, { h->camR[SRK_SLOTS], h->camR[0].bytes },
+            { h->camT[SRK_SLOTS], h->camT[0].bytes }, { h->cam[SRK_SLOTS], h->cam[0].bytes } };
+        for (auto& n : need)
+            if (dev_alloc(h, n.b, n.bytes) != SRK_OK) {
+                h->la_no_memory = true;
+                return false;
+            }
+        return true;
+    }
+    bool la_allow(int ord, bool with_first) const
+    {
+        if (ord == la_next_judge) return true;
+        const int i = la_rec(0, ord - 1);
+        if (i >= 0 && recs[(size_t)i].own_reject) return true;
+        if (ord != la_next_judge + 1 || !with_first) return false;
+        return ord == 2 ? (spec_wanted || rep->iterations >= 1) : (prev_attempts >= 4 || la_next_judge >= 4);
+    }
+    int la_fill()
+    {
+        bool with_first = false;
+        for (int pass = 0; pass < 2; ++pass) {
+            const int sl = pass == 0 ? la_home : 1 - la_home;
+            if (la_slot_busy(sl)) continue;
+            int k = la_next_judge;
+            double f = hessian_factor;
+            while (la_rec(0, k) >= 0) ++k, f *= 10;
+            if (k > la_next_judge && ((max_hessian_factor && f > *max_hessian_factor) || !la_allow(k, with_first))) break;
+            const int trial = la_free_set();
+            if (trial < 0) {
+                if (k > la_next_judge) break;
+                h->last_error = "look-ahead: no free scene buffer set";
+                return SRK_E_STATE;
+            }
+            Rec r = la_new(0, k, f, sl, h->cur, trial, false);
+            int rc = la_schur(r, nullptr);
+            if (rc == SRK_OK) rc = la_rest(r);
+            recs.push_back(r);
+            if (rc != SRK_OK) return rc;
+            with_first = with_first || k == la_next_judge;
+        }
+        return SRK_OK;
+    }
+    int la_look_ahead(size_t i)
+    {
+        const Rec src = recs[i];
+        if (la_ahead) return SRK_OK;
+        if (max_iterations > 0 && rep->iterations + 1 >= max_iterations) return SRK_OK;
+        if (allowed_err_change && std::fabs(src.err - err_value) < *allowed_err_change) return SRK_OK;
+        bool earlier = false;
+        for (const Rec& r : recs) earlier = earlier || (r.gen == 0 && r.in_flight() && r.ord < src.ord);
+        if (!earlier || !la_buffers()) return SRK_OK;
+        const int trial = la_free_set();
+        if (trial < 0) return SRK_OK;
+        const int sl = src.slot;
+        int rc = la_order(sl, -1, h->la_W.p);
+        if (rc == SRK_OK) rc = phase_derivatives(h, src.trial, deriv_set(h, true), h->att[sl].stream);
+        if (rc == SRK_OK && hipEventRecord(h->la_ev_jac, h->att[sl].stream) != hipSuccess) rc = SRK_E_DEVICE;
+        if (rc != SRK_OK) return rc;
+        la_ahead_dslot = sl;
+        int fav = std::min(src.ord, 2);
+#ifdef SRK_DEV
+        if (g_la_favourite > 0) fav = std::min(g_la_favourite, 2);
+#endif
+        double f = src.factor / 10;
+        if (fav == 2 && max_hessian_factor && f * 10 > *max_hessian_factor) fav = 1;
+        if (fav == 2) f *= 10;
+        Rec r = la_new(1, fav, f, sl, src.trial, trial, true);
+        rc = la_schur(r, nullptr);
+        if (rc == SRK_OK) rc = la_rest(r);
+        recs.push_back(r);
+        la_ahead = true;
+        la_ahead_source = src.id;
+        return rc;
+    }
+    int la_timeout(int sl)
+    {
+        if (srk_debug()) fprintf(stderr, "srk_ba[rank %d]: hand-off timeout in the fused solve (slot %d); repeating unfused\n", h->rank, sl);
+        for (int k = 0; k < 2; ++k)
+            if (hipStreamSynchronize(h->att[k].stream) != hipSuccess) return SRK_E_DEVICE;
+        for (Rec& r : recs) {
+            r.complete = true;
+            la_drop(r);
+        }
+        recs.clear();
+        la_ahead = false;
+        fusion_off(h);
+        h->poisoned = true;
+        return clear_poison(h);
+    }
+    int la_on_done(size_t i)
+    {
+        const int sl = recs[i].slot;
+        const int64_t id = recs[i].id;
+        const double* hb = h->la_back + 3 * (SRK_LA_RING * sl + recs[i].ring);
+        recs[i].err = hb[0], recs[i].info = (int)hb[1], recs[i].info2 = (int)hb[2];
+        recs[i].st = Rec::Done;
+        la_trace("done", recs[i]);
+        for (Rec& r : recs)
+            if (r.slot == sl && r.id <= id) r.complete = true;
+        if ((recs[i].info & 8) != 0) return la_timeout(sl);
+        const Rec r = recs[i];
+        if (r.gen != 0 || r.info != 0 || r.info2 != 0) return SRK_OK;
+        if (!(r.err - err_value < 0)) recs[i].own_reject = true;
+        if (r.ord == la_next_judge) return SRK_OK;
+        if (r.err - err_value < 0) return la_look_ahead(i);
+        return la_fill();
+    }
+    int la_wait_any()
+    {
+        int cand[2], n = 0;
+        for (size_t i = 0; i < recs.size(); ++i)
+            if (recs[i].in_flight() && n < 2) cand[n++] = (int)i;
+        if (n == 0) {
+            h->last_error = "look-ahead: nothing in flight";
+            return SRK_E_STATE;
+        }
+        if (n == 1) {
+            if (hipEventSynchronize(h->att[recs[(size_t)cand[0]].slot].done) != hipSuccess) return SRK_E_DEVICE;
+            return la_on_done((size_t)cand[0]);
+        }
+        for (;;)
+            for (int k = 0; k < n; ++k) {
+                const hipError_t e = hipEventQuery(h->att[recs[(size_t)cand[k]].slot].done);
+                if (e == hipSuccess) return la_on_done((size_t)cand[k]);
+                if (e != hipErrorNotReady) return SRK_E_DEVICE;
+            }
+    }
+    int la_start_iteration()
+    {
+        const int home = la_home;
+        srk_ba::Attempt& ah = h->att[home];
+        int rc = la_order(home, -1, h->W.p);
+        if (rc == SRK_OK) rc = phase_derivatives(h, h->cur, deriv_set(h), ah.stream);
+        if (rc == SRK_OK && hipEventRecord(h->ev_jac, ah.stream) != hipSuccess) rc = SRK_E_DEVICE;
+        if (rc != SRK_OK) return rc;
+        la_cur_dslot = home;
+        const bool pair = la_allow(2, true) && !(max_hessian_factor && hessian_factor * 10 > *max_hessian_factor);
+        int fav = pair ? std::min(la_fav, 2) : 1;
+#ifdef SRK_DEV
+        if (pair && g_la_favourite > 0) fav = std::min(g_la_favourite, 2);
+#endif
+        const int t0 = la_free_set();
+        if (t0 < 0) return SRK_E_STATE;
+        Rec first = la_new(0, fav, fav == 2 ? hessian_factor * 10 : hessian_factor, home, h->cur, t0, false);
+        rc = la_schur(first, nullptr);
+        recs.push_back(first);
+        const size_t i0 = recs.size() - 1;
+        if (pair && rc == SRK_OK) {
+            const int t1 = la_free_set();
+            if (t1 < 0) return SRK_E_STATE;
+            Rec second = la_new(0, 3 - fav, fav == 2 ? hessian_factor : hessian_factor * 10, 1 - home, h->cur, t1, false);
+            rc = la_schur(second, ah.ev_a);
+            recs.push_back(second);
+        }
+        if (rc == SRK_OK) rc = la_rest(recs[i0]);
+        if (pair && rc == SRK_OK) rc = la_rest(recs[i0 + 1]);
+        return rc;
+    }
+    int iterate_lookahead()
+    {
+        if (max_iterations > 0 && rep->iterations >= max_iterations) {
+            rep->status = SRK_STATUS_MAX_ITERATIONS;
+            result_true = false;
+            return Done;
+        }
+        decrease = Decrease::Undecided;
+        have_prev = false;
+        err_new_prev = 0, err_new = std::nan("");
+        accepted_slot = 0;
+        la_next_judge = 1;
+        const int64_t attempts_before = rep->attempts;
+        int rc = SRK_OK;
+        rep->jacobian_launches += 2;
+        t_iter = std::chrono::steady_clock::now();
+        if (!la_started && (rc = la_start_iteration()) != SRK_OK) return fail_device(rc);
+        la_started = false;
+        while (undecided()) {
+            la_retire();
+            const int i = la_rec(0, la_next_judge);
+            if (i >= 0 && recs[(size_t)i].st == Rec::Done) {
+                Rec& r = recs[(size_t)i];
+                r.st = Rec::Judged;
+                la_last_judged = r;
+                ++la_next_judge;
+                if ((rc = judge_numbers(r.slot, r.err, r.info, r.info2)) != SRK_OK) return fail_device(rc);
+                if (undecided()) spec_wanted = true;
+                continue;
+            }
+            if ((rc = la_fill()) != SRK_OK) return fail_device(rc);
+            if ((rc = la_wait_any()) != SRK_OK) return fail_device(rc);
+        }
+        prev_attempts = rep->attempts - attempts_before;
+        const Rec acc = la_last_judged;
+        for (Rec& r : recs)
+            if (r.gen == 0) la_drop(r);
+        const bool keep_ahead = decrease == Decrease::Accepted && la_ahead && la_ahead_source == acc.id;
+        if (!keep_ahead)
+            for (Rec& r : recs) la_drop(r);
+        la_ahead = false;
+        if (decrease != Decrease::Accepted) {
+            rep->status = decrease == Decrease::Overflow ? SRK_STATUS_HESSIAN_OVERFLOW : SRK_STATUS_ERR_CONVERGED;
+            result_true = false;
+            return Done;
+        }
+        h->cur = acc.trial;
+        rep->iterations += 1;
+        if (h->iter_log.size() < (size_t)1 << 20)
+            h->iter_log.push_back({ (int32_t)prev_attempts, std::chrono::duration<double, std::milli>(std::chrono::steady_clock::now() - t_begin).count(),
+                                    err_new, hessian_factor });
+        double change = err_new - err_value;
+        rep->err_final = err_new;
+        if (allowed_err_change && std::fabs(change) < *allowed_err_change) {
+            rep->status = SRK_STATUS_SMALL_ERR_CHANGE;
+            result_true = true;
+            return Done;
+        }
+        err_value = err_new;
+        hessian_factor /= 10;
+        la_fav = std::min(acc.ord, 2);
+        la_home = acc.slot;
+        if (keep_ahead) {
+            std::swap(h->W, h->la_W), std::swap(h->Vg, h->la_Vg), std::swap(h->Ug, h->la_Ug), std::swap(h->dj_stage, h->la_dj_stage);
+            std::swap(h->ev_jac, h->la_ev_jac);
+            la_cur_dslot = la_ahead_dslot;
+            for (Rec& r : recs)
+                if (r.gen == 1) r.gen = 0;
+            la_started = true;
+        }
+        return Again;
+    }
+    int finish_lookahead()
+    {
+        for (int k = 0; k < 2; ++k) HIPCHK(h, hipStreamSynchronize(h->att[k].stream));
+        for (Rec& r : recs) {
+            r.complete = true;
+            la_drop(r);
+        }
+        la_retire();
+        int w = 0;
+        for (int k = 0; k < 2; ++k, ++w) {
+            while (w == h->cur || (la_last_judged.id && w == la_last_judged.base)) ++w;
+            h->att[k].trial = w <= SRK_SLOTS && h->pts[w].p ? w : h->att[k].trial;
+        }
+        if (la_last_judged.id && la_slot_last[la_last_judged.slot] != la_last_judged.id) {
+            Rec r = la_last_judged;
+            r.trial = h->att[r.slot].trial;
+            int rc = la_schur(r, nullptr);
+            if (rc == SRK_OK) rc = la_rest(r);
+            if (rc != SRK_OK) return fail_device(rc);
+            HIPCHK(h, hipStreamSynchronize(h->att[r.slot].stream));
+            const double* hb = h->la_back + 3 * (SRK_LA_RING * r.slot + r.ring);
+            if (hb[1] != 0.0 || hb[2] != 0.0) la_poison = true;
+        }
+        if (la_last_judged.id) h->last_hessian_factor = la_last_judged.factor;
+        if (la_poison) h->poisoned = true;
+        return SRK_OK;
+    }
+
     int iterate()
     {
+        if (la_on) return iterate_lookahead();
         hipStream_t s = h->main_stream;
         if (max_iterations > 0 && rep->iterations >= max_iterations) {
             rep->status = SRK_STATUS_MAX_ITERATIONS;
@@ -2986,7 +3418,7 @@
         }
         int rc;
         if ((rc = mark(0)) != SRK_OK) return rc;
-        rc = phase_derivatives(h);
+        rc = phase_derivatives(h, h->cur, deriv_set(h), h->main_stream);
         if (rc != SRK_OK) return fail_device(rc);
         if ((rc = mark(1)) != SRK_OK) return rc;
         rep->jacobian_launches += 2;
@@ -3039,6 +3471,10 @@
 
     int finish()
     {
+        if (la_on) {
+            const int rc = finish_lookahead();
+            if (rc != SRK_OK) return rc;
+        }
         if (spec_drain) {
             for (int k = 1; k < SRK_SLOTS; ++k) {
                 if (!h->att[k].allocated) continue;
@@ -3789,6 +4225,13 @@
     return SRK_OK;
 }
 
+int srk_ba_set_lookahead(srk_ba* h, int on)
+{
+    if (!h || (on != 0 && on != 1)) return SRK_E_ARGS;
+    h->lookahead = on != 0;
+    return SRK_OK;
+}
+
 int srk_ba_set_frame_reordering(srk_ba* h, int mode)
 {
     if (!h || mode < -1 || mode > 1) return SRK_E_ARGS;
```

Result: no change. 370.1 (-0.3%).
